# sile/libflate

Measured on AMD Instinct MI355X. Metric: gzip encode+decode throughput on 256 MiB synthetic text per GPU (uncompressed bytes through the round trip), higher is better.
Workload: dtype u8; 1 GPU; cfg2: gzip::Encoder (DefaultLz77Encoder, default options, mtime=0) + gzip::Decoder on TEXT(268435456 B) per GPU, write schedule S8K (8192-byte writes); bytes_per_gpu=268435456, schedule=S8K, compressed_bytes=129579521, parallelism=1 rank

## Files before the change

include/lfx_testhooks.h:

```cpp
#ifndef LFX_TESTHOOKS_H
#define LFX_TESTHOOKS_H

#include "lfx.h"

#ifdef __cplusplus
extern "C" {
#endif

int lfx_debug_huff_block(const uint32_t *hist320, uint32_t type, uint32_t *lit288, uint32_t *dist32, uint32_t *hdr160,
                         uint32_t *hdr_bits, uint64_t *body_bits);

int lfx_debug_plan(int format, const lfx_encode_opts *o, const lfx_schedule *s, uint64_t n, uint64_t *chunk_out,
                   size_t max_chunks, size_t *n_chunks, uint64_t *block_out, size_t max_blocks, size_t *n_blocks);

int lfx_debug_plan_incremental(int format, const lfx_encode_opts *o, const lfx_schedule *s, uint64_t n,
                               uint32_t take_every, uint64_t *chunk_out, size_t max_chunks, size_t *n_chunks,
                               uint64_t *block_out, size_t max_blocks, size_t *n_blocks);

void lfx_debug_symbols(uint32_t length, uint32_t distance, uint32_t *out6);

#ifdef __cplusplus
}
#endif
#endif
```

libflate_amd/csrc/lfx_ctx.h:

```cpp
#pragma once
#include <hip/hip_runtime.h>

#include <mutex>
#include <string>
#include <vector>

#include "lfx_common.h"
#include "lfx_device.h"
#include <string.h>

#include "lfx_hostio.h"

namespace lfx {

struct DevBuf {
    void *p = nullptr;
    size_t cap = 0;
    uint32_t gen = 0;
    int reserve(size_t bytes);
    void release();
};

struct Diag {
    bool debug = false;
    bool match_v1 = false;
    bool match_v5 = false;
    int r7_cap = 0;
    int match_parts = 1;
    bool no_serial = false;
    bool batch_serial = false;
    bool no_markers = false;
    bool no_pieces = false;
    bool no_final_cand = false;
    bool window_chain = false;
    int free_shift = -1;
    bool no_small_scan = false;
    bool two_pass = false;
    bool no_pin_slots = false;
    int find2_exp = 0;
    bool hist_separate = false;
    bool store_tight = false;
    int enc_batch_mb = 0;
    int pocr_max = 100;
    void read();
};

struct RangeState {
    int state = -1;
    uint64_t total = 0, before = 0, max_len = 0;
    uint8_t *d_out = nullptr;
    uint32_t nsu = 0;
};

struct Ctx {
    int device = 0;
    RangeState range;
    std::vector<uint8_t> range_stored;
    std::vector<uint64_t> range_temp_off;
    std::vector<uint32_t> range_cap;
    Diag diag;
    int n_cu = 0;
    hipStream_t own_stream = nullptr, stream = nullptr;
    hipStream_t side_stream = nullptr;
    hipEvent_t ev_fork = nullptr, ev_join = nullptr, ev_zero = nullptr;
    hipEvent_t ev_part[4] = {}, ev_res = nullptr;
    const void *prezero_ptr = nullptr;
    uint64_t prezero_bytes = 0;
    std::recursive_mutex mu;
    std::string err;
    void set_error(const std::string &e) { err = e; }

    DevBuf d_chunks, d_blocks, d_segs, d_pwgs, d_cd, d_md, d_codes, d_ncodes, d_hist, d_bc, d_block_start, d_tile_bits,
        d_tile_start, d_ck, d_res, d_small, d_hdr, d_io_in, d_io_out, d_vis, d_segtmp, d_stage, d_chunkmap, d_glnk, d_ucount;
    std::vector<uint8_t> up_shadow[4];
    uint64_t up_dev[4] = {0, 0, 0, 0};
    DevBuf d_dec_streams, d_dec_state, d_dec_tmp, d_dec_cand, d_dec_blocks, d_dec_tabs, d_dec_sym, d_dec_win, d_dec_maps,
        d_dec_temp, d_dec_lanesx;
    DevBuf d_idx_tasks, d_idx_probe, d_idx_stage;
    DevBuf d_idx_enc;
    struct IdxCollect *idx = nullptr;
    struct IdxCollect *idx_enc = nullptr;
    std::vector<DevBuf *> all_bufs() {
        return {&d_chunks, &d_blocks, &d_segs, &d_pwgs, &d_cd, &d_md, &d_codes, &d_ncodes, &d_hist, &d_bc, &d_block_start,
                &d_tile_bits, &d_tile_start, &d_ck, &d_res, &d_small, &d_hdr, &d_io_in, &d_io_out, &d_vis, &d_segtmp, &d_stage, &d_chunkmap, &d_glnk, &d_ucount,
                &d_dec_streams, &d_dec_state, &d_dec_tmp, &d_dec_cand, &d_dec_blocks, &d_dec_tabs, &d_dec_sym, &d_dec_win, &d_dec_maps,
                &d_dec_temp, &d_dec_lanesx, &d_idx_tasks, &d_idx_probe, &d_idx_stage, &d_idx_enc};
    }
    void *h_res = nullptr;
    static constexpr size_t PIN_ARENA = 1u << 20;
    size_t pin_used = 0;
    struct PinDown { void *slot, *dst; size_t n; };
    std::vector<PinDown> pin_pending;
    void pin_reset() { pin_used = 0; pin_pending.clear(); }
    void *pin_take(size_t n) {
        const size_t at = (pin_used + 63) & ~(size_t)63;
        if (!h_res || diag.no_pin_slots || at + n > PIN_ARENA) return nullptr;
        pin_used = at + n;
        return (uint8_t *)h_res + 4096 + at;
    }
    hipError_t small_up(void *dev, const void *host, size_t n, hipStream_t st) {
        if (!n) return hipSuccess;
        void *slot = pin_take(n);
        if (!slot) return hipMemcpyAsync(dev, host, n, hipMemcpyHostToDevice, st);
        memcpy(slot, host, n);
        return hipMemcpyAsync(dev, slot, n, hipMemcpyHostToDevice, st);
    }
    hipError_t small_down(void *host, const void *dev, size_t n, hipStream_t st) {
        if (!n) return hipSuccess;
        void *slot = pin_take(n);
        if (!slot) return hipMemcpyAsync(host, dev, n, hipMemcpyDeviceToHost, st);
        pin_pending.push_back({slot, host, n});
        return hipMemcpyAsync(slot, dev, n, hipMemcpyDeviceToHost, st);
    }
    hipError_t small_sync(hipStream_t st) {
        const hipError_t e = hipStreamSynchronize(st);
        for (const PinDown &d : pin_pending) memcpy(d.dst, d.slot, d.n);
        pin_pending.clear();
        return e;
    }

    uint32_t cur_nchunks = 0, cur_nblocks = 0;
    uint64_t cur_ntiles = 0, cur_n = 0;
    const uint32_t *cur_tile_map = nullptr;
    const uint8_t *cur_in = nullptr;
    bool force_match_v1 = false;
    uint64_t match_fallbacks = 0;
    HostIo hostio;
    static constexpr size_t POOL_MAX = 8;
    std::vector<PinVec> pin_pool;
    std::vector<DevBuf> dev_pool;
    PinVec take_pin() {
        std::lock_guard<std::recursive_mutex> lock(mu);
        if (pin_pool.empty()) return PinVec();
        size_t best = 0;
        for (size_t i = 1; i < pin_pool.size(); i++)
            if (pin_pool[i].capacity() > pin_pool[best].capacity()) best = i;
        PinVec v = std::move(pin_pool[best]);
        pin_pool.erase(pin_pool.begin() + (std::ptrdiff_t)best);
        v.clear();
        return v;
    }
    void give_pin(PinVec &&v) {
        std::lock_guard<std::recursive_mutex> lock(mu);
        if (v.capacity() && pin_pool.size() < POOL_MAX) { v.clear(); pin_pool.push_back(std::move(v)); }
    }
    DevBuf take_dev() {
        std::lock_guard<std::recursive_mutex> lock(mu);
        if (dev_pool.empty()) return DevBuf();
        DevBuf b = dev_pool.back();
        dev_pool.pop_back();
        return b;
    }
    void give_dev(DevBuf &b) {
        std::lock_guard<std::recursive_mutex> lock(mu);
        if (b.p && dev_pool.size() < POOL_MAX) dev_pool.push_back(b);
        else b.release();
        b = DevBuf();
    }
    std::vector<uint8_t> shard_hdr;
    int shard_format = 0;
    bool shard_last = false;

    int timing_on = 0;
    bool timing_fine() const { return timing_on >= 2; }
    hipEvent_t ev[17] = {};
    char ev_name[17][24] = {};
    int n_ev = 0;
    void phase(const char *name);
};

struct HostCodes {
    const uint32_t *codes;
    uint64_t n_codes;
    const uint32_t *chunk_codes;
};
int encode_prepare(Ctx *c, const struct Plan &plan, const struct PlanOpts &po, const uint8_t *d_in,
                   uint64_t n, int ck_mode, const HostCodes *hc = nullptr);

}
```

libflate_amd/csrc/lfx_decode.cpp:

```cpp
#include "../../include/lfx.h"

#include <hip/hip_runtime.h>

#include <algorithm>
#include <cstddef>
#include <cstdio>
#include <cstdlib>
#include <cstring>
#include <mutex>
#include <string>
#include <vector>

#include "lfx_ctx.h"
#include "lfx_container.h"
#include "lfx_decode.h"
#include "lfx_index.h"
#include <thread>
#include <chrono>

static_assert(offsetof(lfx::DecStream, out_off) == 16 && sizeof(lfx::DecStream) % 8 == 0, "checksum_ranges stride");
static_assert(offsetof(lfx::InflateResult, out_len) == 8 && sizeof(lfx::InflateResult) % 8 == 0, "checksum_ranges stride");
#include "lfx_device.h"
#include "lfx_abi_guard.h"

using namespace lfx;

#define HIP_TRY(expr)                                                                 \
    do {                                                                              \
        hipError_t e_ = (expr);                                                       \
        if (e_ != hipSuccess) {                                                       \
            c->set_error(std::string(#expr) + ": " + hipGetErrorString(e_));          \
            return LFX_E_DEVICE;                                                      \
        }                                                                             \
    } while (0)
#define LAUNCH_TRY(call)                                                              \
    do {                                                                              \
        int e_ = (call);                                                              \
        if (e_) {                                                                     \
            c->set_error(std::string(#call) + ": " + hipGetErrorString((hipError_t)e_)); \
            return LFX_E_DEVICE;                                                      \
        }                                                                             \
    } while (0)

namespace {

std::string format_error(uint32_t err, uint32_t a0, uint32_t a1) {
    char m[200];
    switch (err) {
        case ERR_EOF: return "failed to fill whole buffer";
        case ERR_HUFF: return "Invalid huffman coded stream";
        case ERR_CONFLICT: snprintf(m, sizeof m, "Bit region conflict: symbol=%u", a0); return m;
        case ERR_HDIST: snprintf(m, sizeof m, "The value of HDIST is too big: max=30, actual=%u", a0); return m;
        case ERR_NO_PREV: return "No preceding value";
        case ERR_DIST_LIST:
            snprintf(m, sizeof m, "The length of `distance_code_bitwidthes` is too large: actual=%u, expected=%u", a0, a1);
            return m;
        case ERR_286: snprintf(m, sizeof m, "The value %u must not occur in compressed data", a0); return m;
        case ERR_BACKREF: snprintf(m, sizeof m, "Too long backword reference: buffer.len=%u, distance=%u", a0, a1); return m;
        case ERR_BTYPE3: return "btype 0x11 of DEFLATE is reserved(error) value";
        case ERR_LEN_NLEN: snprintf(m, sizeof m, "LEN=%u is not the one's complement of NLEN=%u", a0, a1); return m;
        case ERR_STORED_SHORT: snprintf(m, sizeof m, "The reader has incorrect length: expected %u, read %u", a0, a1); return m;
        case ERR_NOSPACE: return "output capacity too small";
        case ERR_ZLIB_CHECK:
            snprintf(m, sizeof m, "Inconsistent ZLIB check bits: `CMF(%u) * 256 + FLG(%u)` must be a multiple of 31", a0, a1);
            return m;
        case ERR_METHOD: snprintf(m, sizeof m, "Compression methods other than DEFLATE(8) are unsupported: method=%u", a0); return m;
        case ERR_CINFO: snprintf(m, sizeof m, "CINFO above 7 are not allowed: value=%u", a0); return m;
        case ERR_FDICT: snprintf(m, sizeof m, "Preset dictionaries are not supported: dictionary_id=0x%X", a0); return m;
        case ERR_GZIP_ID: return "Unexpected GZIP ID";
        case ERR_HCRC: snprintf(m, sizeof m, "CRC16 of GZIP header mismatched: value=%u, expected=%u", a0, a1); return m;
        case ERR_CRC32: snprintf(m, sizeof m, "CRC32 mismatched: value=%u, expected=%u", a0, a1); return m;
        case ERR_ADLER32: snprintf(m, sizeof m, "Adler32 checksum mismatched: value=%u, expected=%u", a0, a1); return m;
        default: return "";
    }
}
int map_status(uint32_t st) {
    return st == 0 ? LFX_OK : st == 1 ? LFX_E_INVALID_DATA : st == 2 ? LFX_E_UNEXPECTED_EOF : LFX_E_NOSPACE;
}

struct MemberResult {
    int status = LFX_OK;
    uint64_t out_len = 0;
    uint64_t blk_out_start = 0;
    uint64_t end_byte = 0;
    std::string msg;
    uint64_t end_bit = 0;
    bool final_seen = false;
    bool need_cap = false;
    int ck_mode = 0;
    uint32_t trailer_len = 0;
    bool ck_done = false;
    uint32_t crc32 = 0, adler32 = 1;
    uint8_t trailer[8] = {0, 0, 0, 0, 0, 0, 0, 0};
};

int run_jobs(Ctx *c, const uint8_t *d_in, uint8_t *d_out, const std::vector<InflateJob> &jobs,
             std::vector<InflateResult> &res) {
    const size_t n = jobs.size();
    res.resize(n);
    if (!n) return LFX_OK;
    int rc;
    if ((rc = c->d_dec_streams.reserve(sizeof(InflateJob) * n))) return rc;
    if ((rc = c->d_dec_state.reserve(sizeof(InflateResult) * n))) return rc;
    HIP_TRY(hipMemcpyAsync(c->d_dec_streams.p, jobs.data(), sizeof(InflateJob) * n, hipMemcpyHostToDevice, c->stream));
    LAUNCH_TRY(launch_inflate(c->stream, d_in, d_out, (const InflateJob *)c->d_dec_streams.p,
                              (InflateResult *)c->d_dec_state.p, (uint32_t)n));
    HIP_TRY(hipMemcpyAsync(res.data(), c->d_dec_state.p, sizeof(InflateResult) * n, hipMemcpyDeviceToHost, c->stream));
    HIP_TRY(hipStreamSynchronize(c->stream));
    return LFX_OK;
}

int inflate_member(Ctx *c, const uint8_t *d_in, uint64_t n, uint64_t off0, uint8_t *d_out, uint64_t cap,
                   MemberResult &mr, uint64_t start_bit0 = ~0ull, uint64_t stop_bit = ~0ull, bool partial = false,
                   uint64_t hist = 0) {
    const uint64_t first_bit = start_bit0 == ~0ull ? off0 * 8 : start_bit0;
    mr.end_bit = first_bit;
    hipStream_t st = c->stream;
    c->pin_reset();
    std::vector<InflateJob> jobs;
    std::vector<InflateResult> res;
    bool parallel_done = false;
    const uint64_t comp = n > off0 ? n - off0 : 0;
    if (comp >= (4u << 10)) {
        int rc;
        bool overflow = false;
        uint32_t n1 = 0;
        std::vector<uint64_t> starts;
        auto find_candidates = [&]() -> int {
            const uint32_t shard_cap = find_shard_cap(comp);
            const uint32_t final_cap = (uint32_t)std::min<uint64_t>(std::max<uint64_t>(1u << 16, comp / 4096), 1u << 24);
            int rc;
            if ((rc = c->d_dec_cand.reserve(8ull * shard_cap * FIND_SHARDS + 8ull * final_cap + 4 * FIND_HDR_WORDS))) return rc;
            uint32_t *d_count = (uint32_t *)c->d_dec_cand.p;
            uint32_t *d_final_count = d_count + FIND_HDR_FINAL;
            uint64_t *d_final = (uint64_t *)((uint8_t *)c->d_dec_cand.p + 4 * FIND_HDR_WORDS);
            uint64_t *d_cand = d_final + final_cap;
            HIP_TRY(hipMemsetAsync(d_count, 0, 4 * FIND_HDR_WORDS, st));
            const uint64_t tail_bytes = std::max<uint64_t>(comp / 8, 8ull << 20);
            const uint64_t final_from = c->diag.no_final_cand ? ~0ull >> 1 : comp > tail_bytes ? (n - tail_bytes) * 8 : 0;
            LAUNCH_TRY(launch_find_stage1(st, d_in, n, off0, d_count, d_cand, shard_cap, final_from, (uint32_t)std::max(c->n_cu, 1)));
            c->phase("find1");
            const int find2_exp = c->diag.find2_exp >= 1 && c->diag.find2_exp <= 4 ? c->diag.find2_exp : 0;
            if (find2_exp) {
                LAUNCH_TRY(launch_find_stage2(st, d_in, n, d_cand, shard_cap, d_count, d_count + FIND_HDR_WORK, d_final_count, d_final, final_cap,
                                              (uint32_t)std::max(c->n_cu, 1), nullptr, find2_exp));
                HIP_TRY(hipMemsetAsync(d_count + FIND_HDR_FINAL, 0, 4, st));
                HIP_TRY(hipMemsetAsync(d_count + FIND_HDR_WORK, 0, 4 * (FIND_HDR_WORDS - FIND_HDR_WORK), st));
                c->phase("find2x");
            }
            LAUNCH_TRY(launch_find_stage2(st, d_in, n, d_cand, shard_cap, d_count, d_count + FIND_HDR_WORK, d_final_count, d_final, final_cap,
                                          (uint32_t)std::max(c->n_cu, 1), c->diag.debug ? (uint64_t *)(d_count + FIND_HDR_DBG) : nullptr));
            constexpr uint32_t HEAD_N = 1024;
            const uint32_t head_n = std::min<uint32_t>(HEAD_N, final_cap);
            std::vector<uint64_t> back(FIND_HDR_WORDS / 2 + head_n);
            HIP_TRY(c->small_down(back.data(), d_count, 8ull * back.size(), st));
            HIP_TRY(c->small_sync(st));
            const uint32_t *hc = (const uint32_t *)back.data();
            std::vector<uint64_t> cand(back.begin() + FIND_HDR_WORDS / 2, back.end());
            overflow = hc[FIND_SHARDS] != 0;
            n1 = 0;
            for (uint32_t k = 0; k < FIND_SHARDS; k++) { if (hc[k] > shard_cap) overflow = true; n1 += hc[k]; }
            if (c->diag.debug) {
                uint64_t d[7];
                memcpy(d, hc + FIND_HDR_DBG, sizeof d);
                fprintf(stderr, "[lfx] finder stage 2: batches=%llu cycles per batch: stage+fields=%llu table=%llu walk=%llu; steps per batch=%.1f "
                        "restagings=%llu; wavefront lives (sum)=%llu\n", (unsigned long long)d[5], (unsigned long long)(d[0] / (d[5] ? d[5] : 1)),
                        (unsigned long long)(d[1] / (d[5] ? d[5] : 1)), (unsigned long long)(d[2] / (d[5] ? d[5] : 1)),
                        (double)d[3] / (double)(d[5] ? d[5] : 1), (unsigned long long)d[4], (unsigned long long)d[6]);
            }
            starts.clear();
            starts.push_back(first_bit);
            if (overflow) return LFX_OK;
            uint32_t nf = hc[FIND_HDR_FINAL];
            if (nf > final_cap) nf = final_cap;
            cand.resize(nf);
            if (nf > head_n) HIP_TRY(hipMemcpy(cand.data() + head_n, d_final + head_n, 8ull * (nf - head_n), hipMemcpyDeviceToHost));
            c->phase("find2");
            for (uint32_t i = 0; i < nf; i++) if (cand[i] != first_bit) starts.push_back(cand[i]);
            std::sort(starts.begin(), starts.end());
            return LFX_OK;
        };
        const bool small_first = comp < (1536u << 10) && stop_bit == ~0ull && !partial && !c->diag.no_pieces;
        if (small_first) starts.push_back(first_bit);
        else if ((rc = find_candidates())) return rc;
        if (!overflow) {
            uint32_t nc = (uint32_t)starts.size();
            auto start_at = [&](uint32_t i) { return i < nc ? starts[i] : n * 8; };
            std::vector<BlkEmit> emit;
            uint32_t n_placed = 0;
            bool scan_small = false;
            uint64_t pos = first_bit, total = 0, total_codes = 0;
            bool ok_chain = false, chain_final = false;
            bool front_bad = false;
            uint64_t last_end = 0;
            bool pieces_mode = false;
            uint32_t n_on_demand = 0;
            bool pieces_multi = false;
            bool units_per_piece = false;
            const size_t tab_bytes = blk_tabs_bytes();
            const bool giant_blocks = nc <= 8 && comp / nc >= (2u << 20);
            if (!small_first && !giant_blocks && nc >= 2 && nc <= (uint32_t)c->diag.pocr_max && comp / nc >= (128u << 10) && stop_bit == ~0ull &&
                !partial && !c->diag.no_pieces) {
                const uint64_t end_bits = n * 8;
                const uint64_t ptarget = (uint64_t)std::max<int64_t>(2ll * std::max(c->n_cu, 1) - (int64_t)nc, (int64_t)nc);
                const uint64_t PIECE_BITS = std::min<uint64_t>(4ull << 20, std::max<uint64_t>(256ull << 10,
                                            ((end_bits - first_bit) / ptarget + 63) & ~63ull));
                const uint64_t OVERLAP = PIECE_BITS <= (1ull << 20) ? 2048 : 8192;
                std::vector<BlkJob> pj;
                std::vector<uint32_t> first_piece(nc + 1, 0);
                auto add_pieces = [&](std::vector<BlkJob> &jobs, uint64_t s0, uint64_t s1) {
                    const uint64_t len = s1 - s0;
                    const uint64_t np0 = std::max<uint64_t>((len + PIECE_BITS - 1) / PIECE_BITS, 1);
                    const uint64_t pb = std::max<uint64_t>(((len + np0 - 1) / np0 + 63) & ~63ull, 64);
                    const uint32_t np = (uint32_t)std::max<uint64_t>((len + pb - 1) / pb, 1);
                    for (uint32_t q = 0; q < np; q++) {
                        const uint64_t lo = s0 + q * pb;
                        jobs.push_back(BlkJob{s0, std::min(lo + pb, s1), q ? lo : 0, q ? lo - OVERLAP : 0, 1u, 0u});
                    }
                };
                for (uint32_t i = 0; i < nc; i++) {
                    first_piece[i] = (uint32_t)pj.size();
                    add_pieces(pj, starts[i], start_at(i + 1));
                }
                first_piece[nc] = (uint32_t)pj.size();
                const uint32_t npj = (uint32_t)pj.size();
                units_per_piece = npj >= (uint32_t)std::max(c->n_cu, 1);
                constexpr uint32_t REPAIRS = 2;
                const uint32_t repair_slots = REPAIRS * (2 * (uint32_t)((end_bits - first_bit) / nc / PIECE_BITS + 2) + 4);
                const uint32_t nslots = npj + repair_slots;
                int rc2;
                if ((rc2 = c->d_dec_streams.reserve(sizeof(BlkJob) * nslots))) return rc2;
                if ((rc2 = c->d_dec_state.reserve(sizeof(BlkInfo) * nslots))) return rc2;
                if ((rc2 = c->d_dec_blocks.reserve(sizeof(BlkLanes) * (size_t)nslots))) return rc2;
                if ((rc2 = c->d_dec_tabs.reserve(tab_bytes * nslots))) return rc2;
                HIP_TRY(hipMemcpyAsync(c->d_dec_streams.p, pj.data(), sizeof(BlkJob) * npj, hipMemcpyHostToDevice, st));
                LAUNCH_TRY(launch_blk_scan(st, d_in, n, (const BlkJob *)c->d_dec_streams.p, npj, (BlkInfo *)c->d_dec_state.p,
                                           (BlkLanes *)c->d_dec_blocks.p, c->d_dec_tabs.p));
                std::vector<BlkInfo> pi(npj);
                HIP_TRY(hipMemcpyAsync(pi.data(), c->d_dec_state.p, sizeof(BlkInfo) * npj, hipMemcpyDeviceToHost, st));
                HIP_TRY(hipStreamSynchronize(st));
                bool fail = false;
                auto walk_range = [&](const BlkInfo *infos, uint32_t cnt, uint32_t slot0) -> int {
                    uint64_t prev_end = 0;
                    for (uint32_t q = 0; q < cnt; q++) {
                        const BlkInfo &r = infos[q];
                        if (r.status == BLK_BAD || r.btype == 0 || (q && r.data_bit != prev_end) || r.end_bit <= pos || r.end_bit > end_bits) return 2;
                        BlkEmit e{};
                        e.start_bit = pos; e.data_bit = r.data_bit; e.code_off = total_codes; e.out_off = total;
                        e.n_out = r.n_out; e.n_codes = r.n_codes; e.nlanes = r.nlanes; e.btype = r.btype; e.cand = slot0 + q;
                        e.hist = hist + total;
                        e.end_limit = r.status == BLK_NO_EOB ? r.end_bit : 0;
                        emit.push_back(e);
                        total += r.n_out;
                        total_codes += r.n_codes;
                        prev_end = r.end_bit;
                        if (r.status == BLK_OK) {
                            last_end = r.end_bit;
                            pieces_multi |= q > 0;
                            if (r.bfinal) { ok_chain = true; chain_final = true; } else pos = r.end_bit;
                            return 0;
                        }
                    }
                    return 1;
                };
                uint32_t repairs = 0, rslot = npj;
                for (uint32_t i = 0; i < nc && !fail && !ok_chain; i++) {
                    if (starts[i] != pos) { fail = true; break; }
                    const size_t emit_mark = emit.size();
                    const uint64_t total_mark = total, codes_mark = total_codes;
                    int res = walk_range(&pi[first_piece[i]], first_piece[i + 1] - first_piece[i], first_piece[i]);
                    if (res == 1 && i + 1 < nc && repairs < REPAIRS) {
                        emit.resize(emit_mark); total = total_mark; total_codes = codes_mark;
                        std::vector<BlkJob> rj;
                        add_pieces(rj, starts[i], start_at(i + 2));
                        const uint32_t nr = (uint32_t)rj.size();
                        if (rslot + nr > nslots) { fail = true; break; }
                        HIP_TRY(hipMemcpyAsync((BlkJob *)c->d_dec_streams.p + rslot, rj.data(), sizeof(BlkJob) * nr, hipMemcpyHostToDevice, st));
                        LAUNCH_TRY(launch_blk_scan(st, d_in, n, (const BlkJob *)c->d_dec_streams.p + rslot, nr, (BlkInfo *)c->d_dec_state.p + rslot,
                                                   (BlkLanes *)c->d_dec_blocks.p + rslot, (uint8_t *)c->d_dec_tabs.p + tab_bytes * rslot));
                        std::vector<BlkInfo> ri(nr);
                        HIP_TRY(hipMemcpyAsync(ri.data(), (BlkInfo *)c->d_dec_state.p + rslot, sizeof(BlkInfo) * nr, hipMemcpyDeviceToHost, st));
                        HIP_TRY(hipStreamSynchronize(st));
                        res = walk_range(ri.data(), nr, rslot);
                        if (c->diag.debug) fprintf(stderr, "[lfx]  pieces: candidate %u (bit %llu) is a false one, its block scanned again in %u pieces: %d\n", i + 1,
                                                   (unsigned long long)starts[i + 1], nr, res);
                        rslot += nr;
                        repairs++;
                        i++;
                    }
                    if (res != 0) fail = true;
                }
                if (c->diag.debug) fprintf(stderr, "[lfx]  pieces over %u candidate ranges: ok=%d fail=%d pieces=%zu of %u total=%llu\n", nc, (int)ok_chain, (int)fail,
                                           emit.size(), npj, (unsigned long long)total);
                if (fail || !ok_chain) { emit.clear(); pos = first_bit; total = 0; total_codes = 0; ok_chain = false; chain_final = false; last_end = 0; pieces_multi = false; units_per_piece = false; }
                else pieces_mode = true;
                c->phase("pieces");
            }
            if (!pieces_mode && (small_first || (nc <= 8 && comp / nc >= (2u << 20))) && stop_bit == ~0ull && !partial && !c->diag.no_pieces) {
                const uint64_t end_bits = n * 8;
                const uint64_t PIECE_BITS = std::min<uint64_t>(4ull << 20, std::max<uint64_t>(256ull << 10,
                                            ((end_bits - first_bit) / (2ull * (uint64_t)std::max(c->n_cu, 1)) + 63) & ~63ull));
                const uint64_t OVERLAP = PIECE_BITS <= (1ull << 20) ? 2048 : 8192;
                const uint32_t cap_slots = (uint32_t)std::min<uint64_t>((end_bits - first_bit) / PIECE_BITS * 2 + 64, 1u << 20);
                int rc2;
                if ((rc2 = c->d_dec_streams.reserve(sizeof(BlkJob) * cap_slots))) return rc2;
                if ((rc2 = c->d_dec_state.reserve(sizeof(BlkInfo) * cap_slots))) return rc2;
                if ((rc2 = c->d_dec_blocks.reserve(sizeof(BlkLanes) * (size_t)cap_slots))) return rc2;
                if ((rc2 = c->d_dec_tabs.reserve(tab_bytes * cap_slots))) return rc2;
                uint32_t base = 0;
                bool fail = false;
                for (uint32_t iter = 0; iter < (small_first ? 4u : 64u) && !fail && !ok_chain; iter++) {
                    const uint32_t np = (uint32_t)((end_bits - pos + PIECE_BITS - 1) / PIECE_BITS);
                    if (np == 0 || base + np > cap_slots) { fail = true; break; }
                    std::vector<BlkJob> pj(np);
                    for (uint32_t q = 0; q < np; q++) {
                        const uint64_t lo = pos + q * PIECE_BITS;
                        pj[q] = BlkJob{pos, std::min(lo + PIECE_BITS, end_bits), q ? lo : 0, q ? lo - OVERLAP : 0, 1u, 0u};
                    }
                    HIP_TRY(hipMemcpyAsync((BlkJob *)c->d_dec_streams.p + base, pj.data(), sizeof(BlkJob) * np, hipMemcpyHostToDevice, st));
                    LAUNCH_TRY(launch_blk_scan(st, d_in, n, (const BlkJob *)c->d_dec_streams.p + base, np, (BlkInfo *)c->d_dec_state.p + base,
                                               (BlkLanes *)c->d_dec_blocks.p + base, (uint8_t *)c->d_dec_tabs.p + tab_bytes * base));
                    std::vector<BlkInfo> pi(np);
                    HIP_TRY(hipMemcpyAsync(pi.data(), (BlkInfo *)c->d_dec_state.p + base, sizeof(BlkInfo) * np, hipMemcpyDeviceToHost, st));
                    HIP_TRY(hipStreamSynchronize(st));
                    uint32_t used = 0;
                    bool closed = false;
                    uint64_t prev_end = 0;
                    for (uint32_t q = 0; q < np && !closed; q++) {
                        const BlkInfo &r = pi[q];
                        if (c->diag.debug && (q < 3 || r.status != BLK_NO_EOB))
                            fprintf(stderr, "[lfx]   piece %u/%u: status=%u btype=%u data=%llu end=%llu prev_end=%llu lanes=%u codes=%u out=%llu rounds=%u cyc_hdr=%u cyc_total=%u\n", q, np,
                                    r.status, r.btype, (unsigned long long)r.data_bit, (unsigned long long)r.end_bit,
                                    (unsigned long long)prev_end, r.nlanes, r.n_codes, (unsigned long long)r.n_out, r.rounds, r.cyc_hdr, r.cyc_total);
                        if (r.status == BLK_BAD || (q && r.data_bit != prev_end) || r.end_bit <= pos || r.end_bit > end_bits) { fail = true; break; }
                        if (q == 0 && r.btype == 0 && r.status != BLK_OK) { fail = true; break; }
                        BlkEmit e{};
                        e.start_bit = pos; e.data_bit = r.data_bit; e.code_off = total_codes; e.out_off = total;
                        e.n_out = r.n_out; e.n_codes = r.n_codes; e.nlanes = r.nlanes; e.btype = r.btype; e.cand = base + q;
                        e.hist = hist + total;
                        e.end_limit = r.status == BLK_NO_EOB ? r.end_bit : 0;
                        emit.push_back(e);
                        total += r.n_out;
                        total_codes += r.n_codes;
                        used = q + 1;
                        prev_end = r.end_bit;
                        if (r.status == BLK_OK) {
                            closed = true;
                            last_end = r.end_bit;
                            pieces_multi |= q > 0;
                            if (r.bfinal) { ok_chain = true; chain_final = true; } else pos = r.end_bit;
                        }
                    }
                    if (!closed) fail = true;
                    base += used;
                }
                if (c->diag.debug) fprintf(stderr, "[lfx]  pieces: ok=%d fail=%d pieces=%zu total=%llu\n", (int)ok_chain, (int)fail, emit.size(), (unsigned long long)total);
                if (fail || !ok_chain) { emit.clear(); pos = first_bit; total = 0; total_codes = 0; ok_chain = false; last_end = 0; pieces_multi = false; }
                else pieces_mode = true;
                c->phase("pieces");
                if (small_first && !pieces_mode) {
                    if ((rc = find_candidates())) return rc;
                    nc = (uint32_t)starts.size();
                }
            }
            if (!pieces_mode && !overflow) {
            std::vector<BlkJob> bj(nc);
            for (uint32_t i = 0; i < nc; i++) bj[i] = BlkJob{starts[i], start_at(i + 1)};
            std::vector<int32_t> alt(nc, -1);
            {
                std::vector<uint64_t> len(nc);
                for (uint32_t i = 0; i < nc; i++) len[i] = bj[i].end_bit - bj[i].start_bit;
                std::vector<uint64_t> sorted = len;
                std::nth_element(sorted.begin(), sorted.begin() + nc / 2, sorted.end());
                const uint64_t median = sorted[nc / 2], thresh = median / 5 * 3;
                const uint32_t max_extra = nc / 4 + 4;
                for (uint32_t i = 0; i + 1 < nc && bj.size() - nc < max_extra; i++) {
                    if (len[i] >= thresh && len[i + 1] >= thresh) continue;
                    if (i + 2 == nc && len[i] >= thresh) continue;
                    if (len[i] + len[i + 1] > median + median / 4) continue;
                    alt[i] = (int32_t)bj.size();
                    bj.push_back(BlkJob{starts[i], start_at(i + 2)});
                }
            }
            if (nc > 1 && nc <= 8 && alt[0] < 0 && comp / nc >= (2u << 20)) {
                alt[0] = (int32_t)bj.size();
                bj.push_back(BlkJob{starts[0], n * 8});
            }
            const uint32_t nj = (uint32_t)bj.size();
            constexpr uint32_t EXTRA = 64, MAX_ON_DEMAND = 1u << 16;
            if ((rc = c->d_dec_streams.reserve(sizeof(BlkJob) * (nj + 1)))) return rc;
            if ((rc = c->d_dec_state.reserve(sizeof(BlkInfo) * (nj + EXTRA + 1)))) return rc;
            if ((rc = c->d_dec_blocks.reserve(sizeof(BlkLanes) * (size_t)(nj + EXTRA + 1)))) return rc;
            if ((rc = c->d_dec_tabs.reserve(tab_bytes * (nj + EXTRA + 1)))) return rc;
            std::vector<uint8_t> stored(nj + EXTRA + 1, 0);
            bool store_mode = !c->diag.two_pass && nj && (n * 8) / nj >= (1ull << 20);
            scan_small = !c->diag.no_small_scan && nj && (n * 8) / nj < (512ull << 10);
            if (store_mode) {
                uint64_t off = 0;
                for (uint32_t j = 0; j < nj; j++) {
                    const uint64_t bits = bj[j].end_bit > bj[j].start_bit ? bj[j].end_bit - bj[j].start_bit : 0;
                    const uint64_t slice = std::max<uint64_t>((bits + 1023) / 1024, 128);
                    const uint64_t cap = (slice / (c->diag.store_tight ? 16 : 2) + 448 + 64 + 3) & ~3ull;
                    bj[j].temp_off = off;
                    bj[j].cap = (uint32_t)cap;
                    off += 1024 * cap;
                }
                if (off * 4 > (16ull << 30) || c->d_dec_temp.reserve(off * 4) || c->d_dec_lanesx.reserve(sizeof(BlkLanesX) * (size_t)(nj + 1))) {
                    store_mode = false;
                    for (uint32_t j = 0; j < nj; j++) { bj[j].temp_off = 0; bj[j].cap = 0; }
                }
            }
            HIP_TRY(c->small_up(c->d_dec_streams.p, bj.data(), sizeof(BlkJob) * nj, st));
            if (store_mode)
                LAUNCH_TRY(launch_blk_scan_store(st, d_in, n, (const BlkJob *)c->d_dec_streams.p, nj, (BlkInfo *)c->d_dec_state.p,
                                                 (BlkLanes *)c->d_dec_blocks.p, c->d_dec_tabs.p, (uint32_t *)c->d_dec_temp.p,
                                                 (BlkLanesX *)c->d_dec_lanesx.p));
            else
                LAUNCH_TRY(launch_blk_scan(st, d_in, n, (const BlkJob *)c->d_dec_streams.p, nj, (BlkInfo *)c->d_dec_state.p,
                                           (BlkLanes *)c->d_dec_blocks.p, c->d_dec_tabs.p, scan_small));
            std::vector<BlkInfo> bi(nj);
            HIP_TRY(c->small_down(bi.data(), c->d_dec_state.p, sizeof(BlkInfo) * nj, st));
            HIP_TRY(c->small_sync(st));
            for (BlkInfo &b : bi) if (b.status == BLK_OK && b.end_bit > n * 8) b.status = BLK_NO_EOB;
            if (store_mode) for (uint32_t j = 0; j < nj; j++) stored[j] = bi[j].status == BLK_OK && bi[j].btype != 0 && bi[j]._pad == 0;
            c->phase("blk_scan");
            std::vector<uint32_t> slot(nc);
            for (uint32_t i = 0; i < nc; i++)
                slot[i] = (bi[i].status == BLK_NO_EOB && alt[i] >= 0 && bi[alt[i]].status == BLK_OK) ? (uint32_t)alt[i] : i;
            if (c->diag.debug) {
                fprintf(stderr, "[lfx] finder: stage1=%u candidates=%u scan jobs=%u (alternatives: %u)\n", n1, nc, nj, nj - nc);
                for (uint32_t i = 0; i < nc && i < 12; i++)
                    fprintf(stderr, "[lfx]  cand %u start=%llu status=%u btype=%u final=%u end=%llu n_out=%llu n_codes=%u lanes=%u rounds=%u cyc_hdr=%u cyc_total=%u\n",
                            i, (unsigned long long)starts[i], bi[i].status, bi[i].btype, bi[i].bfinal,
                            (unsigned long long)bi[i].end_bit, (unsigned long long)bi[i].n_out, bi[i].n_codes,
                            bi[i].nlanes, bi[i].rounds, bi[i].cyc_hdr, bi[i].cyc_total);
                uint32_t nbad = 0, maxr = 0;
                for (uint32_t i = 0; i < nc; i++) { nbad += bi[i].status != BLK_OK; maxr = std::max(maxr, bi[i].rounds); }
                fprintf(stderr, "[lfx]  not-ok=%u max_rounds=%u\n", nbad, maxr);
            }
            for (uint32_t widen = 2; widen <= 6; widen++) {
                std::vector<uint32_t> redo;
                for (uint32_t i = 0; i < nc; i++) if (bi[slot[i]].status == BLK_NO_EOB && i + widen <= nc) redo.push_back(i);
                if (redo.empty()) break;
                std::vector<BlkJob> rj(redo.size());
                for (size_t q = 0; q < redo.size(); q++) rj[q] = BlkJob{starts[redo[q]], start_at(redo[q] + widen)};
                if ((rc = c->d_dec_tmp.reserve(sizeof(BlkJob) * redo.size()))) return rc;
                BlkJob *d_rj = (BlkJob *)c->d_dec_tmp.p;
                HIP_TRY(hipMemcpyAsync(d_rj, rj.data(), sizeof(BlkJob) * redo.size(), hipMemcpyHostToDevice, st));
                for (size_t q = 0; q < redo.size(); q++) {
                    slot[redo[q]] = redo[q];
                    stored[redo[q]] = 0;
                    LAUNCH_TRY(launch_blk_scan(st, d_in, n, d_rj + q, 1, (BlkInfo *)c->d_dec_state.p + redo[q],
                                               (BlkLanes *)c->d_dec_blocks.p + redo[q],
                                               (uint8_t *)c->d_dec_tabs.p + tab_bytes * redo[q], scan_small));
                }
                for (size_t q = 0; q < redo.size(); q++)
                    HIP_TRY(hipMemcpyAsync(&bi[redo[q]], (BlkInfo *)c->d_dec_state.p + redo[q], sizeof(BlkInfo), hipMemcpyDeviceToHost, st));
                HIP_TRY(hipStreamSynchronize(st));
            }
            c->phase("repair");
            uint32_t n_extra = 0;
            n_on_demand = 0;
            for (;;) {
                if (pos == stop_bit && !emit.empty()) { ok_chain = true; break; }
                auto it = std::lower_bound(starts.begin(), starts.end(), pos);
                uint32_t k;
                BlkInfo r;
                if (it != starts.end() && *it == pos) { k = slot[(uint32_t)(it - starts.begin())]; r = bi[k]; }
                else {
                    if (pos >= n * 8 || n_on_demand++ >= MAX_ON_DEMAND || n_extra >= EXTRA) break;
                    k = nj + n_extra;
                    const BlkJob one{pos, it != starts.end() ? *it : n * 8};
                    BlkJob *d_one = (BlkJob *)c->d_dec_streams.p + nj;
                    HIP_TRY(hipMemcpyAsync(d_one, &one, sizeof one, hipMemcpyHostToDevice, st));
                    LAUNCH_TRY(launch_blk_scan(st, d_in, n, d_one, 1, (BlkInfo *)c->d_dec_state.p + k,
                                               (BlkLanes *)c->d_dec_blocks.p + k, (uint8_t *)c->d_dec_tabs.p + tab_bytes * k, scan_small));
                    HIP_TRY(hipMemcpyAsync(&r, (BlkInfo *)c->d_dec_state.p + k, sizeof r, hipMemcpyDeviceToHost, st));
                    HIP_TRY(hipStreamSynchronize(st));
                    if (r.status == BLK_OK && r.btype != 0) n_extra++;
                }
                if (r.status == BLK_OK && r.end_bit > n * 8) r.status = BLK_NO_EOB;
                if (r.status != BLK_OK || r.end_bit <= pos) { front_bad = emit.empty() && r.status == BLK_BAD; break; }
                if (partial && total + r.n_out > cap) { mr.need_cap = emit.empty(); break; }
                BlkEmit e{};
                e.start_bit = pos; e.data_bit = r.data_bit; e.code_off = total_codes; e.out_off = total;
                e.n_out = r.n_out; e.n_codes = r.n_codes; e.nlanes = r.nlanes; e.btype = r.btype; e.cand = k;
                e.hist = hist + total;
                if (k < nj && stored[k]) { e.placed = 1; e.temp_off = bj[k].temp_off; e.cap = bj[k].cap; n_placed++; }
                emit.push_back(e);
                total += r.n_out;
                total_codes += r.n_codes;
                last_end = r.end_bit;
                if (r.bfinal) { ok_chain = true; chain_final = true; break; }
                pos = r.end_bit;
            }
            if (partial && !ok_chain && !emit.empty()) ok_chain = true;
            }
            if (c->diag.debug) fprintf(stderr, "[lfx]  chain ok=%d blocks=%zu pos=%llu total=%llu on_demand=%u\n", (int)ok_chain, emit.size(), (unsigned long long)pos, (unsigned long long)total, n_on_demand);
            if (partial && emit.empty() && !front_bad) {
                mr.status = LFX_OK; mr.out_len = 0; mr.blk_out_start = 0; mr.final_seen = false;
                mr.end_bit = first_bit; mr.end_byte = first_bit / 8;
                return LFX_OK;
            }
            if (ok_chain && total <= cap) {
                const uint32_t ne = (uint32_t)emit.size();
                if ((rc = c->d_dec_tmp.reserve(sizeof(BlkEmit) * 2 * (size_t)ne + 64))) return rc;
                if ((rc = c->d_hist.reserve(sizeof(BlkUnits) * 2 * (size_t)ne + 64))) return rc;
                if ((rc = c->d_codes.reserve(4 * std::max<uint64_t>(total_codes, 1)))) return rc;
                uint32_t *d_flags = (uint32_t *)c->d_dec_tmp.p;
                BlkEmit *d_emit = (BlkEmit *)((uint8_t *)c->d_dec_tmp.p + 64);
                uint64_t *dbgbuf = nullptr;
                if (c->diag.debug) {
                    if ((rc = c->d_ck.reserve(64ull * 8 * ne + 64))) return rc;
                    dbgbuf = (uint64_t *)c->d_ck.p;
                    HIP_TRY(hipMemsetAsync(dbgbuf, 0, 64ull * 8 * ne, st));
                }
                {
                    std::vector<uint8_t> upl(64 + sizeof(BlkEmit) * (size_t)ne, 0);
                    memcpy(upl.data() + 64, emit.data(), sizeof(BlkEmit) * (size_t)ne);
                    HIP_TRY(c->small_up(d_flags, upl.data(), upl.size(), st));
                }
                const uint64_t slots = 4ull * (uint64_t)std::max(c->n_cu, 1);
                const uint32_t unit_target = (uint32_t)std::min<uint64_t>((total_codes + slots - 1) / slots + 1, 0x7FFFFFFFu);
                uint32_t free_shift = 15;
                while (free_shift < 20 && (total >> (free_shift + 1)) >= 2ull * (uint64_t)std::max(c->n_cu, 1)) free_shift++;
                if (pieces_mode && units_per_piece) free_shift = 20;
                if (c->diag.free_shift >= 0) free_shift = (uint32_t)c->diag.free_shift;
                if (n_placed)
                    LAUNCH_TRY(launch_blk_place(st, d_emit, ne, (const BlkLanes *)c->d_dec_blocks.p, (const BlkLanesX *)c->d_dec_lanesx.p,
                                                (const uint32_t *)c->d_dec_temp.p, (uint32_t *)c->d_codes.p, d_flags,
                                                (BlkUnits *)c->d_hist.p, unit_target, nullptr, free_shift));
                if (n_placed < ne)
                    LAUNCH_TRY(launch_blk_emit(st, d_in, n, d_emit, ne, (const BlkLanes *)c->d_dec_blocks.p,
                                               (uint32_t *)c->d_codes.p, d_flags, (BlkUnits *)c->d_hist.p, unit_target, nullptr,
                                               c->d_dec_tabs.p, free_shift, total_codes >= 32768ull * ne, scan_small && !pieces_mode));
                c->phase("blk_emit");
                bool giant = pieces_multi;
                for (const BlkEmit &e : emit) giant |= e.n_out >= (8ull << 20);
                const bool probe = !giant && total / ne < (256u << 10);
                uint32_t fl = 0;
                if (probe) {
                    HIP_TRY(c->small_down(&fl, d_flags, 4, st));
                    HIP_TRY(c->small_sync(st));
                }
                bool ck_spec = false;
                if (!giant && !(probe && fl == 2 && !c->diag.no_markers)) {
                    LAUNCH_TRY(launch_blk_materialize(st, d_in, d_emit, ne, (const BlkLanes *)c->d_dec_blocks.p,
                                                      (const BlkUnits *)c->d_hist.p, (const uint32_t *)c->d_codes.p, d_out, dbgbuf));
                    const uint64_t tb = (pos == stop_bit ? pos : last_end), tpos = tb / 8 + ((tb & 7) ? 1 : 0);
                    if (mr.ck_mode && total && !partial && !c->diag.debug && tpos + mr.trailer_len <= n) {
                        c->phase("lz77_copy");
                        const uint64_t nspans = ck_nspans(total);
                        if ((rc = c->d_ck.reserve(12 * nspans))) return rc;
                        if ((rc = c->d_res.reserve(256))) return rc;
                        uint32_t *ck = (uint32_t *)c->d_ck.p;
                        LAUNCH_TRY(launch_checksum(st, d_out, total, ck, ck + nspans, ck + 2 * nspans, (EncodeResult *)c->d_res.p, mr.ck_mode));
                        HIP_TRY(hipMemcpyAsync(c->h_res, c->d_res.p, sizeof(EncodeResult), hipMemcpyDeviceToHost, st));
                        if (mr.trailer_len) HIP_TRY(hipMemcpyAsync((uint8_t *)c->h_res + 256, d_in + tpos, mr.trailer_len, hipMemcpyDeviceToHost, st));
                        ck_spec = true;
                    }
                }
                HIP_TRY(c->small_down(&fl, d_flags, 4, st));
                HIP_TRY(c->small_sync(st));
                if (ck_spec && fl == 0) {
                    const EncodeResult er = *(EncodeResult *)c->h_res;
                    mr.ck_done = true; mr.crc32 = er.crc32; mr.adler32 = er.adler32;
                    memcpy(mr.trailer, (uint8_t *)c->h_res + 256, mr.trailer_len);
                    c->phase("checksum");
                }
                if (giant && !(fl & 1) && !c->diag.no_markers) fl = 2;
                else if (giant) {
                    LAUNCH_TRY(launch_blk_materialize(st, d_in, d_emit, ne, (const BlkLanes *)c->d_dec_blocks.p,
                                                      (const BlkUnits *)c->d_hist.p, (const uint32_t *)c->d_codes.p, d_out, dbgbuf));
                    HIP_TRY(hipStreamSynchronize(st));
                }
                if (!ck_spec) c->phase("lz77_copy");
                if (c->diag.debug) {
                    fprintf(stderr, "[lfx]  emit flags=%u\n", fl);
                    std::vector<BlkUnits> uv(ne);
                    (void)hipMemcpy(uv.data(), c->d_hist.p, sizeof(BlkUnits) * ne, hipMemcpyDeviceToHost);
                    for (uint32_t u = 0; u < 3 && u < ne; u++)
                        fprintf(stderr, "[lfx]  K2 block %u: units=%u hdr=%u decode=%u cut=%u select=%u\n", u, uv[u].n, uv[u].cyc[0],
                                uv[u].cyc[1], uv[u].cyc[2], uv[u].cyc[3]);
                    std::vector<uint64_t> dv(64ull * ne);
                    (void)hipMemcpy(dv.data(), dbgbuf, 64ull * 8 * ne, hipMemcpyDeviceToHost);
                    uint32_t nunits = 0;
                    uint64_t maxcyc = 0, tmin = ~0ull, tmax = 0;
                    for (uint32_t u = 0; u < 8 * ne; u++) {
                        if (!dv[u * 8 + 1]) continue;
                        nunits++;
                        maxcyc = std::max(maxcyc, dv[u * 8]);
                        tmin = std::min(tmin, dv[u * 8 + 6]); tmax = std::max(tmax, dv[u * 8 + 6]);
                    }
                    fprintf(stderr, "[lfx]  K3: units=%u max_cycles=%llu end-time spread=%.1f us (100 MHz clock)\n", nunits,
                            (unsigned long long)maxcyc, (double)(tmax - tmin) / 100.0);
                    for (uint32_t u = 0; u < 8 && u < 8 * ne; u++)
                        fprintf(stderr, "[lfx]  K3 unit %u: cycles=%llu batches=%llu nseq=%llu seq_cycles=%llu codes=%llu bytes=%llu\n", u,
                                (unsigned long long)dv[u * 8], (unsigned long long)dv[u * 8 + 1], (unsigned long long)dv[u * 8 + 2],
                                (unsigned long long)dv[u * 8 + 3], (unsigned long long)dv[u * 8 + 4], (unsigned long long)dv[u * 8 + 5]);
                }
                const uint8_t *init_win = hist ? d_out - MAX_WINDOW : nullptr;
                if (fl == 2 && !c->diag.no_markers) {
                    std::vector<BlkUnits> uv(ne);
                    HIP_TRY(hipMemcpyAsync(uv.data(), c->d_hist.p, sizeof(BlkUnits) * ne, hipMemcpyDeviceToHost, st));
                    HIP_TRY(hipStreamSynchronize(st));
                    std::vector<SymUnit> su;
                    uint64_t max_len = 0;
                    for (uint32_t q = 0; q < ne; q++)
                        for (uint32_t b = 0; b < uv[q].fn && b < MAX_FREE_UNITS; b++) {
                            const uint64_t len = uv[q].fout0[b + 1] - uv[q].fout0[b];
                            if (!len) continue;
                            su.push_back(SymUnit{emit[q].out_off + uv[q].fout0[b], len});
                            max_len = std::max(max_len, len);
                        }
                    const uint32_t nsu = (uint32_t)su.size();
                    if ((rc = c->d_dec_sym.reserve(2 * std::max<uint64_t>(total, 1)))) return rc;
                    if ((rc = c->d_dec_win.reserve(32768ull * std::max<uint32_t>(nsu, 1) + sizeof(SymUnit) * (size_t)nsu + 64))) return rc;
                    uint8_t *d_win = (uint8_t *)c->d_dec_win.p;
                    SymUnit *d_su = (SymUnit *)(d_win + 32768ull * std::max<uint32_t>(nsu, 1));
                    HIP_TRY(hipMemcpyAsync(d_su, su.data(), sizeof(SymUnit) * nsu, hipMemcpyHostToDevice, st));
                    LAUNCH_TRY(launch_blk_materialize_sym(st, d_in, d_emit, ne, (const BlkUnits *)c->d_hist.p,
                                                          (const uint32_t *)c->d_codes.p, (uint16_t *)c->d_dec_sym.p,
                                                          nsu <= (uint32_t)std::max(c->n_cu, 1) && !c->diag.window_chain));
                    c->phase("lz77_sym");
                    if (nsu >= 16 && !c->diag.window_chain) {
                        if ((rc = c->d_dec_maps.reserve(window_prefix_scratch_bytes(nsu)))) return rc;
                        LAUNCH_TRY(launch_window_prefix(st, (const uint16_t *)c->d_dec_sym.p, d_su, nsu, c->d_dec_maps.p, d_win, init_win));
                    } else LAUNCH_TRY(launch_window_chain(st, (const uint16_t *)c->d_dec_sym.p, d_su, nsu, d_win, init_win));
                    c->phase("win_chain");
                    LAUNCH_TRY(launch_sym_substitute(st, (const uint16_t *)c->d_dec_sym.p, d_su, nsu, d_win, d_out, max_len, init_win));
                    HIP_TRY(hipStreamSynchronize(st));
                    c->phase("substitute");
                    if (c->diag.debug) fprintf(stderr, "[lfx]  cross-block references: %u blocks, %u units through markers\n", ne, nsu);
                    fl = 0;
                }
                if (fl == 2) {
                    std::vector<BlkEmit> runs;
                    for (uint32_t q = 0; q < ne; ) {
                        BlkEmit r = emit[q];
                        uint32_t q2 = q + 1;
                        if (r.btype != 0) {
                            r.btype = 2;
                            uint64_t nco = r.n_codes;
                            while (q2 < ne && emit[q2].btype != 0 && nco + emit[q2].n_codes < 0xFFFFFFFFull) {
                                nco += emit[q2].n_codes; r.n_out += emit[q2].n_out; q2++;
                            }
                            r.n_codes = (uint32_t)nco;
                        }
                        r.preload = r.hist != 0;
                        runs.push_back(r);
                        q = q2;
                    }
                    const uint32_t nr = (uint32_t)runs.size();
                    std::vector<BlkUnits> ru(nr);
                    for (uint32_t q = 0; q < nr; q++) {
                        ru[q] = BlkUnits{};
                        ru[q].n = 1; ru[q].code0[0] = 0; ru[q].code0[1] = runs[q].n_codes; ru[q].out0[0] = 0; ru[q].out0[1] = runs[q].n_out;
                    }
                    BlkEmit *d_runs = (BlkEmit *)((uint8_t *)c->d_dec_tmp.p + 64) + ne;
                    BlkUnits *d_ru = (BlkUnits *)c->d_hist.p + ne;
                    HIP_TRY(hipMemcpyAsync(d_runs, runs.data(), sizeof(BlkEmit) * nr, hipMemcpyHostToDevice, st));
                    HIP_TRY(hipMemcpyAsync(d_ru, ru.data(), sizeof(BlkUnits) * nr, hipMemcpyHostToDevice, st));
                    for (uint32_t q = 0; q < nr; q++)
                        LAUNCH_TRY(launch_blk_materialize(st, d_in, d_runs + q, 1, (const BlkLanes *)c->d_dec_blocks.p, d_ru + q,
                                                          (const uint32_t *)c->d_codes.p, d_out, nullptr));
                    HIP_TRY(hipStreamSynchronize(st));
                    c->phase("lz77_chain");
                    if (c->diag.debug) fprintf(stderr, "[lfx]  cross-block references: %u blocks re-materialised in %u ordered runs\n", ne, nr);
                    fl = 0;
                }
                if (fl == 0) {
                    if (c->idx && (rc = idx_record_chain(c, emit.data(), ne, (const BlkLanes *)c->d_dec_blocks.p, c->idx->bit_base,
                                                         c->idx->out_base, true)))
                        return rc;
                    mr.status = LFX_OK;
                    mr.out_len = total;
                    mr.blk_out_start = total;
                    const uint64_t eb = pos == stop_bit ? pos : last_end;
                    mr.end_byte = eb / 8 + ((eb & 7) ? 1 : 0);
                    mr.end_bit = eb;
                    mr.final_seen = chain_final;
                    parallel_done = true;
                }
            }
        }
    }
    if (!parallel_done && c->diag.no_serial) { c->set_error("serial fallback disabled (LFX_NO_SERIAL)"); return LFX_E_UNSUPPORTED; }
    if (!parallel_done) {
        jobs.clear();
        InflateJob j{};
        j.in_off = 0; j.in_len = n; j.start_bit = first_bit;
        j.out_off = 0; j.out_cap = cap; j.hist_avail = hist; j.flags = 0;
        j.stop_bit = stop_bit == ~0ull ? 0 : stop_bit;
        jobs.push_back(j);
        int rc;
        if ((rc = run_jobs(c, d_in, d_out, jobs, res))) return rc;
        c->phase("serial");
        InflateResult &r = res[0];
        if (stop_bit != ~0ull && r.status == 0 && (r.final_seen || r.end_bit != stop_bit)) {
            r.status = 1; r.err = ERR_HUFF; r.a0 = r.a1 = 0;
        }
        mr.status = map_status(r.status);
        mr.out_len = r.out_len;
        mr.blk_out_start = r.status ? r.blk_out_start : r.out_len;
        mr.end_byte = std::min<uint64_t>((r.end_bit + 7) / 8, n);
        mr.end_bit = r.end_bit;
        mr.final_seen = r.status == 0 && r.final_seen;
        mr.msg = format_error(r.err, r.a0, r.a1);
        if (partial && r.status != 0 && (r.status == 2 || r.status == 3 || r.end_bit + 64 >= n * 8)) {
            mr.status = LFX_OK;
            mr.out_len = mr.blk_out_start = r.blk_out_start;
            mr.end_bit = r.blk_start_bit;
            mr.end_byte = r.blk_start_bit / 8;
            mr.final_seen = false;
            mr.need_cap = r.status == 3 && r.blk_out_start == 0;
            mr.msg.clear();
        }
    }
    return LFX_OK;
}

struct DecodeOutcome {
    int status = LFX_OK;
    uint64_t out_len = 0, delivered_len = 0, consumed = 0;
    bool header_failed = false;
    bool more = false;
    std::string msg;
};

int decode_stream(Ctx *c, int format, uint32_t flags, const uint8_t *d_in, uint64_t n, uint8_t *d_out,
                  uint64_t cap, DecodeOutcome &oc, uint64_t base = 0, uint64_t out_at = 0, bool one_member = false,
                  std::vector<lfx_member> *members = nullptr) {
    (void)hipSetDevice(c->device);
    hipStream_t st = c->stream;
    bool first = base == 0;
    oc.consumed = base;
    oc.out_len = oc.delivered_len = out_at;
    int rc;
    if ((rc = c->d_res.reserve(256))) return rc;
    if ((rc = c->d_small.reserve(70000))) return rc;
    for (;;) {
        uint64_t off0 = 0;
        if (format != LFX_DEFLATE) {
            DecStream ds{base, n - base, 0, 0};
            DecHeader dh{};
            c->pin_reset();
            HIP_TRY(c->small_up(c->d_small.p, &ds, sizeof ds, st));
            LAUNCH_TRY(launch_container(st, format, 1, d_in, (const DecStream *)c->d_small.p,
                                        (DecHeader *)((uint8_t *)c->d_small.p + 256)));
            HIP_TRY(c->small_down(&dh, (uint8_t *)c->d_small.p + 256, sizeof dh, st));
            HIP_TRY(c->small_sync(st));
            if (dh.status != 0) {
                if (!first && dh.status == 2) {
                    oc.consumed = n;
                    break;
                }
                oc.status = map_status(dh.status);
                oc.header_failed = first;
                oc.msg = format_error(dh.err, dh.a0, dh.a1);
                oc.consumed = base + dh.deflate_off;
                oc.out_len = oc.delivered_len = out_at;
                return LFX_OK;
            }
            off0 = dh.deflate_off;
        }
        if (c->idx) {
            c->idx->bit_base = base * 8;
            c->idx->out_base = out_at;
            c->idx->cand.push_back(IdxCand{(base + off0) * 8, (base + off0) * 8, out_at, IDX_BTYPE_READ});
        }
        MemberResult mr;
        mr.ck_mode = format == LFX_GZIP ? 1 : format == LFX_ZLIB ? 2 : 0;
        mr.trailer_len = format == LFX_GZIP ? 8 : format == LFX_ZLIB ? 4 : 0;
        if ((rc = inflate_member(c, d_in + base, n - base, off0, d_out + out_at, cap - out_at, mr))) return rc;
        oc.out_len = out_at + mr.out_len;
        oc.delivered_len = out_at + mr.blk_out_start;
        oc.consumed = base + mr.end_byte;
        if (mr.status != LFX_OK) { oc.status = mr.status; oc.msg = mr.msg; return LFX_OK; }
        if (format != LFX_DEFLATE) {
            const uint64_t need = format == LFX_GZIP ? 8 : 4;
            const uint64_t tpos = base + mr.end_byte;
            if (n - tpos < need) {
                oc.status = LFX_E_UNEXPECTED_EOF;
                oc.msg = "failed to fill whole buffer";
                oc.consumed = n;
                return LFX_OK;
            }
            uint8_t t[8];
            EncodeResult er{};
            if (mr.ck_done) {
                er.crc32 = mr.crc32; er.adler32 = mr.adler32;
                memcpy(t, mr.trailer, need);
            } else {
                const uint64_t nspans = ck_nspans(mr.out_len);
                if ((rc = c->d_ck.reserve(12 * nspans))) return rc;
                uint32_t *ck = (uint32_t *)c->d_ck.p;
                LAUNCH_TRY(launch_checksum(st, d_out + out_at, mr.out_len, ck, ck + nspans, ck + 2 * nspans, (EncodeResult *)c->d_res.p,
                                           format == LFX_GZIP ? 1 : format == LFX_ZLIB ? 2 : 3));
                HIP_TRY(hipMemcpyAsync(c->h_res, c->d_res.p, sizeof(EncodeResult), hipMemcpyDeviceToHost, st));
                HIP_TRY(hipMemcpyAsync(t, d_in + tpos, need, hipMemcpyDeviceToHost, st));
                HIP_TRY(hipStreamSynchronize(st));
                c->phase("checksum");
                er = *(EncodeResult *)c->h_res;
            }
            oc.consumed = tpos + need;
            if (format == LFX_GZIP) {
                const uint32_t crc = (uint32_t)t[0] | (uint32_t)t[1] << 8 | (uint32_t)t[2] << 16 | (uint32_t)t[3] << 24;
                if (crc != er.crc32) {
                    oc.status = LFX_E_INVALID_DATA;
                    oc.msg = format_error(ERR_CRC32, er.crc32, crc);
                    return LFX_OK;
                }
            } else {
                const uint32_t ad = (uint32_t)t[0] << 24 | (uint32_t)t[1] << 16 | (uint32_t)t[2] << 8 | t[3];
                if (ad != er.adler32) {
                    oc.status = LFX_E_INVALID_DATA;
                    oc.msg = format_error(ERR_ADLER32, er.adler32, ad);
                    return LFX_OK;
                }
            }
        }
        if (members) members->push_back(lfx_member{base, oc.consumed - base, out_at, mr.out_len});
        out_at = oc.out_len;
        if (one_member) { oc.more = true; break; }
        if (!(format == LFX_GZIP && (flags & LFX_DEC_MULTI))) break;
        base = oc.consumed;
        first = false;
    }
    oc.out_len = oc.delivered_len = out_at;
    return LFX_OK;
}

}

extern "C" int lfx_decode_device(lfx_ctx *cc, int format, uint32_t flags, const void *d_in, uint64_t n,
                                 void *d_out, uint64_t cap, uint64_t *out_len, uint64_t *consumed) try {
    if (!cc) return LFX_E_DEVICE;
    Ctx *c = reinterpret_cast<Ctx *>(cc);
    std::lock_guard<std::recursive_mutex> lock(c->mu);
    if (format < 0 || format > 2) return LFX_E_ARG;
    (void)hipSetDevice(c->device);
    c->n_ev = 0;
    c->phase("start");
    DecodeOutcome oc;
    int rc = decode_stream(c, format, flags, (const uint8_t *)d_in, n, (uint8_t *)d_out, cap, oc);
    if (rc) return rc;
    if (oc.status == LFX_OK) c->phase("done");
    if (oc.out_len > cap) oc.out_len = cap;
    if (out_len) *out_len = oc.out_len;
    if (consumed) *consumed = oc.consumed;
    if (oc.status != LFX_OK) c->set_error(oc.msg);
    return oc.status;
} LFX_ABI_CATCH

extern "C" int lfx_decode_shard_device(lfx_ctx *cc, const void *d_in, uint64_t n, uint64_t start_bit,
                                       uint64_t total_bits, int is_last, void *d_out, uint64_t cap,
                                       uint64_t *out_len) try {
    if (!cc) return LFX_E_DEVICE;
    Ctx *c = reinterpret_cast<Ctx *>(cc);
    std::lock_guard<std::recursive_mutex> lock(c->mu);
    (void)hipSetDevice(c->device);
    c->n_ev = 0;
    c->phase("start");
    MemberResult mr;
    int rc = inflate_member(c, (const uint8_t *)d_in, n, start_bit >> 3, (uint8_t *)d_out, cap, mr, start_bit,
                            is_last ? ~0ull : start_bit + total_bits);
    if (rc) return rc;
    if (out_len) *out_len = mr.out_len;
    if (mr.status != LFX_OK) c->set_error(mr.msg);
    return mr.status;
} LFX_ABI_CATCH

static_assert(sizeof(lfx_blk_tuple) == 56, "tuple layout (all-gathered as raw bytes)");

extern "C" int lfx_decode_range_scan(lfx_ctx *cc, const void *d_part_, uint64_t n_part, uint64_t lo_byte, uint64_t hi_byte,
                                     uint64_t first_bit, uint64_t final_from_bit, uint32_t rank, lfx_blk_tuple *tuples, uint32_t cap,
                                     uint32_t *count) try {
    if (!cc) return LFX_E_DEVICE;
    Ctx *c = reinterpret_cast<Ctx *>(cc);
    std::lock_guard<std::recursive_mutex> lock(c->mu);
    (void)hipSetDevice(c->device);
    hipStream_t st = c->stream;
    const uint8_t *d_in = (const uint8_t *)d_part_;
    if (!count || hi_byte < lo_byte || n_part < hi_byte - lo_byte) return LFX_E_ARG;
    *count = 0;
    c->n_ev = 0;
    c->phase("start");
    const uint64_t n = n_part, range_bits = (hi_byte - lo_byte) * 8, base_bit = lo_byte * 8;
    const uint32_t shard_cap = find_shard_cap(n);
    const uint32_t final_cap = (uint32_t)std::min<uint64_t>(std::max<uint64_t>(1u << 16, n / 4096), 1u << 24);
    int rc;
    if ((rc = c->d_dec_cand.reserve(8ull * shard_cap * FIND_SHARDS + 8ull * final_cap + 4 * FIND_HDR_WORDS))) return rc;
    uint32_t *d_count = (uint32_t *)c->d_dec_cand.p;
    uint32_t *d_final_count = d_count + FIND_HDR_FINAL;
    uint64_t *d_cand = (uint64_t *)((uint8_t *)c->d_dec_cand.p + 4 * FIND_HDR_WORDS);
    uint64_t *d_final = d_cand + (uint64_t)shard_cap * FIND_SHARDS;
    HIP_TRY(hipMemsetAsync(d_count, 0, 4 * FIND_HDR_WORDS, st));
    std::vector<uint64_t> starts;
    if (n >= 16) {
        const uint64_t base0 = lo_byte * 8;
        const uint64_t final_local = final_from_bit <= base0 ? 0 : std::min<uint64_t>(final_from_bit - base0, ~0ull >> 1);
        LAUNCH_TRY(launch_find_stage1(st, d_in, n, 0, d_count, d_cand, shard_cap, final_local, (uint32_t)std::max(c->n_cu, 1)));
        LAUNCH_TRY(launch_find_stage2(st, d_in, n, d_cand, shard_cap, d_count, d_count + FIND_HDR_WORK, d_final_count, d_final, final_cap,
                                      (uint32_t)std::max(c->n_cu, 1)));
        uint32_t hc[FIND_HDR_FINAL + 1];
        HIP_TRY(hipMemcpyAsync(hc, d_count, sizeof hc, hipMemcpyDeviceToHost, st));
        HIP_TRY(hipStreamSynchronize(st));
        bool overflow = hc[FIND_SHARDS] != 0;
        for (uint32_t k = 0; k < FIND_SHARDS; k++) if (hc[k] > shard_cap) overflow = true;
        if (overflow) { c->set_error("block finder overflow"); return LFX_E_UNSUPPORTED; }
        uint32_t nf = hc[FIND_HDR_FINAL];
        if (nf > final_cap) nf = final_cap;
        starts.resize(nf);
        if (nf) HIP_TRY(hipMemcpy(starts.data(), d_final, 8ull * nf, hipMemcpyDeviceToHost));
    }
    c->phase("find");
    if (first_bit != ~0ull) {
        if (first_bit < base_bit || first_bit - base_bit >= n * 8) return LFX_E_ARG;
        starts.push_back(first_bit - base_bit);
    }
    std::sort(starts.begin(), starts.end());
    starts.erase(std::unique(starts.begin(), starts.end()), starts.end());
    uint32_t nc = 0;
    while (nc < starts.size() && starts[nc] < range_bits) nc++;
    if (nc > cap) { c->set_error("more candidates than the caller's tuple buffer holds"); return LFX_E_NOSPACE; }
    const size_t tab_bytes = blk_tabs_bytes();
    c->range_stored.clear();
    if (nc) {
        auto start_at = [&](uint32_t i) { return i < starts.size() ? starts[i] : n * 8; };
        std::vector<BlkJob> bj(nc);
        for (uint32_t i = 0; i < nc; i++) bj[i] = BlkJob{starts[i], start_at(i + 1)};
        if ((rc = c->d_dec_streams.reserve(sizeof(BlkJob) * (nc + 1)))) return rc;
        if ((rc = c->d_dec_state.reserve(sizeof(BlkInfo) * (nc + 1)))) return rc;
        if ((rc = c->d_dec_blocks.reserve(sizeof(BlkLanes) * (size_t)(nc + 1)))) return rc;
        if ((rc = c->d_dec_tabs.reserve(tab_bytes * (nc + 1)))) return rc;
        bool store_mode = !c->diag.two_pass && (n * 8) / nc >= (1ull << 20);
        if (store_mode) {
            uint64_t off = 0;
            for (uint32_t j = 0; j < nc; j++) {
                const uint64_t bits = bj[j].end_bit > bj[j].start_bit ? bj[j].end_bit - bj[j].start_bit : 0;
                const uint64_t slice = std::max<uint64_t>((bits + 1023) / 1024, 128);
                const uint64_t lcap = (slice / (c->diag.store_tight ? 16 : 2) + 448 + 64 + 3) & ~3ull;
                bj[j].temp_off = off;
                bj[j].cap = (uint32_t)lcap;
                off += 1024 * lcap;
            }
            if (off * 4 > (16ull << 30) || c->d_dec_temp.reserve(off * 4) || c->d_dec_lanesx.reserve(sizeof(BlkLanesX) * (size_t)(nc + 1))) {
                store_mode = false;
                for (uint32_t j = 0; j < nc; j++) { bj[j].temp_off = 0; bj[j].cap = 0; }
            }
        }
        HIP_TRY(hipMemcpyAsync(c->d_dec_streams.p, bj.data(), sizeof(BlkJob) * nc, hipMemcpyHostToDevice, st));
        if (store_mode)
            LAUNCH_TRY(launch_blk_scan_store(st, d_in, n, (const BlkJob *)c->d_dec_streams.p, nc, (BlkInfo *)c->d_dec_state.p,
                                             (BlkLanes *)c->d_dec_blocks.p, c->d_dec_tabs.p, (uint32_t *)c->d_dec_temp.p,
                                             (BlkLanesX *)c->d_dec_lanesx.p));
        else
            LAUNCH_TRY(launch_blk_scan(st, d_in, n, (const BlkJob *)c->d_dec_streams.p, nc, (BlkInfo *)c->d_dec_state.p,
                                       (BlkLanes *)c->d_dec_blocks.p, c->d_dec_tabs.p));
        std::vector<BlkInfo> bi(nc);
        HIP_TRY(hipMemcpyAsync(bi.data(), c->d_dec_state.p, sizeof(BlkInfo) * nc, hipMemcpyDeviceToHost, st));
        HIP_TRY(hipStreamSynchronize(st));
        for (BlkInfo &b : bi) if (b.status == BLK_OK && b.end_bit > n * 8) b.status = BLK_NO_EOB;
        c->range_stored.assign(nc, 0);
        c->range_temp_off.assign(nc, 0);
        c->range_cap.assign(nc, 0);
        if (store_mode)
            for (uint32_t j = 0; j < nc; j++) {
                c->range_stored[j] = bi[j].status == BLK_OK && bi[j].btype != 0 && bi[j]._pad == 0;
                c->range_temp_off[j] = bj[j].temp_off;
                c->range_cap[j] = bj[j].cap;
            }
        for (uint32_t widen = 2; widen <= 6; widen++) {
            std::vector<uint32_t> redo;
            for (uint32_t i = 0; i < nc; i++) if (bi[i].status == BLK_NO_EOB && i + widen <= starts.size()) redo.push_back(i);
            if (redo.empty()) break;
            std::vector<BlkJob> rj(redo.size());
            for (size_t q = 0; q < redo.size(); q++) { rj[q] = BlkJob{starts[redo[q]], start_at(redo[q] + widen)}; c->range_stored[redo[q]] = 0; }
            if ((rc = c->d_dec_tmp.reserve(sizeof(BlkJob) * redo.size()))) return rc;
            BlkJob *d_rj = (BlkJob *)c->d_dec_tmp.p;
            HIP_TRY(hipMemcpyAsync(d_rj, rj.data(), sizeof(BlkJob) * redo.size(), hipMemcpyHostToDevice, st));
            for (size_t q = 0; q < redo.size(); q++)
                LAUNCH_TRY(launch_blk_scan(st, d_in, n, d_rj + q, 1, (BlkInfo *)c->d_dec_state.p + redo[q],
                                           (BlkLanes *)c->d_dec_blocks.p + redo[q], (uint8_t *)c->d_dec_tabs.p + tab_bytes * redo[q]));
            for (size_t q = 0; q < redo.size(); q++)
                HIP_TRY(hipMemcpyAsync(&bi[redo[q]], (BlkInfo *)c->d_dec_state.p + redo[q], sizeof(BlkInfo), hipMemcpyDeviceToHost, st));
            HIP_TRY(hipStreamSynchronize(st));
        }
        for (uint32_t i = 0; i < nc; i++) {
            lfx_blk_tuple &t = tuples[i];
            t = lfx_blk_tuple{};
            t.start_bit = base_bit + starts[i];
            t.end_bit = base_bit + bi[i].end_bit;
            t.n_out = bi[i].n_out;
            t.n_codes = bi[i].n_codes;
            t.btype = (uint8_t)bi[i].btype;
            t.bfinal = (uint8_t)bi[i].bfinal;
            t.status = (uint8_t)(bi[i].status == BLK_OK && bi[i].end_bit > n * 8 ? (uint32_t)BLK_NO_EOB : bi[i].status);
            t._pad = 0;
            t.slot = i;
            t.rank = (uint16_t)rank;
            t._pad2 = 0;
            t.nlanes = bi[i].nlanes;
            t.data_bit = base_bit + bi[i].data_bit;
        }
    }
    c->phase("blk_scan");
    *count = nc;
    return LFX_OK;
} LFX_ABI_CATCH

extern "C" int lfx_decode_chain(const lfx_blk_tuple *all, uint32_t n_all, uint64_t first_bit, uint32_t *chain, uint32_t cap,
                                uint32_t *n_chain, uint64_t *total_out) try {
    if (!all || !chain || !n_chain) return LFX_E_ARG;
    std::vector<uint32_t> order(n_all);
    for (uint32_t i = 0; i < n_all; i++) order[i] = i;
    std::sort(order.begin(), order.end(), [&](uint32_t a, uint32_t b) {
        return all[a].start_bit != all[b].start_bit ? all[a].start_bit < all[b].start_bit : all[a].rank < all[b].rank;
    });
    uint64_t pos = first_bit, total = 0;
    uint32_t k = 0;
    for (;;) {
        auto it = std::lower_bound(order.begin(), order.end(), pos, [&](uint32_t a, uint64_t v) { return all[a].start_bit < v; });
        if (it == order.end() || all[*it].start_bit != pos) return LFX_E_UNSUPPORTED;
        const lfx_blk_tuple &t = all[*it];
        if (t.status != BLK_OK || t.end_bit <= pos) return LFX_E_UNSUPPORTED;
        if (k >= cap) return LFX_E_NOSPACE;
        chain[k++] = *it;
        total += t.n_out;
        if (t.bfinal) break;
        pos = t.end_bit;
    }
    *n_chain = k;
    if (total_out) *total_out = total;
    return LFX_OK;
} LFX_ABI_CATCH

extern "C" int lfx_decode_range_emit(lfx_ctx *cc, const void *d_part_, uint64_t n_part, uint64_t lo_byte, const lfx_blk_tuple *all,
                                     const uint32_t *chain, uint32_t n_chain, uint32_t rank, void *d_out_, uint64_t cap,
                                     uint64_t *out_len, uint64_t *out_base, uint32_t *state) try {
    if (!cc) return LFX_E_DEVICE;
    Ctx *c = reinterpret_cast<Ctx *>(cc);
    std::lock_guard<std::recursive_mutex> lock(c->mu);
    (void)hipSetDevice(c->device);
    hipStream_t st = c->stream;
    const uint8_t *d_in = (const uint8_t *)d_part_;
    uint8_t *d_out = (uint8_t *)d_out_;
    const uint64_t base_bit = lo_byte * 8;
    c->range = RangeState{};
    std::vector<BlkEmit> emit;
    uint64_t before = 0, total = 0, total_codes = 0;
    uint32_t n_placed = 0;
    bool seen = false;
    for (uint32_t q = 0; q < n_chain; q++) {
        const lfx_blk_tuple &t = all[chain[q]];
        if (t.rank != rank) { if (!seen) before += t.n_out; continue; }
        seen = true;
        BlkEmit e{};
        e.start_bit = t.start_bit - base_bit; e.data_bit = t.data_bit - base_bit; e.code_off = total_codes; e.out_off = total;
        e.n_out = t.n_out; e.n_codes = t.n_codes; e.nlanes = t.nlanes; e.btype = t.btype; e.cand = t.slot;
        e.hist = before + total;
        if (t.slot < c->range_stored.size() && c->range_stored[t.slot]) {
            e.placed = 1; e.temp_off = c->range_temp_off[t.slot]; e.cap = c->range_cap[t.slot]; n_placed++;
        }
        emit.push_back(e);
        total += t.n_out;
        total_codes += t.n_codes;
    }
    if (out_base) *out_base = before;
    if (out_len) *out_len = total;
    if (state) *state = 0;
    if (total > cap) { c->set_error("output capacity too small"); return LFX_E_NOSPACE; }
    c->range.state = 0; c->range.total = total; c->range.d_out = d_out; c->range.before = before;
    if (emit.empty()) return LFX_OK;
    const uint32_t ne = (uint32_t)emit.size();
    int rc;
    if ((rc = c->d_dec_tmp.reserve(sizeof(BlkEmit) * (size_t)ne + 64))) return rc;
    if ((rc = c->d_hist.reserve(sizeof(BlkUnits) * (size_t)ne + 64))) return rc;
    if ((rc = c->d_codes.reserve(4 * std::max<uint64_t>(total_codes, 1)))) return rc;
    uint32_t *d_flags = (uint32_t *)c->d_dec_tmp.p;
    BlkEmit *d_emit = (BlkEmit *)((uint8_t *)c->d_dec_tmp.p + 64);
    HIP_TRY(hipMemsetAsync(d_flags, 0, 64, st));
    HIP_TRY(hipMemcpyAsync(d_emit, emit.data(), sizeof(BlkEmit) * ne, hipMemcpyHostToDevice, st));
    const uint64_t slots = 4ull * (uint64_t)std::max(c->n_cu, 1);
    const uint32_t unit_target = (uint32_t)std::min<uint64_t>((total_codes + slots - 1) / slots + 1, 0x7FFFFFFFu);
    uint32_t free_shift = 15;
    while (free_shift < 20 && (total >> (free_shift + 1)) >= 2ull * (uint64_t)std::max(c->n_cu, 1)) free_shift++;
    if (n_placed)
        LAUNCH_TRY(launch_blk_place(st, d_emit, ne, (const BlkLanes *)c->d_dec_blocks.p, (const BlkLanesX *)c->d_dec_lanesx.p,
                                    (const uint32_t *)c->d_dec_temp.p, (uint32_t *)c->d_codes.p, d_flags, (BlkUnits *)c->d_hist.p,
                                    unit_target, nullptr, free_shift));
    if (n_placed < ne)
        LAUNCH_TRY(launch_blk_emit(st, d_in, n_part, d_emit, ne, (const BlkLanes *)c->d_dec_blocks.p, (uint32_t *)c->d_codes.p, d_flags,
                                   (BlkUnits *)c->d_hist.p, unit_target, nullptr, c->d_dec_tabs.p, free_shift, total_codes >= 32768ull * ne));
    c->phase("blk_emit");
    const bool probe = total / ne < (256u << 10);
    uint32_t fl = 0;
    if (probe) {
        HIP_TRY(hipMemcpyAsync(&fl, d_flags, 4, hipMemcpyDeviceToHost, st));
        HIP_TRY(hipStreamSynchronize(st));
    }
    if (!(probe && fl)) {
        LAUNCH_TRY(launch_blk_materialize(st, d_in, d_emit, ne, (const BlkLanes *)c->d_dec_blocks.p, (const BlkUnits *)c->d_hist.p,
                                          (const uint32_t *)c->d_codes.p, d_out, nullptr));
        HIP_TRY(hipMemcpyAsync(&fl, d_flags, 4, hipMemcpyDeviceToHost, st));
        HIP_TRY(hipStreamSynchronize(st));
    }
    c->phase("lz77_copy");
    if (fl & 1) {
        c->range.state = -1;
        c->set_error("a back-reference reaches in front of the member's first byte: decode it with lfx_decode_device for the exact error");
        return LFX_E_INVALID_DATA;
    }
    if (fl == 2) {
        std::vector<BlkUnits> uv(ne);
        HIP_TRY(hipMemcpyAsync(uv.data(), c->d_hist.p, sizeof(BlkUnits) * ne, hipMemcpyDeviceToHost, st));
        HIP_TRY(hipStreamSynchronize(st));
        std::vector<SymUnit> su;
        uint64_t max_len = 0;
        for (uint32_t q = 0; q < ne; q++)
            for (uint32_t b = 0; b < uv[q].fn && b < MAX_FREE_UNITS; b++) {
                const uint64_t len = uv[q].fout0[b + 1] - uv[q].fout0[b];
                if (!len) continue;
                su.push_back(SymUnit{emit[q].out_off + uv[q].fout0[b], len});
                max_len = std::max(max_len, len);
            }
        const uint32_t nsu = (uint32_t)su.size();
        if ((rc = c->d_dec_sym.reserve(2 * std::max<uint64_t>(total, 1)))) return rc;
        if ((rc = c->d_dec_win.reserve(32768ull * (std::max<uint32_t>(nsu, 1) + 1) + sizeof(SymUnit) * (size_t)nsu + 64))) return rc;
        if ((rc = c->d_dec_maps.reserve(window_prefix_scratch_bytes(std::max<uint32_t>(nsu, 1))))) return rc;
        SymUnit *d_su = (SymUnit *)((uint8_t *)c->d_dec_win.p + 32768ull * (std::max<uint32_t>(nsu, 1) + 1));
        HIP_TRY(hipMemcpyAsync(d_su, su.data(), sizeof(SymUnit) * nsu, hipMemcpyHostToDevice, st));
        LAUNCH_TRY(launch_blk_materialize_sym(st, d_in, d_emit, ne, (const BlkUnits *)c->d_hist.p, (const uint32_t *)c->d_codes.p,
                                              (uint16_t *)c->d_dec_sym.p, nsu <= (uint32_t)std::max(c->n_cu, 1)));
        HIP_TRY(hipStreamSynchronize(st));
        c->phase("lz77_sym");
        c->range.state = 1; c->range.nsu = nsu; c->range.max_len = max_len;
        if (state) *state = 1;
    }
    return LFX_OK;
} LFX_ABI_CATCH

extern "C" int lfx_decode_range_map(lfx_ctx *cc, void *d_map) try {
    if (!cc) return LFX_E_DEVICE;
    Ctx *c = reinterpret_cast<Ctx *>(cc);
    std::lock_guard<std::recursive_mutex> lock(c->mu);
    (void)hipSetDevice(c->device);
    if (c->range.state < 0 || !d_map) { c->set_error("lfx_decode_range_map: no range_emit on this context"); return LFX_E_ARG; }
    if (c->range.state == 1) {
        const uint32_t nsu = c->range.nsu;
        const SymUnit *d_su = (const SymUnit *)((uint8_t *)c->d_dec_win.p + 32768ull * (std::max<uint32_t>(nsu, 1) + 1));
        LAUNCH_TRY(launch_window_rank_map(c->stream, (const uint16_t *)c->d_dec_sym.p, d_su, nsu, c->d_dec_maps.p, (uint16_t *)d_map));
    } else LAUNCH_TRY(launch_bytes_to_map(c->stream, c->range.d_out, c->range.total, (uint16_t *)d_map));
    HIP_TRY(hipStreamSynchronize(c->stream));
    return LFX_OK;
} LFX_ABI_CATCH

extern "C" int lfx_decode_range_finish(lfx_ctx *cc, const void *d_maps, uint32_t rank, uint32_t *crc32, uint32_t *adler32) try {
    if (!cc) return LFX_E_DEVICE;
    Ctx *c = reinterpret_cast<Ctx *>(cc);
    std::lock_guard<std::recursive_mutex> lock(c->mu);
    (void)hipSetDevice(c->device);
    hipStream_t st = c->stream;
    if (crc32) *crc32 = 0;
    if (adler32) *adler32 = 1;
    if (c->range.state < 0) { c->set_error("lfx_decode_range_finish: no range_emit on this context"); return LFX_E_ARG; }
    const uint64_t total = c->range.total;
    uint8_t *d_out = c->range.d_out;
    int rc;
    if (c->range.state == 1) {
        const uint32_t nsu = c->range.nsu;
        uint8_t *d_win = (uint8_t *)c->d_dec_win.p;
        uint8_t *d_init = d_win + 32768ull * std::max<uint32_t>(nsu, 1);
        const SymUnit *d_su = (const SymUnit *)(d_init + 32768);
        const uint8_t *init_win = nullptr;
        if (c->range.before) {
            if (!d_maps || !rank) { c->set_error("this slice reads the output of the ranks in front of it: their maps are needed"); return LFX_E_ARG; }
            if ((uintptr_t)d_maps & 15) { c->set_error("the gathered maps must be 16-byte aligned"); return LFX_E_ARG; }
            LAUNCH_TRY(launch_window_ranks(st, (const uint16_t *)d_maps, rank, d_init));
            init_win = d_init;
        }
        if (nsu >= 16 && !c->diag.window_chain)
            LAUNCH_TRY(launch_window_prefix(st, (const uint16_t *)c->d_dec_sym.p, d_su, nsu, c->d_dec_maps.p, d_win, init_win));
        else LAUNCH_TRY(launch_window_chain(st, (const uint16_t *)c->d_dec_sym.p, d_su, nsu, d_win, init_win));
        c->phase("win_chain");
        LAUNCH_TRY(launch_sym_substitute(st, (const uint16_t *)c->d_dec_sym.p, d_su, nsu, d_win, d_out, c->range.max_len, init_win));
        c->phase("substitute");
        c->range.state = 0;
    }
    if (total) {
        if ((rc = c->d_res.reserve(256))) return rc;
        const uint64_t nspans = ck_nspans(total);
        if ((rc = c->d_ck.reserve(12 * nspans))) return rc;
        uint32_t *ck = (uint32_t *)c->d_ck.p;
        LAUNCH_TRY(launch_checksum(st, d_out, total, ck, ck + nspans, ck + 2 * nspans, (EncodeResult *)c->d_res.p, 3));
        HIP_TRY(hipMemcpyAsync(c->h_res, c->d_res.p, sizeof(EncodeResult), hipMemcpyDeviceToHost, st));
        HIP_TRY(hipStreamSynchronize(st));
        const EncodeResult er = *(EncodeResult *)c->h_res;
        if (crc32) *crc32 = er.crc32;
        if (adler32) *adler32 = er.adler32;
    } else HIP_TRY(hipStreamSynchronize(st));
    c->phase("checksum");
    return LFX_OK;
} LFX_ABI_CATCH

extern "C" int lfx_decode_host(lfx_ctx *cc, int format, uint32_t flags, const void *in, uint64_t n, void *out,
                               uint64_t cap, uint64_t *out_len, uint64_t *consumed) try {
    if (!cc) return LFX_E_DEVICE;
    Ctx *c = reinterpret_cast<Ctx *>(cc);
    std::lock_guard<std::recursive_mutex> lock(c->mu);
    (void)hipSetDevice(c->device);
    int rc;
    if ((rc = c->d_io_in.reserve(std::max<uint64_t>(n, 4)))) return rc;
    if ((rc = c->d_io_out.reserve(std::max<uint64_t>(cap, 4)))) return rc;
    if (int hr = host_to_device(c, c->d_io_in.p, in, n, c->stream)) { c->set_error("host to device copy failed"); return hr; }
    uint64_t ol = 0;
    rc = lfx_decode_device(cc, format, flags, c->d_io_in.p, n, c->d_io_out.p, cap, &ol, consumed);
    if (rc == LFX_E_DEVICE || rc == LFX_E_OOM || rc == LFX_E_ARG) { (void)hipStreamSynchronize(c->stream); return rc; }
    if (ol) { if (int hr = device_to_host(c, out, c->d_io_out.p, ol, c->stream)) { c->set_error("device to host copy failed"); return hr; } }
    if (out_len) *out_len = ol;
    return rc;
} LFX_ABI_CATCH

namespace lfx {
static int batch_fast(Ctx *c, const uint8_t *d_in, uint64_t n_in, uint8_t *d_out, uint32_t count,
                      const std::vector<InflateJob> &jobs, std::vector<uint8_t> &fast, std::vector<InflateResult> &res) {
    constexpr uint32_t MAX_ROUNDS = 4;
    hipStream_t st = c->stream;
    struct Live { uint32_t stream; uint64_t bit, produced; uint32_t nblocks; };
    std::vector<Live> live;
    fast.assign(count, 0);
    res.assign(count, InflateResult{});
    for (uint32_t i = 0; i < count; i++)
        if (jobs[i].in_len >= 64 && jobs[i].in_off + jobs[i].in_len <= n_in)
            live.push_back(Live{i, jobs[i].in_off * 8 + jobs[i].start_bit, 0, 0});
    int rc;
    for (uint32_t round = 0; round < MAX_ROUNDS && !live.empty(); round++) {
        const uint32_t nj = (uint32_t)live.size();
        std::vector<BlkJob> bj(nj);
        for (uint32_t k = 0; k < nj; k++) {
            const InflateJob &j = jobs[live[k].stream];
            bj[k] = BlkJob{live[k].bit, (j.in_off + j.in_len) * 8};
        }
        if ((rc = c->d_dec_streams.reserve(sizeof(BlkJob) * nj))) return rc;
        if ((rc = c->d_dec_state.reserve(sizeof(BlkInfo) * nj))) return rc;
        if ((rc = c->d_dec_cand.reserve(sizeof(BlkLanes) * (size_t)nj))) return rc;
        if ((rc = c->d_dec_tabs.reserve(blk_tabs_bytes() * nj))) return rc;
        HIP_TRY(hipMemcpyAsync(c->d_dec_streams.p, bj.data(), sizeof(BlkJob) * nj, hipMemcpyHostToDevice, st));
        uint64_t range_bits = 0;
        for (uint32_t k = 0; k < nj; k++) range_bits += bj[k].end_bit - bj[k].start_bit;
        const bool small = !c->diag.no_small_scan && range_bits / nj < (512ull << 10);
        LAUNCH_TRY(launch_blk_scan(st, d_in, n_in, (const BlkJob *)c->d_dec_streams.p, nj, (BlkInfo *)c->d_dec_state.p,
                                   (BlkLanes *)c->d_dec_cand.p, c->d_dec_tabs.p, small));
        const bool stamp = c->n_ev + 6 < 17;
        if (stamp) c->phase("blk_scan");
        std::vector<BlkInfo> bi(nj);
        HIP_TRY(hipMemcpyAsync(bi.data(), c->d_dec_state.p, sizeof(BlkInfo) * nj, hipMemcpyDeviceToHost, st));
        HIP_TRY(hipStreamSynchronize(st));
        std::vector<BlkEmit> emit;
        std::vector<uint32_t> owner;
        uint64_t total_codes = 0;
        for (uint32_t k = 0; k < nj; k++) {
            const InflateJob &j = jobs[live[k].stream];
            const BlkInfo &r = bi[k];
            if (r.status != BLK_OK || r.end_bit <= live[k].bit || r.end_bit > (j.in_off + j.in_len) * 8 ||
                live[k].produced + r.n_out > j.out_cap)
                continue;
            BlkEmit e{};
            e.start_bit = live[k].bit; e.data_bit = r.data_bit; e.code_off = total_codes;
            e.out_off = j.out_off + live[k].produced;
            e.n_out = r.n_out; e.n_codes = r.n_codes; e.nlanes = r.nlanes; e.btype = r.btype; e.cand = k;
            e.hist = live[k].produced;
            e.preload = live[k].produced != 0;
            emit.push_back(e);
            owner.push_back(k);
            total_codes += r.n_codes;
        }
        const uint32_t ne = (uint32_t)emit.size();
        std::vector<uint32_t> jf(ne, 0);
        if (ne) {
            if ((rc = c->d_dec_tmp.reserve(sizeof(BlkEmit) * ne + 4ull * ne + 128))) return rc;
            if ((rc = c->d_hist.reserve(sizeof(BlkUnits) * (size_t)ne + 64))) return rc;
            if ((rc = c->d_codes.reserve(4 * std::max<uint64_t>(total_codes, 1)))) return rc;
            uint32_t *d_flags = (uint32_t *)c->d_dec_tmp.p;
            uint32_t *d_jf = d_flags + 16;
            BlkEmit *d_emit = (BlkEmit *)((uint8_t *)c->d_dec_tmp.p + 64 + 4ull * ne + (8 - (4ull * ne) % 8) % 8);
            HIP_TRY(hipMemsetAsync(d_flags, 0, 64 + 4ull * ne, st));
            HIP_TRY(hipMemcpyAsync(d_emit, emit.data(), sizeof(BlkEmit) * ne, hipMemcpyHostToDevice, st));
            const uint64_t slots = 4ull * (uint64_t)std::max(c->n_cu, 1);
            const uint32_t unit_target = (uint32_t)std::min<uint64_t>((total_codes + slots - 1) / slots + 1, 0x7FFFFFFFu);
            LAUNCH_TRY(launch_blk_emit(st, d_in, n_in, d_emit, ne, (const BlkLanes *)c->d_dec_cand.p, (uint32_t *)c->d_codes.p,
                                       d_flags, (BlkUnits *)c->d_hist.p, unit_target, d_jf, c->d_dec_tabs.p, 17, false, small));
            if (stamp) c->phase("blk_emit");
            LAUNCH_TRY(launch_blk_materialize(st, d_in, d_emit, ne, (const BlkLanes *)c->d_dec_cand.p,
                                              (const BlkUnits *)c->d_hist.p, (const uint32_t *)c->d_codes.p, d_out, nullptr));
            if (stamp) c->phase("lz77_copy");
            HIP_TRY(hipMemcpyAsync(jf.data(), d_jf, 4ull * ne, hipMemcpyDeviceToHost, st));
            HIP_TRY(hipStreamSynchronize(st));
        }
        if (c->idx && ne) {
            std::vector<BlkEmit> ok;
            for (uint32_t q = 0; q < ne; q++) if (!jf[q]) ok.push_back(emit[q]);
            if ((rc = idx_record_chain(c, ok.data(), (uint32_t)ok.size(), (const BlkLanes *)c->d_dec_cand.p, 0, 0, false))) return rc;
        }
        std::vector<Live> next;
        for (uint32_t q = 0; q < ne; q++) {
            if (jf[q]) continue;
            Live l = live[owner[q]];
            const BlkInfo &r = bi[owner[q]];
            l.produced += r.n_out;
            l.nblocks++;
            if (r.bfinal) {
                const InflateJob &j = jobs[l.stream];
                InflateResult &o = res[l.stream];
                o.end_bit = r.end_bit - j.in_off * 8;
                o.out_len = l.produced;
                o.blk_out_start = l.produced;
                o.final_seen = 1;
                o.nblocks = l.nblocks;
                fast[l.stream] = 1;
            } else { l.bit = r.end_bit; next.push_back(l); }
        }
        if (c->diag.debug) {
            uint32_t bad = 0, nfl = 0;
            for (uint32_t k = 0; k < nj; k++) bad += bi[k].status != BLK_OK;
            for (uint32_t q = 0; q < ne; q++) nfl += jf[q];
            fprintf(stderr, "[lfx] batch round %u: jobs=%u scan-not-ok=%u emitted=%u cross-block=%u continuing=%zu\n", round, nj, bad,
                    ne, nfl, next.size());
        }
        live.swap(next);
    }
    return LFX_OK;
}
}

namespace {
int decode_batch(Ctx *c, int format, uint32_t count, const void *d_in, const uint64_t *in_off, const uint64_t *in_len,
                 void *d_out, const uint64_t *out_off, const uint64_t *out_cap, std::vector<InflateResult> &res,
                 std::vector<uint64_t> *used = nullptr) {
    hipStream_t st = c->stream;
    std::vector<DecStream> streams(count);
    for (uint32_t i = 0; i < count; i++) streams[i] = DecStream{in_off[i], in_len[i], out_off[i], out_cap[i]};
    int rc;
    const size_t sz_streams = sizeof(DecStream) * count, sz_hdr = sizeof(DecHeader) * count;
    if ((rc = c->d_dec_blocks.reserve(sz_streams + sz_hdr + 16ull * count + 64))) return rc;
    DecStream *d_streams = (DecStream *)c->d_dec_blocks.p;
    DecHeader *d_hdrs = (DecHeader *)((uint8_t *)c->d_dec_blocks.p + sz_streams);
    uint32_t *d_crc = (uint32_t *)((uint8_t *)d_hdrs + sz_hdr);
    uint32_t *d_adler = d_crc + count;
    uint64_t *d_consumed = (uint64_t *)(d_adler + count);
    HIP_TRY(hipMemcpyAsync(d_streams, streams.data(), sz_streams, hipMemcpyHostToDevice, st));
    LAUNCH_TRY(launch_container(st, format, count, (const uint8_t *)d_in, d_streams, d_hdrs));
    std::vector<DecHeader> hdrs(count);
    if (format != LFX_DEFLATE) {
        HIP_TRY(hipMemcpyAsync(hdrs.data(), d_hdrs, sz_hdr, hipMemcpyDeviceToHost, st));
        HIP_TRY(hipStreamSynchronize(st));
    } else {
        HIP_TRY(hipMemsetAsync(d_hdrs, 0, sz_hdr, st));
    }
    c->phase("headers");
    std::vector<InflateJob> jobs(count);
    for (uint32_t i = 0; i < count; i++) {
        if (c->idx && (format == LFX_DEFLATE || hdrs[i].status == 0)) {
            const uint64_t b = (in_off[i] + (format == LFX_DEFLATE ? 0 : hdrs[i].deflate_off)) * 8;
            c->idx->cand.push_back(IdxCand{b, b, out_off[i], IDX_BTYPE_READ});
        }
        InflateJob j{};
        j.in_off = in_off[i];
        j.in_len = in_len[i];
        j.start_bit = (format == LFX_DEFLATE ? 0 : hdrs[i].deflate_off) * 8;
        if (format != LFX_DEFLATE && hdrs[i].status != 0) j.in_len = 0;
        j.out_off = out_off[i];
        j.out_cap = out_cap[i];
        j.flags = 0;
        jobs[i] = j;
    }
    uint64_t n_in = 0;
    for (uint32_t i = 0; i < count; i++) n_in = std::max(n_in, in_off[i] + in_len[i]);
    std::vector<uint8_t> fast;
    std::vector<InflateResult> fres;
    if (c->diag.batch_serial) { fast.assign(count, 0); fres.assign(count, InflateResult{}); }
    else if ((rc = batch_fast(c, (const uint8_t *)d_in, n_in, (uint8_t *)d_out, count, jobs, fast, fres))) return rc;
    c->phase("fast");
    std::vector<InflateJob> slow_jobs;
    std::vector<uint32_t> slow_idx;
    for (uint32_t i = 0; i < count; i++)
        if (!fast[i]) { slow_jobs.push_back(jobs[i]); slow_idx.push_back(i); }
    const uint32_t nslow = (uint32_t)slow_jobs.size();
    if ((rc = c->d_dec_streams.reserve(sizeof(InflateJob) * std::max<uint32_t>(nslow, 1)))) return rc;
    if ((rc = c->d_dec_state.reserve(sizeof(InflateResult) * ((size_t)count + nslow)))) return rc;
    InflateResult *d_res = (InflateResult *)c->d_dec_state.p, *d_slow = d_res + count;
    HIP_TRY(hipMemcpyAsync(d_res, fres.data(), sizeof(InflateResult) * count, hipMemcpyHostToDevice, st));
    if (nslow) {
        HIP_TRY(hipMemcpyAsync(c->d_dec_streams.p, slow_jobs.data(), sizeof(InflateJob) * nslow, hipMemcpyHostToDevice, st));
        LAUNCH_TRY(launch_inflate(st, (const uint8_t *)d_in, (uint8_t *)d_out, (const InflateJob *)c->d_dec_streams.p, d_slow, nslow));
        if (nslow == count) HIP_TRY(hipMemcpyAsync(d_res, d_slow, sizeof(InflateResult) * count, hipMemcpyDeviceToDevice, st));
        else for (uint32_t q = 0; q < nslow; q++)
            HIP_TRY(hipMemcpyAsync(d_res + slow_idx[q], d_slow + q, sizeof(InflateResult), hipMemcpyDeviceToDevice, st));
    }
    HIP_TRY(hipStreamSynchronize(st));
    c->phase("inflate");
    if (format != LFX_DEFLATE)
        LAUNCH_TRY(launch_checksum_ranges(st, (const uint8_t *)d_out, count, (const uint64_t *)d_streams + 2,
                                          sizeof(DecStream) / 8, (const uint64_t *)c->d_dec_state.p + 1,
                                          sizeof(InflateResult) / 8, d_crc, d_adler));
    LAUNCH_TRY(launch_verify_trailers(st, format, count, (const uint8_t *)d_in, d_streams, d_hdrs,
                                      (InflateResult *)c->d_dec_state.p, d_crc, d_adler, d_consumed));
    res.resize(count);
    HIP_TRY(hipMemcpyAsync(res.data(), c->d_dec_state.p, sizeof(InflateResult) * count, hipMemcpyDeviceToHost, st));
    if (used) {
        used->resize(count);
        HIP_TRY(hipMemcpyAsync(used->data(), d_consumed, 8ull * count, hipMemcpyDeviceToHost, st));
    }
    HIP_TRY(hipStreamSynchronize(st));
    c->phase("verify");
    return LFX_OK;
}
}

extern "C" int lfx_decode_batch_device(lfx_ctx *cc, int format, uint32_t count, const void *d_in,
                                       const uint64_t *in_off, const uint64_t *in_len, void *d_out,
                                       const uint64_t *out_off, const uint64_t *out_cap, uint64_t *out_len,
                                       int32_t *status) try {
    if (!cc) return LFX_E_DEVICE;
    Ctx *c = reinterpret_cast<Ctx *>(cc);
    std::lock_guard<std::recursive_mutex> lock(c->mu);
    (void)hipSetDevice(c->device);
    c->n_ev = 0;
    c->phase("start");
    if (!count) return LFX_OK;
    std::vector<InflateResult> res;
    int rc = decode_batch(c, format, count, d_in, in_off, in_len, d_out, out_off, out_cap, res);
    if (rc) return rc;
    int worst = LFX_OK;
    for (uint32_t i = 0; i < count; i++) {
        if (out_len) out_len[i] = res[i].out_len;
        const int s = map_status(res[i].status);
        if (status) status[i] = s;
        if (s != LFX_OK && worst == LFX_OK) { worst = s; c->set_error(format_error(res[i].err, res[i].a0, res[i].a1)); }
    }
    return LFX_OK;
} LFX_ABI_CATCH
// ... 738 lines not shown
```

libflate_amd/csrc/lfx_decode.h:

```cpp
#pragma once
#include <hip/hip_runtime.h>
#include <stdint.h>

#include "lfx_common.h"

namespace lfx {

enum : uint32_t {
    ERR_NONE = 0,
    ERR_EOF,
    ERR_HUFF,
    ERR_CONFLICT,
    ERR_HDIST,
    ERR_NO_PREV,
    ERR_DIST_LIST,
    ERR_286,
    ERR_BACKREF,
    ERR_BTYPE3,
    ERR_LEN_NLEN,
    ERR_STORED_SHORT,
    ERR_NOSPACE,
    ERR_ZLIB_CHECK, ERR_METHOD, ERR_CINFO, ERR_FDICT,
    ERR_GZIP_ID, ERR_HCRC,
    ERR_CRC32, ERR_ADLER32,
};

struct DecStream {
    uint64_t in_off, in_len;
    uint64_t out_off, out_cap;
};
struct DecHeader {
    uint64_t deflate_off;
    uint32_t status;
    uint32_t err, a0, a1;
    uint32_t flags;
    uint32_t _pad;
};

enum : uint32_t { JOB_SINGLE_BLOCK = 1, JOB_COUNT_ONLY = 2 };
struct InflateJob {
    uint64_t in_off;
    uint64_t in_len;
    uint64_t start_bit;
    uint64_t out_off, out_cap;
    uint64_t hist_avail;
    uint64_t stop_bit;
    uint32_t flags;
    uint32_t _pad;
};
struct InflateResult {
    uint64_t end_bit;
    uint64_t out_len;
    uint32_t status;
    uint32_t final_seen;
    uint32_t err, a0, a1;
    uint32_t needs_hist;
    uint32_t nblocks;
    uint32_t _pad;
    uint64_t blk_out_start;
    uint64_t blk_start_bit;
};

enum : uint32_t { BLK_OK = 0, BLK_BAD = 1, BLK_NO_EOB = 2 };
constexpr uint32_t BLK_PIECE_KNOWN = 2;
struct BlkJob {
    uint64_t start_bit;
    uint64_t end_bit;
    uint64_t lo_bit, warm_bit;
    uint32_t piece, _pad;
    uint64_t temp_off;
    uint32_t cap, _pad2;
};
struct BlkInfo {
    uint64_t end_bit;
    uint64_t n_out;
    uint64_t data_bit;
    uint32_t n_codes;
    uint32_t status, btype, bfinal, nlanes, rounds;
    uint32_t _pad;
    uint32_t cyc_hdr, cyc_total;
};
struct BlkLanes {
    uint64_t start[1024];
    uint64_t out_off[1024];
    uint32_t code_off[1024];
};
struct BlkLanesX {
    uint32_t n_head[1024];
    uint32_t n_rest[1024];
    uint32_t rest_at[1024];
    int32_t reach[1024];
    uint32_t cut_code[1024];
    uint32_t cut_out[1024];
};
struct BlkEmit {
    uint64_t start_bit, data_bit;
    uint64_t code_off;
    uint64_t out_off;
    uint64_t n_out;
    uint32_t n_codes, nlanes, btype, cand;
    uint64_t hist;
    uint64_t end_limit;
    uint32_t preload;
    uint32_t placed;
    uint64_t temp_off;
    uint32_t cap, _pad;
};
constexpr uint32_t MAX_FREE_UNITS = 64;
struct BlkUnits {
    uint32_t n;
    uint32_t code0[9];
    uint64_t out0[9];
    uint32_t cyc[4];
    uint32_t fn;
    uint32_t fcode0[MAX_FREE_UNITS + 1];
    uint64_t fout0[MAX_FREE_UNITS + 1];
};
struct SymUnit {
    uint64_t start;
    uint64_t len;
};
size_t blk_tabs_bytes();
int launch_blk_scan(hipStream_t st, const uint8_t *in, uint64_t nbytes, const BlkJob *jobs, uint32_t njobs,
                    BlkInfo *infos, BlkLanes *lanes, void *tabs = nullptr,
                    bool small_blocks = false);
int launch_blk_scan_store(hipStream_t st, const uint8_t *in, uint64_t nbytes, const BlkJob *jobs, uint32_t njobs,
                          BlkInfo *infos, BlkLanes *lanes, void *tabs, uint32_t *temp, BlkLanesX *lanesx);
int launch_blk_place(hipStream_t st, const BlkEmit *jobs, uint32_t njobs, const BlkLanes *lanes, const BlkLanesX *lanesx,
                     const uint32_t *temp, uint32_t *codes, uint32_t *flags, BlkUnits *units, uint32_t unit_target,
                     uint32_t *job_flags, uint32_t free_shift);
int launch_blk_emit(hipStream_t st, const uint8_t *in, uint64_t nbytes, const BlkEmit *jobs, uint32_t njobs,
                    const BlkLanes *lanes, uint32_t *codes, uint32_t *flags, BlkUnits *units, uint32_t unit_target,
                    uint32_t *job_flags = nullptr,
                    const void *tabs = nullptr,
                    uint32_t free_shift = 17,
                    bool large_blocks = false,
                    bool small_blocks = false);
int launch_blk_materialize(hipStream_t st, const uint8_t *in, const BlkEmit *jobs, uint32_t njobs,
                           const BlkLanes *lanes, const BlkUnits *units, const uint32_t *codes, uint8_t *out,
                           uint64_t *dbg);

int launch_blk_materialize_sym(hipStream_t st, const uint8_t *in, const BlkEmit *jobs, uint32_t njobs,
                               const BlkUnits *units, const uint32_t *codes, uint16_t *sym,
                               bool few_units = false );
int launch_window_chain(hipStream_t st, const uint16_t *sym, const SymUnit *units, uint32_t nunits, uint8_t *windows,
                        const uint8_t *init_win = nullptr);
size_t window_prefix_scratch_bytes(uint32_t nunits);
int launch_window_prefix(hipStream_t st, const uint16_t *sym, const SymUnit *units, uint32_t nunits, void *scratch,
                         uint8_t *windows, const uint8_t *init_win = nullptr);
int launch_window_rank_map(hipStream_t st, const uint16_t *sym, const SymUnit *units, uint32_t nunits, void *scratch, uint16_t *out_map);
int launch_bytes_to_map(hipStream_t st, const uint8_t *out, uint64_t len, uint16_t *map);
int launch_window_ranks(hipStream_t st, const uint16_t *maps, uint32_t nranks, uint8_t *win);
int launch_sym_substitute(hipStream_t st, const uint16_t *sym, const SymUnit *units, uint32_t nunits,
                          const uint8_t *windows, uint8_t *out, uint64_t max_len, const uint8_t *init_win = nullptr);

int launch_container(hipStream_t st, int format, uint32_t count, const uint8_t *in,
                     const DecStream *streams, DecHeader *hdrs);
int launch_inflate(hipStream_t st, const uint8_t *in, uint8_t *out, const InflateJob *jobs,
                   InflateResult *results, uint32_t njobs);
constexpr uint32_t FIND_SHARDS = 256;
constexpr uint32_t FIND_HDR_WORDS = 1024, FIND_HDR_FINAL = 320, FIND_HDR_DBG = 360, FIND_HDR_READ = 512 ;
constexpr uint32_t FIND2_GROUPS = 16, FIND_HDR_WORK = 512, FIND_HDR_WORK_STRIDE = 32;
inline uint32_t find_shard_cap(uint64_t comp_bytes) {
    const uint64_t want = comp_bytes / 4000;
    return (uint32_t)(want < 4096 ? 4096 : want > (1u << 23) ? (1u << 23) : want);
}
int launch_find_stage1(hipStream_t st, const uint8_t *in, uint64_t nbytes, uint64_t first_byte,
                       uint32_t *count, uint64_t *cand, uint32_t shard_cap, uint64_t final_from_bit, uint32_t n_cu);
int launch_find_stage2(hipStream_t st, const uint8_t *in, uint64_t nbytes, const uint64_t *cand,
                       uint32_t shard_cap, const uint32_t *count ,
                       uint32_t *work ,
                       uint32_t *final_count, uint64_t *final_list, uint32_t final_cap, uint32_t n_cu,
                       uint64_t *dbg = nullptr ,
                       int exp = 0 );
constexpr uint64_t MEMBER_TILE = 16384;
constexpr uint64_t MEMBER_SKIP = ~0ull;
inline uint64_t member_tiles(uint64_t n) { return (n + MEMBER_TILE - 1) / MEMBER_TILE; }
int launch_member_count(hipStream_t st, const uint8_t *in, uint64_t n, uint32_t *tile_count );
int launch_member_emit(hipStream_t st, const uint8_t *in, uint64_t n, const uint64_t *tile_pos ,
                       uint64_t *out, uint64_t cap);
int launch_verify_trailers(hipStream_t st, int format, uint32_t count, const uint8_t *in,
                           const DecStream *streams, const DecHeader *hdrs, InflateResult *results,
                           const uint32_t *crc, const uint32_t *adler, uint64_t *consumed);
}
```

libflate_amd/csrc/lfx_inflate_fast.hip:

```cpp
#include <hip/hip_runtime.h>
#include <stdint.h>
#include <stdlib.h>

#include <type_traits>

#include "lfx_common.h"
#include "lfx_decode.h"

namespace lfx {

__constant__ uint16_t f_len_base[29] = {3,  4,  5,  6,  7,  8,  9,  10, 11,  13,  15,  17,  19,  23, 27,
                                        31, 35, 43, 51, 59, 67, 83, 99, 115, 131, 163, 195, 227, 258};
__constant__ uint8_t f_len_extra[29] = {0, 0, 0, 0, 0, 0, 0, 0, 1, 1, 1, 1, 2, 2, 2,
                                        2, 3, 3, 3, 3, 4, 4, 4, 4, 5, 5, 5, 5, 0};
__constant__ uint16_t f_dist_base[30] = {1,    2,    3,    4,    5,    7,    9,    13,    17,    25,
                                         33,   49,   65,   97,   129,  193,  257,  385,   513,   769,
                                         1025, 1537, 2049, 3073, 4097, 6145, 8193, 12289, 16385, 24577};
__constant__ uint8_t f_dist_extra[30] = {0, 0, 0, 0, 1, 1, 2, 2,  3,  3,  4,  4,  5,  5,  6,
                                         6, 7, 7, 8, 8, 9, 9, 10, 10, 11, 11, 12, 12, 13, 13};
__constant__ uint8_t f_clen_order[19] = {16, 17, 18, 0, 8, 7, 9, 6, 10, 5, 11, 4, 12, 3, 13, 2, 14, 1, 15};
constexpr uint32_t f_clen_order_c(uint32_t k) {
    constexpr uint8_t o[19] = {16, 17, 18, 0, 8, 7, 9, 6, 10, 5, 11, 4, 12, 3, 13, 2, 14, 1, 15};
    return o[k];
}
// ... 820 lines not shown
    uint32_t rest_flag = 0;
    bool have_cp = false;
    uint32_t *my_temp = nullptr;
    uint32_t lane_cap = 0, ovf = 0;
    if constexpr (STORE) {
        lane_cap = job.cap;
        my_temp = temp + job.temp_off + (uint64_t)tid * lane_cap;
    }
    struct Seg { uint32_t n; uint64_t no; int64_t reach; uint32_t cc, co; };
    Seg A{0, 0, INT64_MAX, 0, 0}, B{0, 0, INT64_MAX, 0, 0};
    bool b_split = false;
    auto seg = [&](uint64_t from, uint64_t to, Seg &g, uint64_t &at, uint32_t *dst, uint32_t room) -> int {
        g = Seg{0, 0, INT64_MAX, 0, 0};
        if constexpr (STORE)
            return lane_decode<true>(T, in, nbytes, from, to, g.n, g.no, dst, g.reach, at, g.cc, g.co, s_ring + tid * RING_STRIDE,
                                     scan_stage + tid * EMIT_STRIDE, room, &ovf);
        else {
            int64_t dummy = 0;
            return lane_decode_fifo<false>(T, in, nbytes, from, to, g.n, g.no, nullptr, dummy, at, g.cc, g.co);
        }
    };
    for (;;) {
        const uint64_t st = s_start[tid];
        if (tid < nl && st != ~0ull) {
            if (st != decoded_from) {
                const uint64_t lim = tid + 1 == nl ? (piece ? e : e + 64) : my_bound;
                const bool retry = have_cp && st < cp_pos;
                uint64_t at = st, from = st, to = retry ? cp_pos : (st + CP_BITS < lim ? st + CP_BITS : lim);
                uint32_t *dst = my_temp;
                uint32_t room = lane_cap < SCAN_HEADCAP ? lane_cap : SCAN_HEADCAP;
                int r = 0;
                bool reuse = false, cache_b = false;
                if (!retry) have_cp = false;
                for (int pass = 0; pass < 2; ++pass) {
                    Seg G;
                    uint64_t ex = from;
                    const int rr = seg(from, to, G, ex, dst, room);
                    if (pass == 0) {
                        A = G; r = rr; at = ex;
                        if (retry) {
                            reuse = r == 0 && at == cp_pos;
                            if (reuse) break;
                            have_cp = false;
                        }
                        B = Seg{0, 0, INT64_MAX, 0, 0};
                        b_split = false;
                        if (!(r == 0 && at < lim)) break;
                        cache_b = !retry;
                        from = at; to = lim;
                        dst = my_temp + (cache_b ? SCAN_HEADCAP : A.n);
                        room = cache_b ? (lane_cap > SCAN_HEADCAP ? lane_cap - SCAN_HEADCAP : 0u) : (lane_cap > A.n ? lane_cap - A.n : 0u);
                    } else {
                        B = G;
                        if (cache_b) {
                            have_cp = true; cp_pos = at; b_split = true; reuse = true;
                            rest_exit = ex;
                            rest_flag = rr == 1 ? 1 : rr == 2 ? 2 : 0;
                        } else { r = rr; at = ex; }
                    }
                }
                if (reuse) { exitpos = rest_exit; flag = rest_flag; }
                else { exitpos = at; flag = r == 1 ? 1 : r == 2 ? 2 : 0; }
                nc = A.n + B.n;
                no = A.no + B.no;
                decoded_from = st;
            }
        } else flag = 4;
        s_flag[tid] = flag; s_exit[tid] = exitpos;
        __syncthreads();
        bool changed = false;
        if (tid + 1 < nl && flag == 0 && s_start[tid + 1] != exitpos) { s_start[tid + 1] = exitpos; changed = true; }
        rounds++;
        const int any = __syncthreads_or(changed ? 1 : 0);
        if (!any || rounds >= 64) break;
    }
    __shared__ uint32_t s_eob;
    if (tid == 0) s_eob = 0xFFFFFFFFu;
    __syncthreads();
    if (tid < nl && s_flag[tid] != 0) atomicMin(&s_eob, tid);
    __syncthreads();
    uint32_t eobl = s_eob;
    bi.rounds = rounds;
    if (rounds >= 64) { bi.status = BLK_BAD; if (tid == 0) infos[blockIdx.x] = bi; return; }
    if (eobl == 0xFFFFFFFFu) {
        bi.status = BLK_NO_EOB;
        if (!piece || nl == 0) { if (tid == 0) infos[blockIdx.x] = bi; return; }
        eobl = nl - 1;
    } else if (s_flag[eobl] != 1) { bi.status = BLK_BAD; if (tid == 0) infos[blockIdx.x] = bi; return; }
    const uint32_t mync = tid <= eobl ? nc : 0;
    const uint64_t myno = tid <= eobl ? no : 0;
    const uint32_t lane = tid & 63, wave = tid >> 6;
    uint32_t x = mync;
    uint64_t y = myno;
    for (int o = 1; o < 64; o <<= 1) {
        const uint32_t a = __shfl_up(x, o);
        const uint64_t c = __shfl_up(y, o);
        if ((int)lane >= o) { x += a; y += c; }
    }
    if (lane == 63) { s_scan[wave] = x; s_scan64[wave] = y; }
    __syncthreads();
    uint32_t px = 0;
    uint64_t py = 0;
    for (uint32_t w = 0; w < wave; ++w) { px += s_scan[w]; py += s_scan64[w]; }
    BlkLanes *L = &lanes[blockIdx.x];
    L->start[tid] = tid <= eobl ? s_start[tid] : ~0ull;
    L->code_off[tid] = px + x - mync;
    L->out_off[tid] = py + y - myno;
    if constexpr (STORE) {
        BlkLanesX *X = &lanesx[blockIdx.x];
        const bool live = tid <= eobl;
        const int64_t rb = B.reach == INT64_MAX ? INT64_MAX : (int64_t)A.no + B.reach;
        const int64_t reach = A.reach < rb ? A.reach : rb;
        const bool a_stands = rb >= (int64_t)A.co;
        uint32_t cc = a_stands ? A.cc : A.n + B.cc, co = a_stands ? A.co : (uint32_t)A.no + B.co;
        if (cc >= A.n + B.n) cc = 0xFFFFFFFFu;
        X->n_head[tid] = live ? A.n : 0u;
        X->n_rest[tid] = live ? B.n : 0u;
        X->rest_at[tid] = b_split ? SCAN_HEADCAP : A.n;
        X->reach[tid] = live && reach != INT64_MAX ? (reach < INT32_MIN ? INT32_MIN : (int32_t)reach) : INT32_MAX;
        X->cut_code[tid] = live ? cc : 0xFFFFFFFFu;
        X->cut_out[tid] = co;
        if (live && ovf) atomicOr(&hdr[7], 1u);
    }
    if (tid == NT - 1) {
        bi.n_codes = px + x;
        bi.n_out = py + y;
    }
    __shared__ uint32_t s_tot;
    __shared__ uint64_t s_tot64;
    if (tid == NT - 1) { s_tot = px + x; s_tot64 = py + y; }
    __syncthreads();
    if (tid == 0) {
        if constexpr (STORE) bi._pad = hdr[7] & 1u;
        bi.n_codes = s_tot; bi.n_out = s_tot64; bi.end_bit = s_exit[eobl]; bi.nlanes = eobl + 1; bi.rounds = rounds;
        bi.cyc_hdr = (uint32_t)(t_hdr - t_begin); bi.cyc_total = (uint32_t)(clock64() - t_begin);
        infos[blockIdx.x] = bi;
    }
}

constexpr uint32_t MAX_UNITS = 8;

template <int NT = SCAN_THREADS>
__device__ __forceinline__ void blk_units_tail(const uint32_t tid, const BlkEmit &job, const BlkLanes *L, const int64_t reach,
                                               uint32_t cut_code, const uint64_t cut_pos, BlkUnits *U, const uint32_t unit_target,
                                               const uint32_t free_shift, const uint64_t t_begin, const uint64_t t_hdr) {
    const uint64_t t_dec = clock64();
    __shared__ int64_t s_wmin[NT / 64];
    const uint32_t lane = tid & 63, wave = tid >> 6;
    int64_t sfx = reach;
    for (int o = 1; o < 64; o <<= 1) {
        const int64_t y = __shfl_down(sfx, o);
        if (lane + o < 64 && y < sfx) sfx = y;
    }
    if (lane == 0) s_wmin[wave] = sfx;
    __syncthreads();
    int64_t later = __shfl_down(sfx, 1);
    if (lane == 63) later = INT64_MAX;
    for (uint32_t w = wave + 1; w < NT / 64; ++w) { const int64_t y = s_wmin[w]; if (y < later) later = y; }
    if (cut_code != 0xFFFFFFFFu && later < (int64_t)cut_pos) cut_code = 0xFFFFFFFFu;
    __shared__ uint32_t s_cut_code[NT];
    __shared__ uint64_t s_cut_pos[NT];
    s_cut_code[tid] = cut_code;
    s_cut_pos[tid] = cut_pos;
    __shared__ uint64_t s_legal[NT / 64];
    const uint64_t legal = __ballot(cut_code != 0xFFFFFFFFu);
    if (lane == 0) s_legal[wave] = legal;
    __syncthreads();
    const uint64_t t_cut = clock64();
    if (tid == 0) {
        uint32_t nu = 0, last = 0;
        uint32_t want_units = (job.n_codes + unit_target / 2) / unit_target;
        if (want_units < 1) want_units = 1;
        if (want_units > MAX_UNITS) want_units = MAX_UNITS;
        const uint32_t tol = job.n_codes / (2 * want_units);
        U->code0[0] = 0; U->out0[0] = 0;
        for (uint32_t b = 1; b < want_units; ++b) {
            const uint32_t ideal = (uint32_t)((uint64_t)job.n_codes * b / want_units);
            uint32_t l0 = (uint32_t)((uint64_t)job.nlanes * b / want_units);
            if (l0 >= NT) l0 = NT - 1;
            int up = -1, dn = -1;
            for (uint32_t w = l0 >> 6; w < NT / 64 && up < 0; ++w) {
                uint64_t m = s_legal[w];
                if (w == (l0 >> 6)) m &= ~0ull << (l0 & 63);
                if (m) up = (int)(w * 64 + (uint32_t)__builtin_ctzll(m));
            }
            for (int w = (int)(l0 >> 6); w >= 0 && dn < 0; --w) {
                uint64_t m = s_legal[w];
                if (w == (int)(l0 >> 6)) m &= (l0 & 63) ? ~0ull >> (64 - (l0 & 63)) : 0ull;
                if (m) dn = w * 64 + 63 - __builtin_clzll(m);
            }
            int pick = -1;
            uint32_t best = 0xFFFFFFFFu;
            if (up >= 0) { const uint32_t cc = s_cut_code[up]; const uint32_t d = cc > ideal ? cc - ideal : ideal - cc; if (d < best) { best = d; pick = up; } }
            if (dn >= 0) { const uint32_t cc = s_cut_code[dn]; const uint32_t d = cc > ideal ? cc - ideal : ideal - cc; if (d < best) { best = d; pick = dn; } }
            if (pick < 0 || best > tol) continue;
            const uint32_t cc = s_cut_code[pick];
            if (cc == 0 || cc <= last || cc >= job.n_codes) continue;
            nu++;
            U->code0[nu] = cc; U->out0[nu] = s_cut_pos[pick];
            last = cc;
        }
        nu++;
        U->code0[nu] = job.n_codes; U->out0[nu] = job.n_out;
        U->n = nu;
        uint32_t fn = 0;
        uint32_t fwant = (uint32_t)(job.n_out >> free_shift);
        fwant = fwant < 1 ? 1 : fwant > MAX_FREE_UNITS ? MAX_FREE_UNITS : fwant;
        U->fcode0[0] = 0; U->fout0[0] = 0;
        for (uint32_t b = 1; b < fwant; ++b) {
            const uint32_t l = (uint32_t)((uint64_t)job.nlanes * b / fwant);
            if (l == 0 || l >= job.nlanes) continue;
            const uint32_t cc = L->code_off[l];
            if (cc <= U->fcode0[fn] || cc >= job.n_codes) continue;
            fn++;
            U->fcode0[fn] = cc; U->fout0[fn] = L->out_off[l];
        }
        fn++;
        U->fcode0[fn] = job.n_codes; U->fout0[fn] = job.n_out;
        U->fn = fn;
        U->cyc[0] = (uint32_t)(t_hdr - t_begin); U->cyc[1] = (uint32_t)(t_dec - t_hdr);
        U->cyc[2] = (uint32_t)(t_cut - t_dec); U->cyc[3] = (uint32_t)(clock64() - t_cut);
    }
}

__device__ __forceinline__ void blk_flag_reach(uint32_t tid, int64_t reach, uint64_t hist, uint32_t *__restrict__ flags,
                                               uint32_t *__restrict__ job_flags) {
    __shared__ uint32_t s_fl;
    if (tid == 0) s_fl = 0;
    __syncthreads();
    if (reach < -(int64_t)hist) atomicOr(&s_fl, 1u);
    else if (reach < 0) atomicOr(&s_fl, 2u);
    __syncthreads();
    if (tid == 0 && s_fl) {
        const uint32_t f = s_fl;
        if ((f & 1u) && job_flags) job_flags[blockIdx.x] = 1u;
        if ((__atomic_load_n(&flags[0], __ATOMIC_RELAXED) & f) != f) atomicOr(&flags[0], f);
    }
}

template <bool RING, int NT = SCAN_THREADS>
__global__ __launch_bounds__(NT, RING ? 4 : 8) void blk_emit_kernel(const uint8_t *__restrict__ in, uint64_t nbytes,
                                                                const BlkEmit *__restrict__ jobs,
                                                                const BlkLanes *__restrict__ lanes,
                                                                uint32_t *__restrict__ codes,
                                                                uint32_t *__restrict__ flags,
                                                                BlkUnits *__restrict__ units, uint32_t unit_target, uint32_t free_shift,
                                                                uint32_t *__restrict__ job_flags,
                                                                const FastTabs *__restrict__ tabs) {
    __shared__ FastTabs T;
    __shared__ __attribute__((aligned(4))) uint8_t lens[640];
    __shared__ uint32_t hdr[8];
    __shared__ uint64_t hdr64[2];
    extern __shared__ uint32_t emit_stage[];
    __shared__ uint32_t s_ring[RING ? NT * RING_STRIDE : 1];
    const uint32_t tid = threadIdx.x;
    const BlkEmit job = jobs[blockIdx.x];
    BlkUnits *U = &units[blockIdx.x];
    if (job.placed) return;
    if (job.btype == 0) {
        if (tid == 0) {
            U->n = 1; U->code0[0] = 0; U->code0[1] = 0; U->out0[0] = 0; U->out0[1] = job.n_out;
            U->fn = 1; U->fcode0[0] = 0; U->fcode0[1] = 0; U->fout0[0] = 0; U->fout0[1] = job.n_out;
        }
        return;
    }
    const uint64_t t_begin = clock64();
    if (tabs) {
        const uint32_t *srcw = (const uint32_t *)&tabs[job.cand];
        uint32_t *dst = (uint32_t *)&T;
        constexpr uint32_t TW = sizeof(FastTabs) / 4, TPER = (TW + NT - 1) / NT;
        uint32_t tv[TPER];
#pragma unroll
        for (uint32_t k = 0; k < TPER; ++k) tv[k] = srcw[min(tid + k * NT, TW - 1)];
#pragma unroll
        for (uint32_t k = 0; k < TPER; ++k) if (tid + k * NT < TW) dst[tid + k * NT] = tv[k];
        __syncthreads();
    } else parse_header<NT>(in, nbytes, job.start_bit, T, lens, hdr, hdr64, tid);
    const uint64_t t_hdr = clock64();
    const BlkLanes *L = &lanes[job.cand];
    int64_t reach = INT64_MAX;
    uint32_t cut_code = 0xFFFFFFFFu;
    uint64_t cut_pos = 0;
    if (tid < job.nlanes) {
        const uint64_t st = L->start[tid];
        const uint64_t lim = tid + 1 < job.nlanes ? L->start[tid + 1] : (job.end_limit ? job.end_limit : ~0ull >> 1);
        uint32_t nc = 0, cc = 0, co = 0;
        const uint64_t out0 = L->out_off[tid];
        uint64_t no = out0, endpos;
        if (RING)
            lane_decode<true>(T, in, nbytes, st, lim, nc, no, codes + job.code_off + L->code_off[tid], reach, endpos, cc, co,
                              s_ring + tid * RING_STRIDE, emit_stage + tid * EMIT_STRIDE);
        else
            lane_decode_fifo<true>(T, in, nbytes, st, lim, nc, no, codes + job.code_off + L->code_off[tid], reach, endpos, cc, co,
                                   emit_stage + tid * EMIT_STRIDE);
        if (cc < nc) { cut_code = L->code_off[tid] + cc; cut_pos = out0 + co; }
    }
    blk_flag_reach(tid, reach, job.hist, flags, job_flags);
    blk_units_tail<NT>(tid, job, L, reach, cut_code, cut_pos, U, unit_target, free_shift, t_begin, t_hdr);
}



__global__ __launch_bounds__(SCAN_THREADS) void blk_place_kernel(const BlkEmit *__restrict__ jobs, const BlkLanes *__restrict__ lanes,
                                                                  const BlkLanesX *__restrict__ lanesx, const uint32_t *__restrict__ temp,
                                                                  uint32_t *__restrict__ codes, uint32_t *__restrict__ flags,
                                                                  BlkUnits *__restrict__ units, uint32_t unit_target, uint32_t free_shift,
                                                                  uint32_t *__restrict__ job_flags) {
    const uint32_t tid = threadIdx.x, lane = tid & 63;
    const BlkEmit job = jobs[blockIdx.x];
    if (!job.placed) return;
    const uint64_t t_begin = clock64();
    BlkUnits *U = &units[blockIdx.x];
    const BlkLanes *L = &lanes[job.cand];
    const BlkLanesX *X = &lanesx[job.cand];
    const bool live = tid < job.nlanes;
    const uint32_t my_head = live ? X->n_head[tid] : 0u, my_rest = live ? X->n_rest[tid] : 0u, my_at = X->rest_at[tid];
    const uint32_t my_off = L->code_off[tid];
    const uint32_t *src0 = temp + job.temp_off + (uint64_t)(tid & ~63u) * job.cap;
    uint32_t *dst0 = codes + job.code_off;
    constexpr uint32_t DEEP = 8;
    const uint32_t j0 = blockIdx.y * 32u;
    for (uint32_t j = j0; j < j0 + 32u; j += 2) {
        uint32_t nh[2], n[2], at[2];
        const uint32_t *src[2];
        uint32_t *dst[2];
#pragma unroll
        for (uint32_t q = 0; q < 2; ++q) {
            nh[q] = (uint32_t)__shfl((int)my_head, (int)(j + q));
            n[q] = nh[q] + (uint32_t)__shfl((int)my_rest, (int)(j + q));
            at[q] = (uint32_t)__shfl((int)my_at, (int)(j + q));
            src[q] = src0 + (uint64_t)(j + q) * job.cap;
            dst[q] = dst0 + (uint32_t)__shfl((int)my_off, (int)(j + q));
        }
        const uint32_t nmax = n[0] > n[1] ? n[0] : n[1];
        for (uint32_t base = 0; base < nmax; base += 64 * DEEP) {
            uint32_t v[2][DEEP];
#pragma unroll
            for (uint32_t q = 0; q < 2; ++q)
#pragma unroll
                for (uint32_t k = 0; k < DEEP; ++k) {
                    const uint32_t i = base + k * 64 + lane;
                    const uint32_t si = i < nh[q] ? i : at[q] + (i - nh[q]);
                    v[q][k] = i < n[q] ? src[q][si] : 0u;
                }
#pragma unroll
            for (uint32_t q = 0; q < 2; ++q)
#pragma unroll
                for (uint32_t k = 0; k < DEEP; ++k) {
                    const uint32_t i = base + k * 64 + lane;
                    if (i < n[q]) dst[q][i] = v[q][k];
                }
        }
    }
    if (blockIdx.y != 0) return;
    const uint64_t t_hdr = clock64();
    int64_t reach = INT64_MAX;
    uint32_t cut_code = 0xFFFFFFFFu;
    uint64_t cut_pos = 0;
    if (live) {
        const uint64_t out0 = L->out_off[tid];
        const int32_t rr = X->reach[tid];
        if (rr != INT32_MAX) reach = (int64_t)out0 + (int64_t)rr;
        const uint32_t cc = X->cut_code[tid];
        if (cc != 0xFFFFFFFFu) { cut_code = my_off + cc; cut_pos = out0 + X->cut_out[tid]; }
    }
    blk_flag_reach(tid, reach, job.hist, flags, job_flags);
    blk_units_tail(tid, job, L, reach, cut_code, cut_pos, U, unit_target, free_shift, t_begin, t_hdr);
}

template <uint32_t THREADS>
struct M2 {
    static constexpr uint32_t WAVES = THREADS / 64;
    static constexpr uint32_t NC = 2 * THREADS;
    static constexpr uint32_t TILE = 4 * THREADS;
    static constexpr uint32_t RING = 32768 + TILE;
    static constexpr uint32_t PASSES = (TILE + 4 * THREADS - 1) / (4 * THREADS);
    static_assert(RING % 4 == 0 && TILE >= 258 && TILE < 0xFFFFu && RING + 64 < 65536, "tile");
};
constexpr uint32_t M2_THREADS = 256;
constexpr uint32_t M2_WIDE_THREADS = 1024;
constexpr uint32_t M2_FEW_JOBS = 4;
constexpr uint32_t M2_SYM_THREADS = 256;
constexpr uint32_t M2_DONE = 0xFFFFu;
#ifndef LFX_M2_PRIO_TILES
#define LFX_M2_PRIO_TILES 8
#endif
constexpr uint32_t M2_PRIO_TILES = LFX_M2_PRIO_TILES;

template <uint32_t RING> __device__ __forceinline__ uint32_t m2_wrap(uint32_t x) { return min(x, x - RING); }
template <uint32_t RING> __device__ __forceinline__ uint32_t m2_back(uint32_t idx, uint32_t d) {
    const uint32_t a = idx - d;
    return min(a, a + RING);
}

template <bool SYM, uint32_t THREADS>
struct M2Lds {
    using elem_t = typename std::conditional<SYM, uint16_t, uint8_t>::type;
    using G = M2<THREADS>;
    static constexpr uint32_t RING_BYTES = ((G::RING + 64) * (uint32_t)sizeof(elem_t) + 15u) & ~15u;
    static constexpr uint32_t P_BYTES = G::PASSES * 4 * THREADS * 2;
    static constexpr uint32_t XC_BYTES = (G::NC + 4) * 8;
    static constexpr uint32_t SW_BYTES = 2 * G::WAVES * 4;
    static constexpr uint32_t BYTES = RING_BYTES + P_BYTES + XC_BYTES + SW_BYTES;
};
template <bool SYM, uint32_t THREADS, bool DYN = false>
__device__ __forceinline__ void materialize2_body(const uint8_t *__restrict__ in, const BlkEmit *__restrict__ jobs,
                                                  const BlkUnits *__restrict__ units,
                                                  const uint32_t *__restrict__ codes,
                                                  typename std::conditional<SYM, uint16_t, uint8_t>::type *__restrict__ out,
                                                  uint32_t njobs, uint64_t *__restrict__ dbg) {
    using elem_t = typename std::conditional<SYM, uint16_t, uint8_t>::type;
    using G = M2<THREADS>;
    using LD = M2Lds<SYM, THREADS>;
    constexpr uint32_t WAVES = G::WAVES, TILE = G::TILE, RING = G::RING, PASSES = G::PASSES, NC = G::NC;
    constexpr uint32_t EPD = 4 / sizeof(elem_t);
    elem_t *ring;
    uint16_t *P;
    uint2 *XC;
    uint32_t *s_w;
    if constexpr (DYN) {
        extern __shared__ __attribute__((aligned(16))) uint8_t m2_dyn[];
        ring = (elem_t *)m2_dyn;
        P = (uint16_t *)(m2_dyn + LD::RING_BYTES);
        XC = (uint2 *)(m2_dyn + LD::RING_BYTES + LD::P_BYTES);
        s_w = (uint32_t *)(m2_dyn + LD::RING_BYTES + LD::P_BYTES + LD::XC_BYTES);
    } else {
        __shared__ __attribute__((aligned(16))) elem_t ring_s[RING + 64];
        __shared__ __attribute__((aligned(8))) uint16_t P_s[PASSES * 4 * THREADS];
        __shared__ __attribute__((aligned(16))) uint2 XC_s[G::NC + 4];
        __shared__ uint32_t s_w_s[2 * WAVES];
        ring = ring_s; P = P_s; XC = XC_s; s_w = s_w_s;
    }
    const uint32_t bidx = blockIdx.x % njobs, u = blockIdx.x / njobs;
    const BlkEmit job = jobs[bidx];
    const uint32_t tid = threadIdx.x, lane = tid & 63, wave = tid >> 6;
    if (job.btype == 0) {
        if (u != 0) return;
        elem_t *o = out + job.out_off;
        const uint8_t *src = in + (job.data_bit >> 3);
        for (uint64_t k = tid; k < job.n_out; k += THREADS) o[k] = src[k];
        return;
    }
    const BlkUnits *U = &units[bidx];
    if (u >= (SYM ? U->fn : U->n)) return;
    const uint32_t c0 = SYM ? U->fcode0[u] : U->code0[u], c1 = SYM ? U->fcode0[u + 1] : U->code0[u + 1];
    const uint64_t ob = SYM ? U->fout0[u] : U->out0[u];
    const uint64_t gbase = job.out_off + ob;
    elem_t *o = out + gbase;
    const uint32_t *cp = codes + job.code_off + c0;
    const uint32_t n = c1 - c0;
    const uint32_t hist = SYM ? 32768u : (u == 0 && job.preload) ? (uint32_t)(job.hist < 32768 ? job.hist : 32768) : 0;
    const uint32_t shift = (uint32_t)((gbase - hist) & (EPD - 1)) + hist;
    for (uint32_t k = tid; k < hist; k += THREADS)
        ring[shift - hist + k] = SYM ? (elem_t)(256 + k) : (elem_t)o[(int64_t)k - (int64_t)hist];
    if (tid < 4) XC[NC + tid] = make_uint2(0xFFFFFFFFu, 0u);
    uint64_t produced = 0, flushed = 0;
    uint32_t tr = shift;
    uint32_t fr = shift;
    uint32_t base = 0, ntiles = 0, nrounds = 0;
    uint32_t cw0 = 2 * tid < n ? cp[2 * tid] : 0u, cw1 = 2 * tid + 1 < n ? cp[2 * tid + 1] : 0u;
    const uint64_t t0 = dbg ? clock64() : 0;
    while (base < n) {
        if ((ntiles & (M2_PRIO_TILES - 1)) == 0) {
            switch (((ntiles / M2_PRIO_TILES) + u) & 3u) {
            case 0: __builtin_amdgcn_s_setprio(0); break;
            case 1: __builtin_amdgcn_s_setprio(1); break;
            case 2: __builtin_amdgcn_s_setprio(2); break;
            default: __builtin_amdgcn_s_setprio(3); break;
            }
        }
        ntiles++;
        const uint32_t i = base + 2 * tid;
        const uint32_t len0 = i < n ? ((cw0 & 0xFFFFu) ? cw0 >> 16 : 1u) : 0u;
        const uint32_t len1 = i + 1 < n ? ((cw1 & 0xFFFFu) ? cw1 >> 16 : 1u) : 0u;
        uint32_t x = wave_inclusive_sum(len0 + len1);
        if (lane == 63) s_w[wave] = x;
        __syncthreads();
        uint32_t tot = 0, cum[WAVES];
#pragma unroll
        for (uint32_t j = 0; j < WAVES; ++j) {
            const uint32_t wj = s_w[j];
            x += j < wave ? wj : 0u;
            tot += wj;
            cum[j] = tot;
        }
        *(uint4 *)&XC[2 * tid] = make_uint4(x - len1, cw0, x, cw1);
        if (tot > TILE) {
            const uint32_t cnt = (uint32_t)__popcll(__ballot(x - len1 <= TILE)) + (uint32_t)__popcll(__ballot(x <= TILE));
            if (lane == 0) s_w[WAVES + wave] = cnt;
        }
        __syncthreads();
        uint32_t take = NC, total = tot;
        if (tot > TILE) {
            take = 0;
#pragma unroll
            for (uint32_t j = 0; j < WAVES; ++j) take += s_w[WAVES + j];
            total = XC[take - 1].x;
        }
        const uint32_t j0 = 2 * tid + take, j1 = j0 + 1;
        const uint32_t rf0 = (j0 >= NC && base + j0 < n) ? cp[base + j0] : 0u;
        const uint32_t rf1 = (j1 >= NC && base + j1 < n) ? cp[base + j1] : 0u;
        uint32_t pp[PASSES][4];
        bool pend = false;
        auto round0 = [&](auto periodic_tag) {
        constexpr bool PERIODIC = decltype(periodic_tag)::value;
#pragma unroll
        for (uint32_t ps = 0; ps < PASSES; ++ps) {
            const uint32_t b = ps * 4 * THREADS + 4 * tid;
#pragma unroll
            for (uint32_t q = 0; q < 4; ++q) pp[ps][q] = M2_DONE;
            if (ps == 0 || __ballot(b < total)) {
                uint32_t k = 0;
#pragma unroll
                for (uint32_t j = 0; j + 1 < WAVES; ++j) k += cum[j] <= b ? 128u : 0u;
#pragma unroll
                for (uint32_t step = 64; step; step >>= 1) k += XC[k + step - 1].x <= b ? step : 0u;
                uint32_t src[4], dst[4], cwq[4];
                bool lit[4], fin[4];
#pragma unroll
                for (uint32_t q = 0; q < 4; ++q) {
                    const uint32_t bi = b + q;
                    if (q) k += bi >= cwq[q - 1] ? 1u : 0u;
                    const uint2 xc = XC[k];
                    const uint32_t d = xc.y & 0xFFFFu;
                    const uint32_t t = m2_wrap<RING>(tr + bi);
                    const bool in = bi < total;
                    lit[q] = d == 0;
                    uint32_t tgt = bi, tt = t;
                    if constexpr (PERIODIC) {
                        const uint32_t s0 = xc.x - (xc.y >> 16);
                        const uint32_t off = bi - s0;
                        if (d != 0 && off >= d) {
                            uint32_t r = off - d * (uint32_t)((float)off * __builtin_amdgcn_rcpf((float)d));
                            r = r >= d ? r - d : r;
                            tgt = s0 + r;
                            tt = m2_wrap<RING>(tr + tgt);
                        }
                    }
                    fin[q] = lit[q] || d > tgt;
                    src[q] = (d > tgt && in) ? m2_back<RING>(tt, d) : t;
                    dst[q] = in ? t : RING + (tid & 63u);
                    pp[ps][q] = (fin[q] || !in) ? M2_DONE : tgt - d;
                    cwq[q] = xc.x;
                    src[q] |= xc.y & 0xFFFF0000u;
                }
                uint32_t hv[4];
#pragma unroll
                for (uint32_t q = 0; q < 4; ++q) hv[q] = ring[src[q] & 0xFFFFu];
#pragma unroll
                for (uint32_t q = 0; q < 4; ++q) ring[dst[q]] = (elem_t)(lit[q] ? src[q] >> 16 : hv[q]);
                pend |= (pp[ps][0] & pp[ps][1] & pp[ps][2] & pp[ps][3]) != M2_DONE;
            }
            *(uint64_t *)&P[b] = (uint64_t)pp[ps][0] | (uint64_t)pp[ps][1] << 16 | (uint64_t)pp[ps][2] << 32 | (uint64_t)pp[ps][3] << 48;
        }
        };
        if (take * 8 < total) round0(std::true_type{}); else round0(std::false_type{});
        __syncthreads();
        while (__ballot(pend)) {
            nrounds++;
            if (pend) {
#pragma unroll
                for (uint32_t ps = 0; ps < PASSES; ++ps) {
                    const uint32_t b = ps * 4 * THREADS + 4 * tid;
                    if (ps && (pp[ps][0] & pp[ps][1] & pp[ps][2] & pp[ps][3]) == M2_DONE) continue;
                    uint32_t nx[4], hv[4], jj[4];
#pragma unroll
                    for (uint32_t q = 0; q < 4; ++q) {
                        jj[q] = pp[ps][q] != M2_DONE ? pp[ps][q] : b + q;
                        nx[q] = P[jj[q]];
                    }
                    asm volatile("" ::: "memory");
#pragma unroll
                    for (uint32_t q = 0; q < 4; ++q) hv[q] = ring[m2_wrap<RING>(tr + jj[q])];
#pragma unroll
                    for (uint32_t q = 0; q < 4; ++q) {
                        ring[m2_wrap<RING>(tr + b + q)] = (elem_t)hv[q];
                        pp[ps][q] = nx[q];
                    }
                    asm volatile("" ::: "memory");
                    *(uint64_t *)&P[b] = (uint64_t)nx[0] | (uint64_t)nx[1] << 16 | (uint64_t)nx[2] << 32 | (uint64_t)nx[3] << 48;
                }
                pend = false;
#pragma unroll
                for (uint32_t ps = 0; ps < PASSES; ++ps) pend |= (pp[ps][0] & pp[ps][1] & pp[ps][2] & pp[ps][3]) != M2_DONE;
            }
        }
        __syncthreads();
        const uint64_t upto = produced + total;
        base += take;
        const bool last = base >= n;
        if ((gbase + flushed) & (EPD - 1)) {
            uint32_t hb = EPD - (uint32_t)((gbase + flushed) & (EPD - 1));
            if (hb > upto - flushed) hb = (uint32_t)(upto - flushed);
            if (tid < hb) o[flushed + tid] = ring[m2_wrap<RING>(fr + tid)];
            flushed += hb;
            fr = m2_wrap<RING>(fr + hb);
        }
        const uint32_t ndw = (uint32_t)((upto - flushed) / EPD);
        uint32_t *o32 = (uint32_t *)(o + flushed);
        for (uint32_t k = tid; k < ndw; k += THREADS) o32[k] = *(const uint32_t *)&ring[m2_wrap<RING>(fr + EPD * k)];
        flushed += (uint64_t)EPD * ndw;
        fr = m2_wrap<RING>(fr + EPD * ndw);
        if (last) {
            const uint32_t rest = (uint32_t)(upto - flushed);
            if (tid < rest) o[flushed + tid] = ring[m2_wrap<RING>(fr + tid)];
            flushed = upto;
        }
        produced = upto;
        tr = m2_wrap<RING>(tr + total);
        cw0 = j0 < NC ? XC[j0].y : rf0;
        cw1 = j1 < NC ? XC[j1].y : rf1;
    }
    if (!SYM && dbg && tid == 0) {
        uint64_t *d = dbg + ((uint64_t)bidx * MAX_UNITS + u) * 8;
        d[0] = clock64() - t0; d[1] = ntiles; d[2] = nrounds; d[3] = 0; d[4] = n; d[5] = produced; d[6] = wall_clock64();
    }
}


template <uint32_t THREADS>
__global__ __launch_bounds__(THREADS) void blk_materialize2_kernel(const uint8_t *__restrict__ in,
                                                                   const BlkEmit *__restrict__ jobs,
                                                                   const BlkUnits *__restrict__ units,
                                                                   const uint32_t *__restrict__ codes,
                                                                   uint8_t *__restrict__ out, uint32_t njobs,
                                                                   uint64_t *__restrict__ dbg) {
    materialize2_body<false, THREADS>(in, jobs, units, codes, out, njobs, dbg);
}

__global__ __launch_bounds__(1024) void window_chain_kernel(const uint16_t *__restrict__ sym,
                                                            const SymUnit *__restrict__ units, uint32_t nunits,
                                                            uint8_t *__restrict__ windows, const uint8_t *__restrict__ init_win) {
    extern __shared__ uint8_t wbuf[];
    uint8_t *prev = wbuf, *cur = wbuf + 32768;
    for (uint32_t i = threadIdx.x; i < 32768; i += 1024) prev[i] = init_win ? init_win[i] : (uint8_t)0;
    uint32_t sn[16];
    auto fetch = [&](uint32_t u) {
        if (u >= nunits) return;
        const SymUnit su = units[u];
#pragma unroll
        for (uint32_t k = 0; k < 8; ++k) {
            const uint32_t i = 4 * (threadIdx.x + 1024 * k);
            const uint64_t at = su.start + su.len - 32768 + i;
            const uint32_t s0 = sym[su.len + i >= 32768 ? at : 0];
            const uint32_t s1 = sym[su.len + i + 1 >= 32768 ? at + 1 : 0];
            const uint32_t s2 = sym[su.len + i + 2 >= 32768 ? at + 2 : 0];
            const uint32_t s3 = sym[su.len + i + 3 >= 32768 ? at + 3 : 0];
            sn[2 * k] = s0 | s1 << 16;
            sn[2 * k + 1] = s2 | s3 << 16;
        }
    };
    fetch(0);
    __syncthreads();
    for (uint32_t u = 0; u < nunits; ++u) {
        const uint64_t len = units[u].len;
        uint32_t sc[16];
#pragma unroll
        for (uint32_t k = 0; k < 16; ++k) sc[k] = sn[k];
        fetch(u + 1);
        uint32_t *wout = (uint32_t *)(windows + (uint64_t)u * 32768);
#pragma unroll
        for (uint32_t k = 0; k < 8; ++k) {
            const uint32_t i = 4 * (threadIdx.x + 1024 * k);
            uint32_t lb[4], sv[4];
            bool own[4];
#pragma unroll
            for (uint32_t q = 0; q < 4; ++q) {
                sv[q] = (sc[2 * k + (q >> 1)] >> (16 * (q & 1))) & 0xFFFFu;
                own[q] = len + i + q >= 32768;
                const uint32_t at = own[q] ? (sv[q] >= 256 ? sv[q] - 256 : 0u) : i + q + (uint32_t)len;
                lb[q] = prev[at];
            }
            uint32_t packed = 0;
#pragma unroll
            for (uint32_t q = 0; q < 4; ++q) packed |= ((own[q] && sv[q] < 256) ? sv[q] : lb[q]) << (8 * q);
            ((uint32_t *)cur)[i >> 2] = packed;
            wout[i >> 2] = packed;
        }
        __syncthreads();
        uint8_t *t = prev; prev = cur; cur = t;
    }
}

__host__ __device__ inline uint32_t wc_group(uint32_t nunits) {
    uint32_t g = 4;
    while (g * g < nunits && g < 64) ++g;
    return g;
}
__device__ __forceinline__ uint32_t unit_map_load(const uint16_t *__restrict__ sym, const SymUnit &su, uint32_t i) {
    return sym[su.len + i >= 32768 ? su.start + su.len - 32768 + i : 0];
}
__device__ __forceinline__ uint32_t unit_map_value(uint32_t loaded, const SymUnit &su, uint32_t i) {
    return su.len + i >= 32768 ? loaded : 256u + i + (uint32_t)su.len;
}
__global__ __launch_bounds__(1024) void window_compose_kernel(const uint16_t *__restrict__ sym,
                                                              const SymUnit *__restrict__ units, uint32_t nunits,
                                                              uint16_t *__restrict__ maps, uint32_t WC_GROUP) {
    extern __shared__ uint16_t mbuf[];
    uint16_t *prev = mbuf, *cur = mbuf + 32768;
    const uint32_t u0 = blockIdx.x * WC_GROUP, u1 = u0 + WC_GROUP < nunits ? u0 + WC_GROUP : nunits;
    if (u0 >= u1) return;
    uint32_t nx[16];
    auto load_unit = [&](const SymUnit &su) {
        if (su.len >= 32768) {
            const uint16_t *p = sym + (su.start + su.len - 32768) + threadIdx.x;
#pragma unroll
            for (uint32_t k = 0; k < 16; ++k) nx[k] = (uint32_t)p[1024 * (2 * k)] | (uint32_t)p[1024 * (2 * k + 1)] << 16;
        } else {
#pragma unroll
            for (uint32_t k = 0; k < 16; ++k)
                nx[k] = unit_map_load(sym, su, threadIdx.x + 1024 * (2 * k)) | unit_map_load(sym, su, threadIdx.x + 1024 * (2 * k + 1)) << 16;
        }
    };
    SymUnit sun = units[u0];
    load_unit(sun);
    for (uint32_t u = u0; u < u1; ++u) {
        const SymUnit su = sun;
        uint32_t sc[16];
#pragma unroll
        for (uint32_t k = 0; k < 16; ++k) sc[k] = nx[k];
        if (u + 1 < u1) {
            sun = units[u + 1];
            load_unit(sun);
        }
        uint16_t *mout = maps + (uint64_t)u * 32768;
        const bool first = u == u0;
#pragma unroll
        for (uint32_t h = 0; h < 4; ++h) {
            uint32_t sv[8], g[8];
#pragma unroll
            for (uint32_t j = 0; j < 8; ++j) {
                const uint32_t k = 8 * h + j;
                sv[j] = unit_map_value((sc[k >> 1] >> (16 * (k & 1))) & 0xFFFFu, su, threadIdx.x + 1024 * k);
                g[j] = prev[sv[j] >= 256 ? sv[j] - 256 : 0u];
            }
#pragma unroll
            for (uint32_t j = 0; j < 8; ++j) {
                const uint32_t k = 8 * h + j;
                const uint32_t v = (!first && sv[j] >= 256) ? g[j] : sv[j];
                cur[threadIdx.x + 1024 * k] = (uint16_t)v;
                mout[threadIdx.x + 1024 * k] = (uint16_t)v;
            }
        }
        __syncthreads();
        uint16_t *t = prev; prev = cur; cur = t;
    }
}
__device__ __forceinline__ void map_octet(const uint4 &q, uint32_t (&s8)[8]) {
    s8[0] = q.x & 0xFFFFu; s8[1] = q.x >> 16; s8[2] = q.y & 0xFFFFu; s8[3] = q.y >> 16;
    s8[4] = q.z & 0xFFFFu; s8[5] = q.z >> 16; s8[6] = q.w & 0xFFFFu; s8[7] = q.w >> 16;
}
__device__ __forceinline__ void window_step_bytes(const uint4 (&mq)[4], const uint8_t *prev, uint8_t *cur, uint8_t *gout) {
#pragma unroll
    for (uint32_t k = 0; k < 4; ++k) {
        const uint32_t o = threadIdx.x + 1024 * k;
        uint32_t s8[8], b8[8];
        map_octet(mq[k], s8);
#pragma unroll
        for (uint32_t j = 0; j < 8; ++j) b8[j] = prev[s8[j] >= 256 ? s8[j] - 256 : 0u];
        uint32_t lo = 0, hi = 0;
#pragma unroll
        for (uint32_t j = 0; j < 4; ++j) {
            lo |= ((s8[j] < 256 ? s8[j] : b8[j]) & 0xFFu) << (8 * j);
            hi |= ((s8[j + 4] < 256 ? s8[j + 4] : b8[j + 4]) & 0xFFu) << (8 * j);
        }
        *(uint2 *)(cur + 8 * o) = make_uint2(lo, hi);
        if (gout) *(uint2 *)(gout + 8 * o) = make_uint2(lo, hi);
    }
}
__global__ __launch_bounds__(1024) void window_groups_kernel(const uint16_t *__restrict__ maps, uint32_t nunits,
                                                             uint8_t *__restrict__ gwin, const uint8_t *__restrict__ init_win,
                                                             uint32_t WC_GROUP) {
    extern __shared__ __attribute__((aligned(16))) uint8_t wbuf[];
    uint8_t *prev = wbuf, *cur = wbuf + 32768;
    for (uint32_t i = threadIdx.x; i < 32768; i += 1024) prev[i] = init_win ? init_win[i] : (uint8_t)0;
    const uint32_t ngroups = (nunits + WC_GROUP - 1) / WC_GROUP;
    auto last_of = [&](uint32_t g) { return (g + 1) * WC_GROUP < nunits ? (g + 1) * WC_GROUP - 1 : nunits - 1; };
    uint4 nx[4];
    if (ngroups) {
        const uint4 *m = (const uint4 *)(maps + (uint64_t)last_of(0) * 32768);
#pragma unroll
        for (uint32_t k = 0; k < 4; ++k) nx[k] = m[threadIdx.x + 1024 * k];
    }
    __syncthreads();
    for (uint32_t g = 0; g < ngroups; ++g) {
        uint4 mq[4];
#pragma unroll
        for (uint32_t k = 0; k < 4; ++k) mq[k] = nx[k];
        if (g + 1 < ngroups) {
            const uint4 *m = (const uint4 *)(maps + (uint64_t)last_of(g + 1) * 32768);
#pragma unroll
            for (uint32_t k = 0; k < 4; ++k) nx[k] = m[threadIdx.x + 1024 * k];
        }
        window_step_bytes(mq, prev, cur, gwin + (uint64_t)g * 32768);
        __syncthreads();
        uint8_t *t = prev; prev = cur; cur = t;
    }
}
__global__ __launch_bounds__(1024) void window_apply_kernel(const uint16_t *__restrict__ maps, const uint8_t *__restrict__ gwin,
                                                            uint8_t *__restrict__ windows, const uint8_t *__restrict__ init_win,
                                                            uint32_t WC_GROUP) {
    __shared__ __attribute__((aligned(16))) uint8_t wl[32768];
    const uint32_t u = blockIdx.x, g = u / WC_GROUP;
    const uint8_t *w = g ? gwin + (uint64_t)(g - 1) * 32768 : init_win;
    const uint4 *m = (const uint4 *)(maps + (uint64_t)u * 32768);
    uint4 mq[4];
#pragma unroll
    for (uint32_t k = 0; k < 4; ++k) mq[k] = m[threadIdx.x + 1024 * k];
    {
        const uint4 z = make_uint4(0, 0, 0, 0);
        const uint4 *w16 = (const uint4 *)w;
        if (w && ((uint64_t)w & 15) == 0) {
            ((uint4 *)wl)[threadIdx.x] = w16[threadIdx.x];
            ((uint4 *)wl)[threadIdx.x + 1024] = w16[threadIdx.x + 1024];
        } else if (w) {
            for (uint32_t i = threadIdx.x; i < 32768; i += 1024) wl[i] = w[i];
        } else {
            ((uint4 *)wl)[threadIdx.x] = z;
            ((uint4 *)wl)[threadIdx.x + 1024] = z;
        }
    }
    __syncthreads();
    uint8_t *wout = windows + (uint64_t)u * 32768;
#pragma unroll
    for (uint32_t k = 0; k < 4; ++k) {
        const uint32_t o = threadIdx.x + 1024 * k;
        uint32_t s8[8], b8[8];
        map_octet(mq[k], s8);
#pragma unroll
        for (uint32_t j = 0; j < 8; ++j) b8[j] = wl[s8[j] >= 256 ? s8[j] - 256 : 0u];
        uint32_t lo = 0, hi = 0;
#pragma unroll
        for (uint32_t j = 0; j < 4; ++j) {
            lo |= ((s8[j] < 256 ? s8[j] : b8[j]) & 0xFFu) << (8 * j);
            hi |= ((s8[j + 4] < 256 ? s8[j + 4] : b8[j + 4]) & 0xFFu) << (8 * j);
        }
        *(uint2 *)(wout + 8 * o) = make_uint2(lo, hi);
    }
}

__global__ __launch_bounds__(1024) void window_rank_map_kernel(const uint16_t *__restrict__ maps, uint32_t nunits,
                                                               uint16_t *__restrict__ out_map, uint32_t WC_GROUP) {
    extern __shared__ __attribute__((aligned(16))) uint16_t mbuf2[];
    uint16_t *prev = mbuf2, *cur = mbuf2 + 32768;
    for (uint32_t i = threadIdx.x; i < 32768; i += 1024) prev[i] = (uint16_t)(256u + i);
    const uint32_t ngroups = (nunits + WC_GROUP - 1) / WC_GROUP;
    auto last_of = [&](uint32_t g) { return (g + 1) * WC_GROUP < nunits ? (g + 1) * WC_GROUP - 1 : nunits - 1; };
    uint4 nx[4];
    if (ngroups) {
        const uint4 *m = (const uint4 *)(maps + (uint64_t)last_of(0) * 32768);
#pragma unroll
        for (uint32_t k = 0; k < 4; ++k) nx[k] = m[threadIdx.x + 1024 * k];
    }
    __syncthreads();
    for (uint32_t g = 0; g < ngroups; ++g) {
        uint4 mq[4];
#pragma unroll
        for (uint32_t k = 0; k < 4; ++k) mq[k] = nx[k];
        if (g + 1 < ngroups) {
            const uint4 *m = (const uint4 *)(maps + (uint64_t)last_of(g + 1) * 32768);
#pragma unroll
            for (uint32_t k = 0; k < 4; ++k) nx[k] = m[threadIdx.x + 1024 * k];
        }
#pragma unroll
        for (uint32_t k = 0; k < 4; ++k) {
            const uint32_t o = threadIdx.x + 1024 * k;
            uint32_t s8[8], g8[8];
            map_octet(mq[k], s8);
#pragma unroll
            for (uint32_t j = 0; j < 8; ++j) g8[j] = prev[s8[j] >= 256 ? s8[j] - 256 : 0u];
#pragma unroll
            for (uint32_t j = 0; j < 8; ++j) s8[j] = s8[j] < 256 ? s8[j] : g8[j];
            *(uint4 *)(cur + 8 * o) = make_uint4(s8[0] | s8[1] << 16, s8[2] | s8[3] << 16, s8[4] | s8[5] << 16, s8[6] | s8[7] << 16);
        }
        __syncthreads();
        uint16_t *t = prev; prev = cur; cur = t;
    }
    for (uint32_t i = threadIdx.x; i < 32768; i += 1024) out_map[i] = prev[i];
}
__global__ __launch_bounds__(256) void bytes_to_map_kernel(const uint8_t *__restrict__ out, uint64_t len, uint16_t *__restrict__ map) {
    const uint32_t i = blockIdx.x * 256 + threadIdx.x;
    if (i >= 32768) return;
    map[i] = len + i >= 32768 ? (uint16_t)out[len + i - 32768] : (uint16_t)(256u + i + (uint32_t)len);
}
__global__ __launch_bounds__(1024) void window_ranks_kernel(const uint16_t *__restrict__ maps, uint32_t nranks, uint8_t *__restrict__ win) {
    extern __shared__ __attribute__((aligned(16))) uint8_t wbuf3[];
    uint8_t *prev = wbuf3, *cur = wbuf3 + 32768;
    for (uint32_t i = threadIdx.x; i < 32768; i += 1024) prev[i] = 0;
    uint4 nx[4];
    if (nranks) {
#pragma unroll
        for (uint32_t k = 0; k < 4; ++k) nx[k] = ((const uint4 *)maps)[threadIdx.x + 1024 * k];
    }
    __syncthreads();
    for (uint32_t r = 0; r < nranks; ++r) {
        uint4 mq[4];
#pragma unroll
        for (uint32_t k = 0; k < 4; ++k) mq[k] = nx[k];
        if (r + 1 < nranks) {
            const uint4 *m = (const uint4 *)(maps + (uint64_t)(r + 1) * 32768);
#pragma unroll
            for (uint32_t k = 0; k < 4; ++k) nx[k] = m[threadIdx.x + 1024 * k];
        }
        window_step_bytes(mq, prev, cur, nullptr);
        __syncthreads();
        uint8_t *t = prev; prev = cur; cur = t;
    }
    for (uint32_t i = threadIdx.x; i < 32768; i += 1024) win[i] = prev[i];
}

__global__ __launch_bounds__(256) void sym_substitute_kernel(const uint16_t *__restrict__ sym,
                                                             const SymUnit *__restrict__ units,
                                                             const uint8_t *__restrict__ windows,
                                                             uint8_t *__restrict__ out, const uint8_t *__restrict__ init_win) {
    const uint32_t u = blockIdx.x;
    const SymUnit su = units[u];
    const uint8_t *w = u ? windows + (uint64_t)(u - 1) * 32768 : (init_win ? init_win : windows);
    const uint64_t lo = (uint64_t)blockIdx.y * 16384, hi = lo + 16384 < su.len ? lo + 16384 : su.len;
    if (lo >= hi) return;
    const uint64_t A = su.start + lo, B = su.start + hi;
    const bool out_aligned = ((uint64_t)out & 7) == 0;
    for (uint64_t p = (A & ~7ull) + 8ull * threadIdx.x; p < B; p += 8ull * 256) {
        const uint4 q = *(const uint4 *)(sym + p);
        const uint32_t s8[8] = {q.x & 0xFFFFu, q.x >> 16, q.y & 0xFFFFu, q.y >> 16, q.z & 0xFFFFu, q.z >> 16, q.w & 0xFFFFu, q.w >> 16};
        uint32_t b8[8];
#pragma unroll
        for (uint32_t j = 0; j < 8; ++j) b8[j] = w[s8[j] >= 256 ? min(s8[j] - 256, 32767u) : 0];
        uint64_t v = 0;
#pragma unroll
        for (uint32_t j = 0; j < 8; ++j) v |= (uint64_t)((s8[j] < 256 ? s8[j] : b8[j]) & 0xFFu) << (8 * j);
// ... 1 lines not shown
        else {
#pragma unroll
            for (uint32_t j = 0; j < 8; ++j) if (p + j >= A && p + j < B) out[p + j] = (uint8_t)(v >> (8 * j));
        }
    }
}

__device__ __forceinline__ void clen_table_build(uint8_t *tab, uint32_t lane, uint64_t clw) {
    uint64_t cnt = 0;
    for (uint32_t s = 0; s < 19; ++s) { const uint32_t w = (uint32_t)(clw >> (3 * s)) & 7; if (w) cnt += 1ull << (5 * w); }
    uint64_t next = 0;
    uint32_t code = 0;
    for (uint32_t w = 1; w <= 7; ++w) {
        code <<= 1;
        next |= (uint64_t)code << (8 * w);
        code += (uint32_t)(cnt >> (5 * w)) & 31;
    }
    for (uint32_t s = 0; s < 19; ++s) {
        const uint32_t w = (uint32_t)(clw >> (3 * s)) & 7;
        const uint32_t c = (uint32_t)(next >> (8 * w)) & 255;
        next += w ? 1ull << (8 * w) : 0ull;
        const uint32_t r = __brev(c) >> (32 - w);
        if (w) tab[r * 64 + lane] = (uint8_t)(s | w << 5);
    }
#pragma unroll
    for (uint32_t k = 0; k < 7; ++k) {
#pragma unroll
        for (uint32_t i0 = 0; i0 < (1u << k); i0 += 16) {
            uint8_t e[16];
#pragma unroll
            for (uint32_t j = 0; j < 16; ++j)
                if (i0 + j < (1u << k)) e[j] = tab[(i0 + j) * 64 + lane];
#pragma unroll
            for (uint32_t j = 0; j < 16; ++j)
                if (i0 + j < (1u << k) && (uint32_t)(e[j] >> 5) <= k) tab[(i0 + j + (1u << k)) * 64 + lane] = e[j];
        }
    }
}

#ifndef LFX_FIND2_HB
#define LFX_FIND2_HB 16
#endif
constexpr uint32_t FIND2_HB = LFX_FIND2_HB;
template <int EXP>
__device__ __forceinline__ bool stage2_check_staged(const uint8_t *__restrict__ in, uint64_t nbytes, uint64_t cand_bit, bool valid,
                                                    uint8_t *cl_tab, uint32_t *hbuf, uint64_t *dbg, uint32_t *work, uint32_t &next_raw) {
    const uint32_t lane = threadIdx.x;
    const uint64_t t0 = dbg ? clock64() : 0;
    const uint64_t a = (uint64_t)in;
    const uint64_t abs0 = cand_bit + (a & 3) * 8;
    gptr_u32 w = (gptr_u32)(a & ~3ull);
    uint64_t gd = abs0 >> 5;
    const uint32_t off = (uint32_t)abs0 & 31;
    const uint64_t wlast = ((a & 3) + nbytes + 3) / 4 - 1;
    auto stage = [&](bool need) {
        uint32_t v[FIND2_HB];
#pragma unroll
        for (uint32_t k = 0; k < FIND2_HB; ++k) { const uint64_t idx = gd + k; v[k] = need ? w[idx < wlast ? idx : wlast] : 0u; }
#pragma unroll
        for (uint32_t k = 0; k < FIND2_HB; ++k)
            if (need) hbuf[k * 64 + lane] = v[k];
    };
    stage(valid && EXP < 3);
    const uint32_t e0 = hbuf[lane], e1 = hbuf[64 + lane], e2 = hbuf[128 + lane], e3 = hbuf[192 + lane];
    const uint32_t x0 = __builtin_amdgcn_alignbit(e1, e0, off), x1 = __builtin_amdgcn_alignbit(e2, e1, off),
                   x2 = __builtin_amdgcn_alignbit(e3, e2, off);
    const uint32_t nl = ((x0 >> 3) & 31) + 257, nd = ((x0 >> 8) & 31) + 1, nc = ((x0 >> 13) & 15) + 4;
    const uint32_t f0 = __builtin_amdgcn_alignbit(x1, x0, 17), f1 = __builtin_amdgcn_alignbit(x2, x1, 17);
    uint64_t clw = 0;
#pragma unroll
    for (uint32_t k = 0; k < 19; ++k) {
        const uint32_t fw = 3 * k + 3 <= 32 ? f0 >> (3 * k) : 3 * k >= 32 ? f1 >> (3 * k - 32) : __builtin_amdgcn_alignbit(f1, f0, 3 * k);
        clw |= (uint64_t)(k < nc ? fw & 7u : 0u) << (3 * f_clen_order_c(k));
    }
    const uint64_t t1 = dbg ? clock64() : 0;
    if (EXP < 2) clen_table_build(cl_tab, lane, clw);
    {
        uint32_t zero;
        asm volatile("v_mov_b32 %0, 0" : "=v"(zero));
        if (lane == 0 && EXP < 4) next_raw = atomicAdd(work + zero, 1u);
    }
    const uint64_t t2 = dbg ? clock64() : 0;
    uint32_t steps = 0, restaged = 0;
    uint32_t have = 0, kl = 0, kd = 0, nlit = 0, ndist = 0, eob_len = 0, last = 0;
    const uint32_t total = nl + nd;
    bool good = valid;
    const uint32_t bp = off + 17 + 3 * nc;
    uint32_t di = (bp >> 5) + 2;
    uint32_t cur = hbuf[(bp >> 5) * 64 + lane], nxt = hbuf[((bp >> 5) + 1) * 64 + lane];
    uint32_t o = bp & 31;
#if !defined(LFX_FIND2_NO_LEAN)
    {
        uint32_t acc = 0;
        last = 31u;
        if (EXP >= 1) good = false;
        bool runA = good;
        uint32_t badv = 0;
        while (__ballot(runA)) {
            if (__ballot(runA && di >= FIND2_HB)) {
                ++restaged;
                gd += di;
                di = runA ? 0u : di;
                gd -= di;
                stage(runA);
            }
            do {
                ++steps;
                const uint32_t win = __builtin_amdgcn_alignbit(nxt, cur, o);
                const uint32_t e = cl_tab[(win & 127) * 64 + lane];
                const uint32_t ahead = hbuf[min(di, FIND2_HB - 1) * 64 + lane];
                const uint32_t sym = e & 31, used = e >> 5;
                const uint32_t k4 = (sym > 15 ? sym - 15 : 0) * 4;
                const uint32_t nbx = (0x7320u >> k4) & 15, basex = (0xB331u >> k4) & 15;
                uint32_t rep = basex + __builtin_amdgcn_ubfe(win, used, nbx);
                const uint32_t val = sym < 16 ? sym : (sym == 16 ? last : 0);
                const bool take = runA && have + rep < nl;
                rep = take ? rep : 0u;
                const uint32_t adv = take ? used + nbx : 0u;
                o += adv;
                const bool pass = o >= 32;
                cur = pass ? nxt : cur;
                nxt = pass ? ahead : nxt;
                di += pass ? 1u : 0u;
                o &= 31u;
                const uint32_t w9 = val ? (0x1000000u >> val) | 1u : 0u;
                acc += __umul24(rep, w9);
                eob_len = (256u - have) < rep ? val : eob_len;
                have += rep;
                last = take ? val : last;
                const bool bad = val == 31u || acc > (32768u << 9 | 511u);
                badv = take && bad ? 1u : badv;
                runA = take && !bad;
            } while (__ballot(runA) && !__ballot(runA && di >= FIND2_HB));
        }
        good = good && badv == 0;
        kl = acc >> 9;
        nlit = acc & 511u;
        last = last == 31u ? 0u : last;
    }
#endif
    bool run = good && have < total;
    while (__ballot(run)) {
        ++steps;
        if (__ballot(run && di >= FIND2_HB)) {
            ++restaged;
            gd += di;
            di = run ? 0u : di;
            gd -= di;
            stage(run);
        }
        const uint32_t win = __builtin_amdgcn_alignbit(nxt, cur, o);
        const uint32_t e = cl_tab[(win & 127) * 64 + lane];
        const uint32_t ahead = hbuf[min(di, FIND2_HB - 1) * 64 + lane];
        const uint32_t sym = e & 31, used = e >> 5;
        const uint32_t k4 = (sym > 15 ? sym - 15 : 0) * 4;
        const uint32_t nbx = (0x7320u >> k4) & 15, basex = (0xB331u >> k4) & 15;
        uint32_t rep = basex + __builtin_amdgcn_ubfe(win, used, nbx);
        uint32_t val = sym < 16 ? sym : (sym == 16 ? last : 0);
        uint32_t adv = used + nbx;
        bool bad = run && ((sym == 16 && have == 0) || have + rep > total);
        rep = run ? rep : 0u;
        val = run ? val : 0u;
        adv = run ? adv : 0u;
        o += adv;
        const bool pass = o >= 32;
        cur = pass ? nxt : cur;
        nxt = pass ? ahead : nxt;
        di += pass ? 1u : 0u;
        o &= 31u;
        const uint32_t nlit_part = have < nl ? min(rep, nl - have) : 0u;
        const uint32_t ndist_part = rep - nlit_part;
        const uint32_t wgt = val ? 32768u >> val : 0u;
        kl += __umul24(nlit_part, wgt);
        kd += __umul24(ndist_part, wgt);
        nlit += val ? nlit_part : 0u;
        ndist += val ? ndist_part : 0u;
        eob_len = (val && have <= 256 && 256 < have + rep) ? val : eob_len;
        bad |= kl > 32768u || kd > 32768u;
        bad |= have + rep >= nl && have < nl && !(kl == 32768u || (nlit == 1 && kl == 16384u));
        have += rep;
        last = val;
        good = good && !bad;
        run = good && have < total;
    }
    if (good) {
        if (eob_len == 0) good = false;
        if (!(kl == 32768u || (nlit == 1 && kl == 16384u))) good = false;
        if (!(kd == 32768u || (ndist == 1 && kd == 16384u) || ndist == 0)) good = false;
        if (((gd + di - 2) << 5) + o > nbytes * 8 + (a & 3) * 8) good = false;
    }
    if (dbg && lane == 0) {
        const uint64_t t3 = clock64();
        atomicAdd((unsigned long long *)&dbg[0], (unsigned long long)(t1 - t0));
        atomicAdd((unsigned long long *)&dbg[1], (unsigned long long)(t2 - t1));
        atomicAdd((unsigned long long *)&dbg[2], (unsigned long long)(t3 - t2));
        atomicAdd((unsigned long long *)&dbg[3], (unsigned long long)steps);
        atomicAdd((unsigned long long *)&dbg[4], (unsigned long long)restaged);
        atomicAdd((unsigned long long *)&dbg[5], 1ull);
    }
    return good;
}

template <int EXP>
__global__ __launch_bounds__(64) void find_blocks_stage2(const uint8_t *__restrict__ in, uint64_t nbytes,
                                                         const uint64_t *__restrict__ cand, uint32_t shard_cap,
                                                         const uint32_t *__restrict__ count, uint32_t *__restrict__ work,
                                                         uint32_t *__restrict__ final_count,
                                                         uint64_t *__restrict__ final_list, uint32_t final_cap,
                                                         uint64_t *__restrict__ dbg) {
    __shared__ uint8_t cl_tab[128 * 64];
    __shared__ uint32_t hbuf[FIND2_HB * 64];
    const uint64_t tk0 = dbg ? clock64() : 0;
    __shared__ uint32_t s_pre[FIND_SHARDS + 1];
    {
        constexpr uint32_t PER = FIND_SHARDS / 64;
        static_assert(PER * 64 == FIND_SHARDS, "lists per lane");
        uint32_t cnt[PER], sum = 0;
#pragma unroll
        for (uint32_t q = 0; q < PER; ++q) { cnt[q] = min(count[threadIdx.x * PER + q], shard_cap); sum += cnt[q]; }
        const uint32_t incl = wave_inclusive_sum(sum);
        uint32_t at = incl - sum;
#pragma unroll
        for (uint32_t q = 0; q < PER; ++q) { s_pre[threadIdx.x * PER + q] = at; at += cnt[q]; }
        if (threadIdx.x == 63) s_pre[FIND_SHARDS] = incl;
    }
    __syncthreads();
    const uint32_t n1 = s_pre[FIND_SHARDS];
    const uint32_t grp = blockIdx.x % FIND2_GROUPS, members = (gridDim.x - grp + FIND2_GROUPS - 1) / FIND2_GROUPS;
    uint32_t *my_work = work + grp * FIND_HDR_WORK_STRIDE;
    uint32_t base = (grp + FIND2_GROUPS * (blockIdx.x / FIND2_GROUPS)) * 64u;
    while (base < n1) {
        uint32_t next_raw = 0;
        const uint32_t gi = base + threadIdx.x;
        const bool valid = gi < n1;
        uint32_t shard = 0;
#pragma unroll
        for (uint32_t step = FIND_SHARDS / 2; step; step >>= 1) shard += s_pre[shard + step] <= gi ? step : 0u;
        const uint64_t i = (uint64_t)shard * shard_cap + (gi - s_pre[shard]);
        const uint64_t cand_bit = valid ? cand[i] : 0;
        const bool good = stage2_check_staged<EXP>(in, nbytes, cand_bit, valid, cl_tab, hbuf, dbg, my_work, next_raw);
        if (good) {
            const uint32_t slot = atomicAdd(final_count, 1u);
            if (slot < final_cap) final_list[slot] = cand_bit;
        }
        __syncthreads();
        if (EXP == 4) base += gridDim.x * 64u;
        else base = (grp + FIND2_GROUPS * (members + (uint32_t)__builtin_amdgcn_readfirstlane((int)next_raw))) * 64u;
    }
    if (dbg && threadIdx.x == 0) atomicAdd((unsigned long long *)&dbg[6], (unsigned long long)(clock64() - tk0));
}

__global__ __launch_bounds__(M2_SYM_THREADS) void blk_materialize2_sym_kernel(const uint8_t *__restrict__ in,
                                                                          const BlkEmit *__restrict__ jobs,
                                                                          const BlkUnits *__restrict__ units,
                                                                          const uint32_t *__restrict__ codes,
                                                                          uint16_t *__restrict__ sym, uint32_t njobs) {
    materialize2_body<true, M2_SYM_THREADS>(in, jobs, units, codes, sym, njobs, nullptr);
}
__global__ __launch_bounds__(M2_WIDE_THREADS) void blk_materialize2_sym_wide_kernel(const uint8_t *__restrict__ in,
                                                                                const BlkEmit *__restrict__ jobs,
                                                                                const BlkUnits *__restrict__ units,
                                                                                const uint32_t *__restrict__ codes,
                                                                                uint16_t *__restrict__ sym, uint32_t njobs) {
    materialize2_body<true, M2_WIDE_THREADS, true>(in, jobs, units, codes, sym, njobs, nullptr);
}

#define LFX_LAUNCH_CHECK()                          \
    do {                                            \
        hipError_t e_ = hipGetLastError();          \
        if (e_ != hipSuccess) return (int)e_;       \
    } while (0)

size_t blk_tabs_bytes() { return sizeof(FastTabs); }
constexpr int SCAN_SMALL = 256;
int launch_blk_scan(hipStream_t st, const uint8_t *in, uint64_t nbytes, const BlkJob *jobs, uint32_t njobs,
                    BlkInfo *infos, BlkLanes *lanes, void *tabs, bool small_blocks) {
    if (!njobs) return 0;
    if (small_blocks)
        hipLaunchKernelGGL((blk_scan_kernel<false, SCAN_SMALL>), dim3(njobs), dim3(SCAN_SMALL), 0, st, in, nbytes, jobs, infos, lanes,
                           (FastTabs *)tabs, (uint32_t *)nullptr, (BlkLanesX *)nullptr);
    else
        hipLaunchKernelGGL((blk_scan_kernel<false, SCAN_THREADS>), dim3(njobs), dim3(SCAN_THREADS), 0, st, in, nbytes, jobs, infos, lanes,
                           (FastTabs *)tabs, (uint32_t *)nullptr, (BlkLanesX *)nullptr);
    LFX_LAUNCH_CHECK();
    return 0;
}
int launch_blk_scan_store(hipStream_t st, const uint8_t *in, uint64_t nbytes, const BlkJob *jobs, uint32_t njobs,
                          BlkInfo *infos, BlkLanes *lanes, void *tabs, uint32_t *temp, BlkLanesX *lanesx) {
    if (!njobs) return 0;
    constexpr size_t stage_bytes = (size_t)SCAN_THREADS * EMIT_STRIDE * 4;
    static bool attr_set[64] = {};
    int dev_ = 0;
    (void)hipGetDevice(&dev_);
    if (!attr_set[dev_ & 63]) {
        (void)hipFuncSetAttribute((const void *)blk_scan_kernel<true, SCAN_THREADS>, hipFuncAttributeMaxDynamicSharedMemorySize, (int)stage_bytes);
        attr_set[dev_ & 63] = true;
    }
    hipLaunchKernelGGL((blk_scan_kernel<true, SCAN_THREADS>), dim3(njobs), dim3(SCAN_THREADS), stage_bytes, st, in, nbytes, jobs, infos, lanes,
                       (FastTabs *)tabs, temp, lanesx);
    LFX_LAUNCH_CHECK();
    return 0;
}
int launch_blk_place(hipStream_t st, const BlkEmit *jobs, uint32_t njobs, const BlkLanes *lanes, const BlkLanesX *lanesx,
                     const uint32_t *temp, uint32_t *codes, uint32_t *flags, BlkUnits *units, uint32_t unit_target, uint32_t *job_flags,
                     uint32_t free_shift) {
    if (!njobs) return 0;
    hipLaunchKernelGGL(blk_place_kernel, dim3(njobs, 2), dim3(SCAN_THREADS), 0, st, jobs, lanes, lanesx, temp, codes, flags, units,
                       unit_target ? unit_target : 1u, free_shift < 15 ? 15u : free_shift, job_flags);
    LFX_LAUNCH_CHECK();
    return 0;
}
int launch_blk_emit(hipStream_t st, const uint8_t *in, uint64_t nbytes, const BlkEmit *jobs, uint32_t njobs,
                    const BlkLanes *lanes, uint32_t *codes, uint32_t *flags, BlkUnits *units, uint32_t unit_target,
                    uint32_t *job_flags, const void *tabs, uint32_t free_shift, bool large_blocks, bool small_blocks) {
    if (!njobs) return 0;
    constexpr size_t stage_bytes = (size_t)SCAN_THREADS * EMIT_STRIDE * 4, stage_small = (size_t)SCAN_SMALL * EMIT_STRIDE * 4;
    static bool attr_set[64] = {};
    int dev_ = 0;
    (void)hipGetDevice(&dev_);
    if (!attr_set[dev_ & 63]) {
        (void)hipFuncSetAttribute((const void *)blk_emit_kernel<false, SCAN_THREADS>, hipFuncAttributeMaxDynamicSharedMemorySize, (int)stage_bytes);
        (void)hipFuncSetAttribute((const void *)blk_emit_kernel<true, SCAN_THREADS>, hipFuncAttributeMaxDynamicSharedMemorySize, (int)stage_bytes);
        attr_set[dev_ & 63] = true;
    }
    const uint32_t ut = unit_target ? unit_target : 1u, fs = free_shift < 15 ? 15u : free_shift;
    if (small_blocks)
        hipLaunchKernelGGL((blk_emit_kernel<false, SCAN_SMALL>), dim3(njobs), dim3(SCAN_SMALL), stage_small, st, in, nbytes, jobs, lanes, codes,
                           flags, units, ut, fs, job_flags, (const FastTabs *)tabs);
    else if (large_blocks)
        hipLaunchKernelGGL((blk_emit_kernel<true, SCAN_THREADS>), dim3(njobs), dim3(SCAN_THREADS), stage_bytes, st, in, nbytes, jobs, lanes,
                           codes, flags, units, ut, fs, job_flags, (const FastTabs *)tabs);
    else
        hipLaunchKernelGGL((blk_emit_kernel<false, SCAN_THREADS>), dim3(njobs), dim3(SCAN_THREADS), stage_bytes, st, in, nbytes, jobs, lanes, codes,
                           flags, units, ut, fs, job_flags, (const FastTabs *)tabs);
    LFX_LAUNCH_CHECK();
    return 0;
}
int launch_blk_materialize(hipStream_t st, const uint8_t *in, const BlkEmit *jobs, uint32_t njobs,
                           const BlkLanes *lanes, const BlkUnits *units, const uint32_t *codes, uint8_t *out,
                           uint64_t *dbg) {
    if (!njobs) return 0;
    if (njobs <= M2_FEW_JOBS)
        hipLaunchKernelGGL(blk_materialize2_kernel<M2_WIDE_THREADS>, dim3(njobs * MAX_UNITS), dim3(M2_WIDE_THREADS), 0, st, in, jobs, units, codes, out, njobs, dbg);
    else
        hipLaunchKernelGGL(blk_materialize2_kernel<M2_THREADS>, dim3(njobs * MAX_UNITS), dim3(M2_THREADS), 0, st, in, jobs, units, codes, out, njobs, dbg);
    LFX_LAUNCH_CHECK();
    return 0;
}
int launch_blk_materialize_sym(hipStream_t st, const uint8_t *in, const BlkEmit *jobs, uint32_t njobs,
                               const BlkUnits *units, const uint32_t *codes, uint16_t *sym, bool few_units) {
    if (!njobs) return 0;
    if (few_units) {
        constexpr int lds = (int)M2Lds<true, M2_WIDE_THREADS>::BYTES;
        static bool attr_set[64] = {};
        int dev_ = 0;
        (void)hipGetDevice(&dev_);
        if (!attr_set[dev_ & 63]) {
            (void)hipFuncSetAttribute((const void *)blk_materialize2_sym_wide_kernel, hipFuncAttributeMaxDynamicSharedMemorySize, lds);
            attr_set[dev_ & 63] = true;
        }
        hipLaunchKernelGGL(blk_materialize2_sym_wide_kernel, dim3(njobs * MAX_FREE_UNITS), dim3(M2_WIDE_THREADS), lds, st, in, jobs, units, codes, sym, njobs);
    } else
        hipLaunchKernelGGL(blk_materialize2_sym_kernel, dim3(njobs * MAX_FREE_UNITS), dim3(M2_SYM_THREADS), 0, st, in, jobs, units, codes, sym, njobs);
    LFX_LAUNCH_CHECK();
    return 0;
}
int launch_window_chain(hipStream_t st, const uint16_t *sym, const SymUnit *units, uint32_t nunits, uint8_t *windows,
                        const uint8_t *init_win) {
    if (!nunits) return 0;
    static bool attr_set[64] = {};
    int dev_ = 0;
    (void)hipGetDevice(&dev_);
    if (!attr_set[dev_ & 63]) {
        (void)hipFuncSetAttribute((const void *)window_chain_kernel, hipFuncAttributeMaxDynamicSharedMemorySize, 65536);
        attr_set[dev_ & 63] = true;
    }
    hipLaunchKernelGGL(window_chain_kernel, dim3(1), dim3(1024), 65536, st, sym, units, nunits, windows, init_win);
    LFX_LAUNCH_CHECK();
    return 0;
}
size_t window_prefix_scratch_bytes(uint32_t nunits) {
    const uint32_t g = wc_group(nunits);
    return (size_t)nunits * 65536 + (size_t)((nunits + g - 1) / g) * 32768;
}
int launch_window_prefix(hipStream_t st, const uint16_t *sym, const SymUnit *units, uint32_t nunits, void *scratch,
                         uint8_t *windows, const uint8_t *init_win) {
    if (!nunits) return 0;
    static bool attr_set[64] = {};
    int dev_ = 0;
    (void)hipGetDevice(&dev_);
    if (!attr_set[dev_ & 63]) {
        (void)hipFuncSetAttribute((const void *)window_compose_kernel, hipFuncAttributeMaxDynamicSharedMemorySize, 131072);
        (void)hipFuncSetAttribute((const void *)window_groups_kernel, hipFuncAttributeMaxDynamicSharedMemorySize, 65536);
        attr_set[dev_ & 63] = true;
    }
    uint16_t *maps = (uint16_t *)scratch;
    uint8_t *gwin = (uint8_t *)scratch + (size_t)nunits * 65536;
    const uint32_t G = wc_group(nunits);
    const uint32_t ngroups = (nunits + G - 1) / G;
    hipLaunchKernelGGL(window_compose_kernel, dim3(ngroups), dim3(1024), 131072, st, sym, units, nunits, maps, G);
    LFX_LAUNCH_CHECK();
    hipLaunchKernelGGL(window_groups_kernel, dim3(1), dim3(1024), 65536, st, maps, nunits, gwin, init_win, G);
    LFX_LAUNCH_CHECK();
    hipLaunchKernelGGL(window_apply_kernel, dim3(nunits), dim3(1024), 0, st, maps, gwin, windows, init_win, G);
    LFX_LAUNCH_CHECK();
    return 0;
}
int launch_window_rank_map(hipStream_t st, const uint16_t *sym, const SymUnit *units, uint32_t nunits, void *scratch, uint16_t *out_map) {
    static bool attr_set[64] = {};
    int dev_ = 0;
    (void)hipGetDevice(&dev_);
    if (!attr_set[dev_ & 63]) {
        (void)hipFuncSetAttribute((const void *)window_compose_kernel, hipFuncAttributeMaxDynamicSharedMemorySize, 131072);
        (void)hipFuncSetAttribute((const void *)window_rank_map_kernel, hipFuncAttributeMaxDynamicSharedMemorySize, 131072);
        attr_set[dev_ & 63] = true;
    }
    uint16_t *maps = (uint16_t *)scratch;
    const uint32_t G = wc_group(nunits);
    const uint32_t ngroups = (nunits + G - 1) / G;
    if (nunits) {
        hipLaunchKernelGGL(window_compose_kernel, dim3(ngroups), dim3(1024), 131072, st, sym, units, nunits, maps, G);
        LFX_LAUNCH_CHECK();
    }
    hipLaunchKernelGGL(window_rank_map_kernel, dim3(1), dim3(1024), 131072, st, maps, nunits, out_map, G);
    LFX_LAUNCH_CHECK();
    return 0;
}
int launch_bytes_to_map(hipStream_t st, const uint8_t *out, uint64_t len, uint16_t *map) {
    hipLaunchKernelGGL(bytes_to_map_kernel, dim3(128), dim3(256), 0, st, out, len, map);
    LFX_LAUNCH_CHECK();
    return 0;
}
int launch_window_ranks(hipStream_t st, const uint16_t *maps, uint32_t nranks, uint8_t *win) {
    static bool attr_set[64] = {};
    int dev_ = 0;
    (void)hipGetDevice(&dev_);
    if (!attr_set[dev_ & 63]) {
        (void)hipFuncSetAttribute((const void *)window_ranks_kernel, hipFuncAttributeMaxDynamicSharedMemorySize, 65536);
        attr_set[dev_ & 63] = true;
    }
    hipLaunchKernelGGL(window_ranks_kernel, dim3(1), dim3(1024), 65536, st, maps, nranks, win);
    LFX_LAUNCH_CHECK();
    return 0;
}
int launch_sym_substitute(hipStream_t st, const uint16_t *sym, const SymUnit *units, uint32_t nunits,
                          const uint8_t *windows, uint8_t *out, uint64_t max_len, const uint8_t *init_win) {
    if (!nunits) return 0;
    const uint32_t gy = (uint32_t)((max_len + 16383) / 16384);
    hipLaunchKernelGGL(sym_substitute_kernel, dim3(nunits, gy ? gy : 1), dim3(256), 0, st, sym, units, windows, out, init_win);
    LFX_LAUNCH_CHECK();
    return 0;
}
int launch_find_stage2(hipStream_t st, const uint8_t *in, uint64_t nbytes, const uint64_t *cand,
                       uint32_t shard_cap, const uint32_t *count, uint32_t *work, uint32_t *final_count, uint64_t *final_list,
                       uint32_t final_cap, uint32_t n_cu, uint64_t *dbg, int exp) {
    static int per_cu_dev[64] = {};
    int dev_ = 0;
    (void)hipGetDevice(&dev_);
    int &per_cu = per_cu_dev[dev_ & 63];
    if (per_cu == 0) {
        int nb = 0;
        if (hipOccupancyMaxActiveBlocksPerMultiprocessor(&nb, (const void *)find_blocks_stage2<0>, 64, 0) != hipSuccess || nb < 1) {
            (void)hipGetLastError();
            nb = 8;
        }
        per_cu = nb;
    }
    const dim3 grid((uint32_t)per_cu * (n_cu ? n_cu : 256u));
    if (exp == 1) hipLaunchKernelGGL(find_blocks_stage2<1>, grid, dim3(64), 0, st, in, nbytes, cand, shard_cap, count, work, final_count, final_list, final_cap, dbg);
    else if (exp == 2) hipLaunchKernelGGL(find_blocks_stage2<2>, grid, dim3(64), 0, st, in, nbytes, cand, shard_cap, count, work, final_count, final_list, final_cap, dbg);
    else if (exp == 3) hipLaunchKernelGGL(find_blocks_stage2<3>, grid, dim3(64), 0, st, in, nbytes, cand, shard_cap, count, work, final_count, final_list, final_cap, dbg);
    else if (exp == 4) hipLaunchKernelGGL(find_blocks_stage2<4>, grid, dim3(64), 0, st, in, nbytes, cand, shard_cap, count, work, final_count, final_list, final_cap, dbg);
    else hipLaunchKernelGGL(find_blocks_stage2<0>, grid, dim3(64), 0, st, in, nbytes, cand, shard_cap, count, work, final_count, final_list, final_cap, dbg);
    LFX_LAUNCH_CHECK();
    return 0;
}

}
```

Before: 58.64 GB/s.

## Materialize placed decode blocks directly from per-lane regions, skip dense code gather

Splits the placement kernel so it only computes flags and units, and moves the copy of per-lane code regions into a dense code array into a separate gather kernel. The materialize kernel can now read codes straight from the per-lane temp regions through a small cursor that binary-searches lane offsets. The gather runs only on paths that still need dense codes (giant blocks, symbol/window and chained runs), and the dense buffer is reserved lazily. This removes a full write and reread of the code stream on the common path, at the cost of indirect, less coalesced fetches inside materialize. Debug counters and a stats hook are also added.

After: 54.81 GB/s. -6.5%, worse.

```diff
diff --git a/include/lfx_testhooks.h b/include/lfx_testhooks.h
--- a/include/lfx_testhooks.h
+++ b/include/lfx_testhooks.h
@@ -19,6 +19,8 @@
 
 void lfx_debug_symbols(uint32_t length, uint32_t distance, uint32_t *out6);
 
+int lfx_debug_decode_stats(lfx_ctx *ctx, uint64_t *out2);
+
 #ifdef __cplusplus
 }
 #endif
diff --git a/libflate_amd/csrc/lfx_ctx.h b/libflate_amd/csrc/lfx_ctx.h
--- a/libflate_amd/csrc/lfx_ctx.h
+++ b/libflate_amd/csrc/lfx_ctx.h
@@ -58,6 +58,7 @@
     std::vector<uint8_t> range_stored;
     std::vector<uint64_t> range_temp_off;
     std::vector<uint32_t> range_cap;
+    uint64_t stat_region_blocks = 0, stat_copied_codes = 0;
     Diag diag;
     int n_cu = 0;
     hipStream_t own_stream = nullptr, stream = nullptr;
diff --git a/libflate_amd/csrc/lfx_decode.cpp b/libflate_amd/csrc/lfx_decode.cpp
--- a/libflate_amd/csrc/lfx_decode.cpp
+++ b/libflate_amd/csrc/lfx_decode.cpp
@@ -1,4 +1,5 @@
 #include "../../include/lfx.h"
+#include "../../include/lfx_testhooks.h"
 
 #include <hip/hip_runtime.h>
 
@@ -506,9 +507,33 @@
                 const uint32_t ne = (uint32_t)emit.size();
                 if ((rc = c->d_dec_tmp.reserve(sizeof(BlkEmit) * 2 * (size_t)ne + 64))) return rc;
                 if ((rc = c->d_hist.reserve(sizeof(BlkUnits) * 2 * (size_t)ne + 64))) return rc;
-                if ((rc = c->d_codes.reserve(4 * std::max<uint64_t>(total_codes, 1)))) return rc;
+                bool giant = pieces_multi;
+                for (const BlkEmit &e : emit) giant |= e.n_out >= (8ull << 20);
+                bool dense_reserved = false, dense = false;
+                auto reserve_dense = [&]() -> int {
+                    if (dense_reserved) return 0;
+                    dense_reserved = true;
+                    return c->d_codes.reserve(4 * std::max<uint64_t>(total_codes, 1));
+                };
                 uint32_t *d_flags = (uint32_t *)c->d_dec_tmp.p;
                 BlkEmit *d_emit = (BlkEmit *)((uint8_t *)c->d_dec_tmp.p + 64);
+                auto gather = [&]() -> int {
+                    if (dense || !n_placed) { dense = true; return 0; }
+                    const int r = reserve_dense();
+                    if (r) return r;
+                    LAUNCH_TRY(launch_blk_gather(st, d_emit, ne, (const BlkLanes *)c->d_dec_blocks.p, (const BlkLanesX *)c->d_dec_lanesx.p,
+                                                 (const uint32_t *)c->d_dec_temp.p, (uint32_t *)c->d_codes.p));
+                    for (const BlkEmit &e : emit) if (e.placed) c->stat_copied_codes += e.n_codes;
+                    dense = true;
+                    return 0;
+                };
+                auto materialize = [&](const BlkEmit *jobs, uint32_t nj_, const BlkUnits *un, uint64_t *dbg_) -> int {
+                    LAUNCH_TRY(launch_blk_materialize(st, d_in, jobs, nj_, (const BlkLanes *)c->d_dec_blocks.p, un, (const uint32_t *)c->d_codes.p,
+                                                      d_out, dbg_, dense ? nullptr : (const BlkLanesX *)c->d_dec_lanesx.p,
+                                                      dense ? nullptr : (const uint32_t *)c->d_dec_temp.p));
+                    return 0;
+                };
+                if ((n_placed < ne || giant) && (rc = reserve_dense())) return rc;
                 uint64_t *dbgbuf = nullptr;
                 if (c->diag.debug) {
                     if ((rc = c->d_ck.reserve(64ull * 8 * ne + 64))) return rc;
@@ -528,15 +553,13 @@
                 if (c->diag.free_shift >= 0) free_shift = (uint32_t)c->diag.free_shift;
                 if (n_placed)
                     LAUNCH_TRY(launch_blk_place(st, d_emit, ne, (const BlkLanes *)c->d_dec_blocks.p, (const BlkLanesX *)c->d_dec_lanesx.p,
-                                                (const uint32_t *)c->d_dec_temp.p, (uint32_t *)c->d_codes.p, d_flags,
-                                                (BlkUnits *)c->d_hist.p, unit_target, nullptr, free_shift));
+                                                d_flags, (BlkUnits *)c->d_hist.p, unit_target, nullptr, free_shift));
                 if (n_placed < ne)
                     LAUNCH_TRY(launch_blk_emit(st, d_in, n, d_emit, ne, (const BlkLanes *)c->d_dec_blocks.p,
                                                (uint32_t *)c->d_codes.p, d_flags, (BlkUnits *)c->d_hist.p, unit_target, nullptr,
                                                c->d_dec_tabs.p, free_shift, total_codes >= 32768ull * ne, scan_small && !pieces_mode));
+                if (giant && (rc = gather())) return rc;
                 c->phase("blk_emit");
-                bool giant = pieces_multi;
-                for (const BlkEmit &e : emit) giant |= e.n_out >= (8ull << 20);
                 const bool probe = !giant && total / ne < (256u << 10);
                 uint32_t fl = 0;
                 if (probe) {
@@ -545,8 +568,8 @@
                 }
                 bool ck_spec = false;
                 if (!giant && !(probe && fl == 2 && !c->diag.no_markers)) {
-                    LAUNCH_TRY(launch_blk_materialize(st, d_in, d_emit, ne, (const BlkLanes *)c->d_dec_blocks.p,
-                                                      (const BlkUnits *)c->d_hist.p, (const uint32_t *)c->d_codes.p, d_out, dbgbuf));
+                    if ((rc = materialize(d_emit, ne, (const BlkUnits *)c->d_hist.p, dbgbuf))) return rc;
+                    if (!dense) for (const BlkEmit &e : emit) c->stat_region_blocks += e.placed && e.n_codes;
                     const uint64_t tb = (pos == stop_bit ? pos : last_end), tpos = tb / 8 + ((tb & 7) ? 1 : 0);
                     if (mr.ck_mode && total && !partial && !c->diag.debug && tpos + mr.trailer_len <= n) {
                         c->phase("lz77_copy");
@@ -570,8 +593,7 @@
                 }
                 if (giant && !(fl & 1) && !c->diag.no_markers) fl = 2;
                 else if (giant) {
-                    LAUNCH_TRY(launch_blk_materialize(st, d_in, d_emit, ne, (const BlkLanes *)c->d_dec_blocks.p,
-                                                      (const BlkUnits *)c->d_hist.p, (const uint32_t *)c->d_codes.p, d_out, dbgbuf));
+                    if ((rc = materialize(d_emit, ne, (const BlkUnits *)c->d_hist.p, dbgbuf))) return rc;
                     HIP_TRY(hipStreamSynchronize(st));
                 }
                 if (!ck_spec) c->phase("lz77_copy");
@@ -619,6 +641,7 @@
                     uint8_t *d_win = (uint8_t *)c->d_dec_win.p;
                     SymUnit *d_su = (SymUnit *)(d_win + 32768ull * std::max<uint32_t>(nsu, 1));
                     HIP_TRY(hipMemcpyAsync(d_su, su.data(), sizeof(SymUnit) * nsu, hipMemcpyHostToDevice, st));
+                    if ((rc = gather())) return rc;
                     LAUNCH_TRY(launch_blk_materialize_sym(st, d_in, d_emit, ne, (const BlkUnits *)c->d_hist.p,
                                                           (const uint32_t *)c->d_codes.p, (uint16_t *)c->d_dec_sym.p,
                                                           nsu <= (uint32_t)std::max(c->n_cu, 1) && !c->diag.window_chain));
@@ -661,9 +684,8 @@
                     BlkUnits *d_ru = (BlkUnits *)c->d_hist.p + ne;
                     HIP_TRY(hipMemcpyAsync(d_runs, runs.data(), sizeof(BlkEmit) * nr, hipMemcpyHostToDevice, st));
                     HIP_TRY(hipMemcpyAsync(d_ru, ru.data(), sizeof(BlkUnits) * nr, hipMemcpyHostToDevice, st));
-                    for (uint32_t q = 0; q < nr; q++)
-                        LAUNCH_TRY(launch_blk_materialize(st, d_in, d_runs + q, 1, (const BlkLanes *)c->d_dec_blocks.p, d_ru + q,
-                                                          (const uint32_t *)c->d_codes.p, d_out, nullptr));
+                    if ((rc = gather())) return rc;
+                    for (uint32_t q = 0; q < nr; q++) if ((rc = materialize(d_runs + q, 1, d_ru + q, nullptr))) return rc;
                     HIP_TRY(hipStreamSynchronize(st));
                     c->phase("lz77_chain");
                     if (c->diag.debug) fprintf(stderr, "[lfx]  cross-block references: %u blocks re-materialised in %u ordered runs\n", ne, nr);
@@ -1077,7 +1099,13 @@
     int rc;
     if ((rc = c->d_dec_tmp.reserve(sizeof(BlkEmit) * (size_t)ne + 64))) return rc;
     if ((rc = c->d_hist.reserve(sizeof(BlkUnits) * (size_t)ne + 64))) return rc;
-    if ((rc = c->d_codes.reserve(4 * std::max<uint64_t>(total_codes, 1)))) return rc;
+    bool dense_reserved = false;
+    auto reserve_dense = [&]() -> int {
+        if (dense_reserved) return 0;
+        dense_reserved = true;
+        return c->d_codes.reserve(4 * std::max<uint64_t>(total_codes, 1));
+    };
+    if (n_placed < emit.size() && (rc = reserve_dense())) return rc;
     uint32_t *d_flags = (uint32_t *)c->d_dec_tmp.p;
     BlkEmit *d_emit = (BlkEmit *)((uint8_t *)c->d_dec_tmp.p + 64);
     HIP_TRY(hipMemsetAsync(d_flags, 0, 64, st));
@@ -1088,8 +1116,7 @@
     while (free_shift < 20 && (total >> (free_shift + 1)) >= 2ull * (uint64_t)std::max(c->n_cu, 1)) free_shift++;
     if (n_placed)
         LAUNCH_TRY(launch_blk_place(st, d_emit, ne, (const BlkLanes *)c->d_dec_blocks.p, (const BlkLanesX *)c->d_dec_lanesx.p,
-                                    (const uint32_t *)c->d_dec_temp.p, (uint32_t *)c->d_codes.p, d_flags, (BlkUnits *)c->d_hist.p,
-                                    unit_target, nullptr, free_shift));
+                                    d_flags, (BlkUnits *)c->d_hist.p, unit_target, nullptr, free_shift));
     if (n_placed < ne)
         LAUNCH_TRY(launch_blk_emit(st, d_in, n_part, d_emit, ne, (const BlkLanes *)c->d_dec_blocks.p, (uint32_t *)c->d_codes.p, d_flags,
                                    (BlkUnits *)c->d_hist.p, unit_target, nullptr, c->d_dec_tabs.p, free_shift, total_codes >= 32768ull * ne));
@@ -1102,7 +1129,9 @@
     }
     if (!(probe && fl)) {
         LAUNCH_TRY(launch_blk_materialize(st, d_in, d_emit, ne, (const BlkLanes *)c->d_dec_blocks.p, (const BlkUnits *)c->d_hist.p,
-                                          (const uint32_t *)c->d_codes.p, d_out, nullptr));
+                                          (const uint32_t *)c->d_codes.p, d_out, nullptr, (const BlkLanesX *)c->d_dec_lanesx.p,
+                                          (const uint32_t *)c->d_dec_temp.p));
+        for (const BlkEmit &e : emit) c->stat_region_blocks += e.placed && e.n_codes;
         HIP_TRY(hipMemcpyAsync(&fl, d_flags, 4, hipMemcpyDeviceToHost, st));
         HIP_TRY(hipStreamSynchronize(st));
     }
@@ -1131,6 +1160,12 @@
         if ((rc = c->d_dec_maps.reserve(window_prefix_scratch_bytes(std::max<uint32_t>(nsu, 1))))) return rc;
         SymUnit *d_su = (SymUnit *)((uint8_t *)c->d_dec_win.p + 32768ull * (std::max<uint32_t>(nsu, 1) + 1));
         HIP_TRY(hipMemcpyAsync(d_su, su.data(), sizeof(SymUnit) * nsu, hipMemcpyHostToDevice, st));
+        if (n_placed) {
+            if ((rc = reserve_dense())) return rc;
+            LAUNCH_TRY(launch_blk_gather(st, d_emit, ne, (const BlkLanes *)c->d_dec_blocks.p, (const BlkLanesX *)c->d_dec_lanesx.p,
+                                         (const uint32_t *)c->d_dec_temp.p, (uint32_t *)c->d_codes.p));
+            for (const BlkEmit &e : emit) if (e.placed) c->stat_copied_codes += e.n_codes;
+        }
         LAUNCH_TRY(launch_blk_materialize_sym(st, d_in, d_emit, ne, (const BlkUnits *)c->d_hist.p, (const uint32_t *)c->d_codes.p,
                                               (uint16_t *)c->d_dec_sym.p, nsu <= (uint32_t)std::max(c->n_cu, 1)));
         HIP_TRY(hipStreamSynchronize(st));
@@ -1138,6 +1173,15 @@
         c->range.state = 1; c->range.nsu = nsu; c->range.max_len = max_len;
         if (state) *state = 1;
     }
+    return LFX_OK;
+} LFX_ABI_CATCH
+
+extern "C" int lfx_debug_decode_stats(lfx_ctx *cc, uint64_t *out2) try {
+    if (!cc || !out2) return LFX_E_ARG;
+    Ctx *c = reinterpret_cast<Ctx *>(cc);
+    std::lock_guard<std::recursive_mutex> lock(c->mu);
+    out2[0] = c->stat_region_blocks; out2[1] = c->stat_copied_codes;
+    c->stat_region_blocks = c->stat_copied_codes = 0;
     return LFX_OK;
 } LFX_ABI_CATCH
 
diff --git a/libflate_amd/csrc/lfx_decode.h b/libflate_amd/csrc/lfx_decode.h
--- a/libflate_amd/csrc/lfx_decode.h
+++ b/libflate_amd/csrc/lfx_decode.h
@@ -127,8 +127,9 @@
 int launch_blk_scan_store(hipStream_t st, const uint8_t *in, uint64_t nbytes, const BlkJob *jobs, uint32_t njobs,
                           BlkInfo *infos, BlkLanes *lanes, void *tabs, uint32_t *temp, BlkLanesX *lanesx);
 int launch_blk_place(hipStream_t st, const BlkEmit *jobs, uint32_t njobs, const BlkLanes *lanes, const BlkLanesX *lanesx,
-                     const uint32_t *temp, uint32_t *codes, uint32_t *flags, BlkUnits *units, uint32_t unit_target,
-                     uint32_t *job_flags, uint32_t free_shift);
+                     uint32_t *flags, BlkUnits *units, uint32_t unit_target, uint32_t *job_flags, uint32_t free_shift);
+int launch_blk_gather(hipStream_t st, const BlkEmit *jobs, uint32_t njobs, const BlkLanes *lanes, const BlkLanesX *lanesx,
+                      const uint32_t *temp, uint32_t *codes);
 int launch_blk_emit(hipStream_t st, const uint8_t *in, uint64_t nbytes, const BlkEmit *jobs, uint32_t njobs,
                     const BlkLanes *lanes, uint32_t *codes, uint32_t *flags, BlkUnits *units, uint32_t unit_target,
                     uint32_t *job_flags = nullptr,
@@ -138,7 +139,8 @@
                     bool small_blocks = false);
 int launch_blk_materialize(hipStream_t st, const uint8_t *in, const BlkEmit *jobs, uint32_t njobs,
                            const BlkLanes *lanes, const BlkUnits *units, const uint32_t *codes, uint8_t *out,
-                           uint64_t *dbg);
+                           uint64_t *dbg,
+                           const BlkLanesX *lanesx = nullptr, const uint32_t *temp = nullptr);
 
 int launch_blk_materialize_sym(hipStream_t st, const uint8_t *in, const BlkEmit *jobs, uint32_t njobs,
                                const BlkUnits *units, const uint32_t *codes, uint16_t *sym,
diff --git a/libflate_amd/csrc/lfx_inflate_fast.hip b/libflate_amd/csrc/lfx_inflate_fast.hip
--- a/libflate_amd/csrc/lfx_inflate_fast.hip
+++ b/libflate_amd/csrc/lfx_inflate_fast.hip
@@ -1146,15 +1146,36 @@
 
 
 __global__ __launch_bounds__(SCAN_THREADS) void blk_place_kernel(const BlkEmit *__restrict__ jobs, const BlkLanes *__restrict__ lanes,
-                                                                  const BlkLanesX *__restrict__ lanesx, const uint32_t *__restrict__ temp,
-                                                                  uint32_t *__restrict__ codes, uint32_t *__restrict__ flags,
+                                                                  const BlkLanesX *__restrict__ lanesx, uint32_t *__restrict__ flags,
                                                                   BlkUnits *__restrict__ units, uint32_t unit_target, uint32_t free_shift,
                                                                   uint32_t *__restrict__ job_flags) {
-    const uint32_t tid = threadIdx.x, lane = tid & 63;
+    const uint32_t tid = threadIdx.x;
     const BlkEmit job = jobs[blockIdx.x];
     if (!job.placed) return;
     const uint64_t t_begin = clock64();
     BlkUnits *U = &units[blockIdx.x];
+    const BlkLanes *L = &lanes[job.cand];
+    const BlkLanesX *X = &lanesx[job.cand];
+    int64_t reach = INT64_MAX;
+    uint32_t cut_code = 0xFFFFFFFFu;
+    uint64_t cut_pos = 0;
+    if (tid < job.nlanes) {
+        const uint64_t out0 = L->out_off[tid];
+        const int32_t rr = X->reach[tid];
+        if (rr != INT32_MAX) reach = (int64_t)out0 + (int64_t)rr;
+        const uint32_t cc = X->cut_code[tid];
+        if (cc != 0xFFFFFFFFu) { cut_code = L->code_off[tid] + cc; cut_pos = out0 + X->cut_out[tid]; }
+    }
+    blk_flag_reach(tid, reach, job.hist, flags, job_flags);
+    blk_units_tail(tid, job, L, reach, cut_code, cut_pos, U, unit_target, free_shift, t_begin, t_begin);
+}
+
+__global__ __launch_bounds__(SCAN_THREADS) void blk_gather_kernel(const BlkEmit *__restrict__ jobs, const BlkLanes *__restrict__ lanes,
+                                                                   const BlkLanesX *__restrict__ lanesx, const uint32_t *__restrict__ temp,
+                                                                   uint32_t *__restrict__ codes) {
+    const uint32_t tid = threadIdx.x, lane = tid & 63;
+    const BlkEmit job = jobs[blockIdx.x];
+    if (!job.placed) return;
     const BlkLanes *L = &lanes[job.cand];
     const BlkLanesX *X = &lanesx[job.cand];
     const bool live = tid < job.nlanes;
@@ -1196,20 +1217,6 @@
                 }
         }
     }
-    if (blockIdx.y != 0) return;
-    const uint64_t t_hdr = clock64();
-    int64_t reach = INT64_MAX;
-    uint32_t cut_code = 0xFFFFFFFFu;
-    uint64_t cut_pos = 0;
-    if (live) {
-        const uint64_t out0 = L->out_off[tid];
-        const int32_t rr = X->reach[tid];
-        if (rr != INT32_MAX) reach = (int64_t)out0 + (int64_t)rr;
-        const uint32_t cc = X->cut_code[tid];
-        if (cc != 0xFFFFFFFFu) { cut_code = my_off + cc; cut_pos = out0 + X->cut_out[tid]; }
-    }
-    blk_flag_reach(tid, reach, job.hist, flags, job_flags);
-    blk_units_tail(tid, job, L, reach, cut_code, cut_pos, U, unit_target, free_shift, t_begin, t_hdr);
 }
 
 template <uint32_t THREADS>
@@ -1247,12 +1254,47 @@
     static constexpr uint32_t SW_BYTES = 2 * G::WAVES * 4;
     static constexpr uint32_t BYTES = RING_BYTES + P_BYTES + XC_BYTES + SW_BYTES;
 };
+struct M2Fetch {
+    const uint32_t *code_off, *n_head, *rest_at;
+    const uint32_t *reg0;
+    const uint32_t *reg;
+    uint32_t cap, t, lo, hi, nh, at;
+    __device__ __forceinline__ void load_slice() {
+        nh = n_head[t]; at = rest_at[t];
+        reg = reg0 + (uint64_t)t * cap;
+    }
+    __device__ __forceinline__ void open(const BlkLanes *L, const BlkLanesX *X, const uint32_t *region0, uint32_t cap_, uint32_t first) {
+        code_off = L->code_off; n_head = X->n_head; rest_at = X->rest_at; reg0 = region0; cap = cap_;
+        t = 0;
+#pragma unroll 1
+        for (uint32_t step = SCAN_THREADS / 2; step; step >>= 1) if (code_off[t + step] <= first) t += step;
+        lo = code_off[t];
+        hi = t + 1 < (uint32_t)SCAN_THREADS ? code_off[t + 1] : 0xFFFFFFFFu;
+        load_slice();
+    }
+    __device__ __forceinline__ uint32_t get(uint32_t i) {
+        if (i >= hi) {
+            do {
+                ++t;
+                lo = hi;
+                hi = t + 1 < (uint32_t)SCAN_THREADS ? code_off[t + 1] : 0xFFFFFFFFu;
+            } while (i >= hi);
+            load_slice();
+        }
+        const uint32_t j = i - lo;
+        return reg[j < nh ? j : at + (j - nh)];
+    }
+};
+
 template <bool SYM, uint32_t THREADS, bool DYN = false>
 __device__ __forceinline__ void materialize2_body(const uint8_t *__restrict__ in, const BlkEmit *__restrict__ jobs,
                                                   const BlkUnits *__restrict__ units,
                                                   const uint32_t *__restrict__ codes,
                                                   typename std::conditional<SYM, uint16_t, uint8_t>::type *__restrict__ out,
-                                                  uint32_t njobs, uint64_t *__restrict__ dbg) {
+                                                  uint32_t njobs, uint64_t *__restrict__ dbg,
+                                                  const BlkLanes *__restrict__ lanes = nullptr,
+                                                  const BlkLanesX *__restrict__ lanesx = nullptr,
+                                                  const uint32_t *__restrict__ temp = nullptr) {
     using elem_t = typename std::conditional<SYM, uint16_t, uint8_t>::type;
     using G = M2<THREADS>;
     using LD = M2Lds<SYM, THREADS>;
@@ -1293,6 +1335,9 @@
     elem_t *o = out + gbase;
     const uint32_t *cp = codes + job.code_off + c0;
     const uint32_t n = c1 - c0;
+    const bool regions = !SYM && temp != nullptr && job.placed;
+    M2Fetch fx;
+    if (regions) fx.open(&lanes[job.cand], &lanesx[job.cand], temp + job.temp_off, job.cap, c0);
     const uint32_t hist = SYM ? 32768u : (u == 0 && job.preload) ? (uint32_t)(job.hist < 32768 ? job.hist : 32768) : 0;
     const uint32_t shift = (uint32_t)((gbase - hist) & (EPD - 1)) + hist;
     for (uint32_t k = tid; k < hist; k += THREADS)
@@ -1302,7 +1347,14 @@
     uint32_t tr = shift;
     uint32_t fr = shift;
     uint32_t base = 0, ntiles = 0, nrounds = 0;
-    uint32_t cw0 = 2 * tid < n ? cp[2 * tid] : 0u, cw1 = 2 * tid + 1 < n ? cp[2 * tid + 1] : 0u;
+    uint32_t cw0 = 0u, cw1 = 0u;
+    if (regions) {
+        if (2 * tid < n) cw0 = fx.get(c0 + 2 * tid);
+        if (2 * tid + 1 < n) cw1 = fx.get(c0 + 2 * tid + 1);
+    } else {
+        cw0 = 2 * tid < n ? cp[2 * tid] : 0u;
+        cw1 = 2 * tid + 1 < n ? cp[2 * tid + 1] : 0u;
+    }
     const uint64_t t0 = dbg ? clock64() : 0;
     while (base < n) {
         if ((ntiles & (M2_PRIO_TILES - 1)) == 0) {
@@ -1342,8 +1394,14 @@
             total = XC[take - 1].x;
         }
         const uint32_t j0 = 2 * tid + take, j1 = j0 + 1;
-        const uint32_t rf0 = (j0 >= NC && base + j0 < n) ? cp[base + j0] : 0u;
-        const uint32_t rf1 = (j1 >= NC && base + j1 < n) ? cp[base + j1] : 0u;
+        uint32_t rf0 = 0u, rf1 = 0u;
+        if (regions) {
+            if (j0 >= NC && base + j0 < n) rf0 = fx.get(c0 + base + j0);
+            if (j1 >= NC && base + j1 < n) rf1 = fx.get(c0 + base + j1);
+        } else {
+            rf0 = (j0 >= NC && base + j0 < n) ? cp[base + j0] : 0u;
+            rf1 = (j1 >= NC && base + j1 < n) ? cp[base + j1] : 0u;
+        }
         uint32_t pp[PASSES][4];
         bool pend = false;
         auto round0 = [&](auto periodic_tag) {
@@ -1468,8 +1526,11 @@
                                                                    const BlkUnits *__restrict__ units,
                                                                    const uint32_t *__restrict__ codes,
                                                                    uint8_t *__restrict__ out, uint32_t njobs,
-                                                                   uint64_t *__restrict__ dbg) {
-    materialize2_body<false, THREADS>(in, jobs, units, codes, out, njobs, dbg);
+                                                                   uint64_t *__restrict__ dbg,
+                                                                   const BlkLanes *__restrict__ lanes,
+                                                                   const BlkLanesX *__restrict__ lanesx,
+                                                                   const uint32_t *__restrict__ temp) {
+    materialize2_body<false, THREADS>(in, jobs, units, codes, out, njobs, dbg, lanes, lanesx, temp);
 }
 
 __global__ __launch_bounds__(1024) void window_chain_kernel(const uint16_t *__restrict__ sym,
@@ -2077,11 +2138,17 @@
     return 0;
 }
 int launch_blk_place(hipStream_t st, const BlkEmit *jobs, uint32_t njobs, const BlkLanes *lanes, const BlkLanesX *lanesx,
-                     const uint32_t *temp, uint32_t *codes, uint32_t *flags, BlkUnits *units, uint32_t unit_target, uint32_t *job_flags,
-                     uint32_t free_shift) {
+                     uint32_t *flags, BlkUnits *units, uint32_t unit_target, uint32_t *job_flags, uint32_t free_shift) {
     if (!njobs) return 0;
-    hipLaunchKernelGGL(blk_place_kernel, dim3(njobs, 2), dim3(SCAN_THREADS), 0, st, jobs, lanes, lanesx, temp, codes, flags, units,
+    hipLaunchKernelGGL(blk_place_kernel, dim3(njobs), dim3(SCAN_THREADS), 0, st, jobs, lanes, lanesx, flags, units,
                        unit_target ? unit_target : 1u, free_shift < 15 ? 15u : free_shift, job_flags);
+    LFX_LAUNCH_CHECK();
+    return 0;
+}
+int launch_blk_gather(hipStream_t st, const BlkEmit *jobs, uint32_t njobs, const BlkLanes *lanes, const BlkLanesX *lanesx,
+                      const uint32_t *temp, uint32_t *codes) {
+    if (!njobs) return 0;
+    hipLaunchKernelGGL(blk_gather_kernel, dim3(njobs, 2), dim3(SCAN_THREADS), 0, st, jobs, lanes, lanesx, temp, codes);
     LFX_LAUNCH_CHECK();
     return 0;
 }
@@ -2113,12 +2180,13 @@
 }
 int launch_blk_materialize(hipStream_t st, const uint8_t *in, const BlkEmit *jobs, uint32_t njobs,
                            const BlkLanes *lanes, const BlkUnits *units, const uint32_t *codes, uint8_t *out,
-                           uint64_t *dbg) {
+                           uint64_t *dbg, const BlkLanesX *lanesx, const uint32_t *temp) {
     if (!njobs) return 0;
+    if (!lanesx) temp = nullptr;
     if (njobs <= M2_FEW_JOBS)
-        hipLaunchKernelGGL(blk_materialize2_kernel<M2_WIDE_THREADS>, dim3(njobs * MAX_UNITS), dim3(M2_WIDE_THREADS), 0, st, in, jobs, units, codes, out, njobs, dbg);
+        hipLaunchKernelGGL(blk_materialize2_kernel<M2_WIDE_THREADS>, dim3(njobs * MAX_UNITS), dim3(M2_WIDE_THREADS), 0, st, in, jobs, units, codes, out, njobs, dbg, lanes, lanesx, temp);
     else
-        hipLaunchKernelGGL(blk_materialize2_kernel<M2_THREADS>, dim3(njobs * MAX_UNITS), dim3(M2_THREADS), 0, st, in, jobs, units, codes, out, njobs, dbg);
+        hipLaunchKernelGGL(blk_materialize2_kernel<M2_THREADS>, dim3(njobs * MAX_UNITS), dim3(M2_THREADS), 0, st, in, jobs, units, codes, out, njobs, dbg, lanes, lanesx, temp);
     LFX_LAUNCH_CHECK();
     return 0;
 }
```
